# ffs97/deep-mixture-vae

Hardware: AMD Instinct MI355X
Metric: images/sec (train), MNIST K=10 z=64 batch=4096/GPU bf16 (higher is better)
Workload: dtype bf16; 1 GPU; configs[1]: DMVAE MLP 784-500-500-(2000|2000)-z64/K10-2000-500-500-784, one ELBO training step (gather+fwd+loss+bwd+Adam), synthetic rows resident in HBM; per_gpu_batch=4096, global_batch=4096, parallelism=dp1, rccl_ranks=0, multi_rank_rccl_verified_before_this_run=False, hip_graph=True, float_atomics=False, update=adam fused into the dW launch, mode=exact (expectation over q(c|x), priors.py:130-145)

## Files before the change

### deep-mixture-vae_amd/csrc/api.hip

```cpp
#include <stdarg.h>
#include <stdlib.h>
#include <string.h>

#include <map>
#include <mutex>
#include <string>
#include <vector>

#include "plan.h"
#include "gmm_fit.h"
#include "gmm_seed.h"
#include "eval_clusters.h"
#include "eval_loglik.h"
#include "tsne.h"
#include "cluster_metrics.h"
#include "mixture_density.h"
#include "knn.h"
#include "measure.h"

namespace dmvae {

static thread_local char g_err[512] = "";
void set_error(const char* fmt, ...) {
    va_list ap;
// ... 361 lines not shown
    if (me != hipSuccess) { set_error("dmvae_debug_conv_dw memset: %s", hipGetErrorString(me)); return (int)me; }
    return conv_layer_dw((hipStream_t)stream, dtype, rows, conv_p, conv_c, kdim, X, ldx, dY, ldy, N, n_valid, split, slab, dW, db);
}

static int debug_finalize_args(const dmvae_debug_finalize* f, const char* who, dmvae_finalize_args* out) {
    DMVAE_REQUIRE(f && f->rp && f->lp && f->state && f->nr >= 0 && f->nl >= 0 && f->nblk >= 0 && f->ncol >= 0 && (f->ncol == 0 || (f->part && f->gout)),
                  "%s: step_finalize arguments: null pointer or negative count", who);
    *out = step_finalize_args(f->rp, f->nr, f->lp, f->nl, f->inv_B, f->state, f->bump_adam, f->b1, f->b2, f->part, f->nblk, f->ncol, f->gout);
    return 0;
}
extern "C" int dmvae_debug_step_finalize(void* stream, const dmvae_debug_finalize* fin) {
    dmvae_finalize_args f;
    TRY(debug_finalize_args(fin, "dmvae_debug_step_finalize", &f));
    return step_finalize_launch((hipStream_t)stream, f.rp, f.nr, f.lp, f.nl, f.inv_B, f.st, f.bump_adam, f.b1, f.b2, f.part, f.nblk, f.ncol, f.gout);
}
extern "C" int dmvae_debug_gemm_dx_riders(void* stream, int M, int N, int K, const void* A, int64_t lda, const void* B, int64_t ldb, const dmvae_epilogue* epi,
                                          const dmvae_debug_finalize* fin, const dmvae_debug_gather* gat, int ngat, int gat_last) {
    DMVAE_REQUIRE(epi && (epi->kind == DMVAE_EPI_LATENT || epi->kind == DMVAE_EPI_RELU_MASK), "dmvae_debug_gemm_dx_riders: the LATENT or RELU_MASK epilogue");
    DMVAE_REQUIRE(fin || gat, "dmvae_debug_gemm_dx_riders: no riders (use dmvae_gemm)");
    DMVAE_REQUIRE(gat ? (ngat > 0 && ngat % 8 == 0) : ngat == 0, "dmvae_debug_gemm_dx_riders: ngat=%d: a positive multiple of 8 with a gather, 0 without", ngat);
    DMVAE_REQUIRE(!(fin && gat && gat->state), "dmvae_debug_gemm_dx_riders: step_finalize advances the batch cursor a gather addressed through the state reads: not in one launch");
    GemmArgs a;
    TRY(gemm_checked((hipStream_t)stream, DMVAE_BF16, DMVAE_GEMM_DX, M, N, K, A, lda, B, ldb, epi, 1, &a));
    GemmRiders r{};
    if (fin) {
        TRY(debug_finalize_args(fin, "dmvae_debug_gemm_dx_riders", &r.fin));
        r.nfin = (r.fin.nblocks + 7) & ~7;
    }
    if (gat) {
        DMVAE_REQUIRE(gat->data && gat->out_bf16 && gat->n_rows >= 0 && gat->dim > 0 && gat->B_pad > 0 && gat->n_valid >= 0 && gat->n_valid <= gat->B_pad &&
                      gat->ld % 4 == 0 && gat->ld >= gat->dim && (int64_t)gat->B_pad * (gat->ld / 4) < (int64_t(1) << 31) - int64_t(512) * 512 * 16,
                      "dmvae_debug_gemm_dx_riders: gather arguments (ld a multiple of 4, >= dim; n_valid <= B_pad; B_pad x ld within 32-bit quad indices)");
        r.gat = gather_args(DMVAE_BF16, gat->data, gat->n_rows, gat->dim, gat->perm, gat->first, gat->batch, gat->n_valid, gat->B_pad, gat->out_bf16, gat->ld,
                            nullptr, gat->ld, (int)gat->ld, gat->state);
        r.ngat = ngat;
        r.gat_last = gat_last ? 1 : 0;
    }
    DMVAE_REQUIRE(gemm_bf16_riders_room(a, false) >= r.nfin + r.ngat, "dmvae_debug_gemm_dx_riders: %d rider ids, the launch has room for %d (-1: not a small-tile launch)",
                  r.nfin + r.ngat, gemm_bf16_riders_room(a, false));
    DMVAE_REQUIRE(!fin || gemm_bf16_carries_finalize(a), "dmvae_debug_gemm_dx_riders: the two-wave 16-row tile cannot carry the step_finalize blocks");
    return gemm_bf16_dispatch((hipStream_t)stream, DMVAE_GEMM_DX, a, 1, &r);
}
extern "C" int dmvae_debug_gemm_grouped_fin(void* stream, const dmvae_gemm_problem* probs, int n, const dmvae_debug_finalize* fin) {
    DMVAE_REQUIRE(probs && n >= 1 && n <= DMVAE_MAX_GROUP, "dmvae_debug_gemm_grouped_fin: 1..%d problems", DMVAE_MAX_GROUP);
    dmvae_finalize_args f;
    TRY(debug_finalize_args(fin, "dmvae_debug_gemm_grouped_fin", &f));
    hipStream_t s = (hipStream_t)stream;
    std::vector<GemmArgs> q(n);
    for (int i = 0; i < n; ++i) {
        const dmvae_gemm_problem& pr = probs[i];
        TRY(gemm_checked(s, DMVAE_BF16, DMVAE_GEMM_DX, pr.M, pr.N, pr.K, pr.A, pr.lda, pr.B, pr.ldb, &pr.epi, 1, &q[i]));
    }
    return gemm_bf16_grouped(s, DMVAE_GEMM_DX, q.data(), n, &f);
}

extern "C" int dmvae_prof_enable(int on) {
    std::lock_guard<std::mutex> lk(g_prof_mu);
    g_prof_on = on != 0;
    return 0;
}
extern "C" int dmvae_prof_collect(dmvae_prof_row* rows, int max_rows) {
    std::lock_guard<std::mutex> lk(g_prof_mu);
    std::map<std::string, dmvae_prof_row> agg;
    std::vector<std::string> order;
    for (auto& r : g_prof) {
        (void)hipEventSynchronize(r.e1);
        float ms = 0.f;
        (void)hipEventElapsedTime(&ms, r.e0, r.e1);
        double kms = 0.0;
        bool kok = !r.k.empty();
        for (auto& pr : r.k) {
            float d = 0.f;
            if (hipEventSynchronize(pr.second) != hipSuccess || hipEventElapsedTime(&d, pr.first, pr.second) != hipSuccess || !(d > 0.f)) kok = false;
            kms += d;
            g_event_pool.push_back(pr.first);
            g_event_pool.push_back(pr.second);
        }
        (void)hipGetLastError();
        auto it = agg.find(r.name);
        if (it == agg.end()) {
            dmvae_prof_row row;
            memset(&row, 0, sizeof(row));
            snprintf(row.name, sizeof(row.name), "%s", r.name);
            it = agg.emplace(r.name, row).first;
            order.push_back(r.name);
        }
        it->second.launches += 1;
        it->second.total_ms += ms;
        it->second.kernel_ms += kok ? kms : 0.0;
        it->second.kernel_launches += kok ? (int64_t)r.k.size() : 0;
        it->second.flops += r.flops;
        it->second.bytes += r.bytes;
        g_event_pool.push_back(r.e0);
        g_event_pool.push_back(r.e1);
    }
    g_prof.clear();
    g_prof_cur = -1;
    int n = 0;
    for (auto& k : order) {
        if (n >= max_rows) break;
        rows[n++] = agg[k];
    }
    return n;
}

extern "C" int dmvae_debug_set_tile(int bm, int bn) {
// ... 20 lines not shown
```

### deep-mixture-vae_amd/csrc/gemm_bf16.hip

```cpp
#include <algorithm>
#include <cmath>
#include <functional>
#include <map>
#include <mutex>
#include <string>
#include <vector>

#include "gemm_tile.h"
#include "measure.h"

MEAS_TABLES_BF16

namespace dmvae {

template <int BM, int BN, int LAYOUT, int EPI, int NSTAGE, int NW, int BKT = BK, bool CONV = false, bool BONLY = false>
__device__ __forceinline__ void gemm_bf16_body(const GemmArgs& a, const int bid_raw, const int gstart, const int nwg, bf16_t* smem,
                                               const dmvae_adam_ctx* ac = nullptr, const int kslice = -1) {
    constexpr bool A_KC = (LAYOUT != DMVAE_GEMM_DW);
    constexpr bool B_KC = (LAYOUT == DMVAE_GEMM_DX);
    constexpr int A_ELEMS = BM * BKT, B_ELEMS = BN * BKT, STAGE = A_ELEMS + B_ELEMS;
    constexpr int WM = NW / 2;
    constexpr int TM = BM / (16 * WM), TN = BN / 32;
    static_assert(!BONLY || (LAYOUT == DMVAE_GEMM_DW && EPI == DMVAE_EPI_STORE_F32 && !CONV), "bias-only strips: dense DW / STORE_F32");
    constexpr int LOADS = ((BONLY ? 0 : BM) + BN) * BKT / (512 * NW);
// ... 185 lines not shown
    float lat[LAT_PRE ? NQ : 1][12];
    if constexpr (LAT_PRE) {
#pragma unroll
        for (int q = 0; q < NQ; ++q) {
            const int idx = q * (64 * NW) + tid;
            const int ml = idx / (BN / 4), c = idx % (BN / 4);
            loadf4(a.epi.aux0, (int64_t)(m0 + ml) * a.epi.ld0 + n0 + c * 4, lat[q]);
            loadf4(a.epi.aux1, (int64_t)(m0 + ml) * a.epi.ld1 + n0 + c * 4, lat[q] + 4);
            loadf4(a.epi.aux2, (int64_t)(m0 + ml) * a.epi.ld2 + n0 + c * 4, lat[q] + 8);
        }
    }
    constexpr bool HAS_BIAS = (EPI == DMVAE_EPI_BIAS_RELU || EPI == DMVAE_EPI_BIAS_F32 || EPI == DMVAE_EPI_BIAS_SIGMOID || EPI == DMVAE_EPI_BIAS_RECON);
    static_assert((64 * NW) % (BN / 4) == 0, "a thread keeps its column block across the epilogue's passes");
    float bq[4] = {0.f, 0.f, 0.f, 0.f};
    if constexpr (HAS_BIAS) loadf4(a.epi.bias, n0 + (tid % (BN / 4)) * 4, bq);
    uint2 gate[EPI == DMVAE_EPI_RELU_MASK ? NQ : 1];
    if constexpr (EPI == DMVAE_EPI_RELU_MASK) {
#pragma unroll
        for (int q = 0; q < NQ; ++q) {
            const int idx = q * (64 * NW) + tid;
            const int ml = idx / (BN / 4), c = idx % (BN / 4);
            if constexpr (MEAS_NO_MASK_READ) gate[q] = make_uint2(0x3f803f80u, 0x3f803f80u);
            else gate[q] = *reinterpret_cast<const uint2*>(reinterpret_cast<const bf16_t*>(a.epi.aux0) + (int64_t)(m0 + ml) * a.epi.ld0 + n0 + c * 4);
        }
    }
#pragma unroll
    for (int t = 0; t < NSTAGE; ++t)
        if (t < nk) issue(t, t);
    if (nk >= NSTAGE) wait_vmcnt<LOADS*(NSTAGE - 1)>();
    else wait_vmcnt<0>();
    __builtin_amdgcn_s_barrier();
    MEAS_ANAT(1);
    rd(0, 0, f0a, f0b);
    for (int kt = 0; kt < nk; kt += NSTAGE) {
#pragma unroll
        for (int s = 0; s < NSTAGE; ++s) {
            if (kt + s < nk) {
                rd(s, 1, f1a, f1b);
                mma(f0a, f0b);
                asm volatile("s_waitcnt lgkmcnt(0)" ::: "memory");
                if (kt + s + NSTAGE <= nk) wait_vmcnt<LOADS*(NSTAGE - 2)>();
                else wait_vmcnt<0>();
                __builtin_amdgcn_s_barrier();
                if constexpr (!MEAS_NO_KLOOP_LOADS) {
                    if (kt + s + NSTAGE < nk) issue(kt + s + NSTAGE, s);
                }
                if (kt + s + 1 < nk) rd((s + 1) % NSTAGE, 0, f0a, f0b);
                mma(f1a, f1b);
            }
        }
    }
    wait_vmcnt<0>();
    __builtin_amdgcn_s_barrier();
    MEAS_KLOOP_END();
    MEAS_ANAT(2);

    float loss = 0.f;
    const int li = lane & 15, g = lane >> 4;
    constexpr int CH = BN / 4, NT = 64 * NW;
    static_assert(BM * BN * 4 <= NSTAGE * STAGE * 2, "fp32 tile must fit in the ring");
    dmvae_epilogue epi_s = a.epi;
    if constexpr (EPI == DMVAE_EPI_STORE_F32 && (CONV || LAYOUT == DMVAE_GEMM_DW)) {
        const int ys = kslice >= 0 ? kslice : (int)blockIdx.y;
        epi_s.out = reinterpret_cast<float*>(epi_s.out) + (int64_t)ys * a.slab_stride;
        if (epi_s.out2) epi_s.out2 = reinterpret_cast<float*>(epi_s.out2) + (int64_t)ys * a.slab_stride2;
    }
    float* ct = reinterpret_cast<float*>(smem);
    if constexpr (MEAS_NO_EPILOGUE) {
#pragma unroll
        for (int i = 0; i < TM; ++i)
#pragma unroll
            for (int j = 0; j < TN; ++j) asm volatile("" ::"v"(acc[i][j]));
    } else if constexpr (!BONLY) {
#pragma unroll
    for (int i = 0; i < TM; ++i)
#pragma unroll
        for (int j = 0; j < TN; ++j) {
            const int ml = wm * (BM / WM) + i * 16 + li;
            const int c = (wn * (BN / 2) + j * 16) / 4 + g;
            *reinterpret_cast<f32x4*>(ct + ml * BN + ((c ^ (ml & 7)) << 2)) = acc[i][j];
        }
    __syncthreads();
    constexpr int KSPLIT_MAX_S = 8;
    constexpr bool KSLICE_OK = !CONV && LAYOUT != DMVAE_GEMM_DW && BM * BN <= 4096 && NW <= 4 && BM * BN * 4 + 16 <= NSTAGE * STAGE * 2 &&
                               (EPI == DMVAE_EPI_BIAS_RELU || EPI == DMVAE_EPI_RELU_MASK || EPI == DMVAE_EPI_BIAS_F32 || EPI == DMVAE_EPI_LATENT);
    if constexpr (KSLICE_OK) {
        if (a.tick != nullptr && gridDim.y > 1) {
            const int S = (int)gridDim.y, tile_lin = tm * tiles_n + tn;
            constexpr int Q = BM * BN;
            static_assert(KSPLIT_MAX_S == 8, "the combine issues eight loads per quad");
            f32x4* slab0 = reinterpret_cast<f32x4*>(a.ws) + (int64_t)tile_lin * S * (Q / 4);
            const f32x4* ct4 = reinterpret_cast<const f32x4*>(ct);
            for (int q = tid; q < Q / 4; q += 64 * NW) {
                const f32x4 v = ct4[q];
                f32x4* dst = slab0 + (int64_t)blockIdx.y * (Q / 4) + q;
                asm volatile("global_store_dwordx4 %0, %1, off sc1" ::"v"(dst), "v"(v) : "memory");
            }
            asm volatile("s_waitcnt vmcnt(0)" ::: "memory");
            __syncthreads();
            int* flag = reinterpret_cast<int*>(ct + BM * BN);
            if (tid == 0) *flag = __hip_atomic_fetch_add(a.tick + tile_lin, 1, __ATOMIC_RELAXED, __HIP_MEMORY_SCOPE_AGENT);
            __syncthreads();
            if (*flag != S - 1) return;
            for (int q = tid; q < Q / 4; q += 64 * NW) {
                const f32x4 *p0, *p1, *p2, *p3, *p4, *p5, *p6, *p7;
                auto at = [&](int sl) { return slab0 + (int64_t)(sl < S ? sl : S - 1) * (Q / 4) + q; };
// ... 131 lines not shown
    __shared__ __attribute__((aligned(16))) bf16_t smem[NSTAGE * (BM + BN) * BK];
    gemm_bf16_body<BM, BN, LAYOUT, EPI, NSTAGE, NW>(a, blockIdx.x, 0, gridDim.x, smem);
}

template <int BM, int BN, int EPI, int NSTAGE, int NW>
__global__ __launch_bounds__(64 * NW, NW / 2) void gemm_bf16_dx_riders_kernel(GemmArgs a, GemmRiders r) {
    __shared__ __attribute__((aligned(16))) bf16_t smem[NSTAGE * (BM + BN) * BK];
    const int lead = r.nfin + (r.gat_last ? 0 : r.ngat);
    if (blockIdx.y > 0 && ((int)blockIdx.x < lead || (r.gat_last && (int)blockIdx.x >= (int)gridDim.x - r.ngat))) return;
    if (r.gat_last && (int)blockIdx.x >= (int)gridDim.x - r.ngat) {
        if constexpr (MEAS_EMPTY_GATHER_RIDERS) return;
        gather_rows_block<bf16_t, 16>((int)blockIdx.x - ((int)gridDim.x - r.ngat), 64 * NW, r.gat);
        return;
    }
    if ((int)blockIdx.x < r.nfin) {
        if (NW > 4 && threadIdx.x >= 256) return;
        if ((int)blockIdx.x < r.fin.nblocks) step_finalize_block((int)blockIdx.x, r.fin, reinterpret_cast<float(*)[17]>(smem));
        return;
    }
    if ((int)blockIdx.x < lead) {
        if constexpr (MEAS_EMPTY_GATHER_RIDERS) return;
        gather_rows_block<bf16_t, 16>((int)blockIdx.x - r.nfin, 64 * NW, r.gat);
        return;
    }
    gemm_bf16_body<BM, BN, DMVAE_GEMM_DX, EPI, NSTAGE, NW>(a, (int)blockIdx.x - lead, lead, (int)gridDim.x - lead - (r.gat_last ? r.ngat : 0), smem);
}

template <int BM, int BN, int LAYOUT, int EPI, int NSTAGE, int NW>
__global__ __launch_bounds__(64 * NW, NW / 2) void gemm_bf16_conv_kernel(GemmArgs a) {
    __shared__ __attribute__((aligned(16))) bf16_t smem[NSTAGE * (BM + BN) * BK];
    if constexpr (LAYOUT == DMVAE_GEMM_DW) {
        if ((gridDim.y & 7) == 0) {
            const int L = (int)(blockIdx.y * gridDim.x + blockIdx.x), xcd = L & 7, j = L >> 3, T = (int)gridDim.x;
            gemm_bf16_body<BM, BN, LAYOUT, EPI, NSTAGE, NW, BK, true>(a, j % T, 0, -1, smem, nullptr, (j / T) * 8 + xcd);
            return;
        }
    }
    gemm_bf16_body<BM, BN, LAYOUT, EPI, NSTAGE, NW, BK, true>(a, blockIdx.x, 0, gridDim.x, smem);
}

void* gemm_bf16_anatomy() { return MEAS_SYMBOL(g_anat); }
void* gemm_bf16_stamps() { return MEAS_SYMBOL(g_stamps); }
struct GroupedArgs {
    int nprob;
    int kind[DMVAE_MAX_GROUP];
    int start[DMVAE_MAX_GROUP + 1];
    int cls_start[DMVAE_MAX_GROUP], cls_end[DMVAE_MAX_GROUP];
    int nsl[DMVAE_MAX_GROUP];
    GemmArgs p[DMVAE_MAX_GROUP];
    dmvae_adam_ctx adam;
    dmvae_finalize_args fin;
    int lead, lead_work;
    int xcut, xr0[8], xcnt[8];
};
template <int BM, int BN, int LAYOUT, int EPI, int NSTAGE, int NW = 4, bool SHORTK = false>
__global__ __launch_bounds__(64 * NW, NW == 8 ? 4 : 1) void gemm_bf16_grouped_kernel(GroupedArgs g) {
    __shared__ __attribute__((aligned(16))) bf16_t smem[SHORTK ? 2 * (64 + 64) * BK : 3 * (128 + 64) * BK];
    const dmvae_adam_ctx* ac = EPI == DMVAE_EPI_ADAM ? &g.adam : nullptr;
    if constexpr (EPI == DMVAE_EPI_ADAM) {
        if ((int)blockIdx.x < g.lead) {
            if ((int)blockIdx.x >= g.lead_work) return;
            const int64_t n4 = g.adam.seg_n >> 2;
            for (int64_t q = (int64_t)blockIdx.x * (64 * NW) + threadIdx.x; q < n4; q += (int64_t)g.lead_work * (64 * NW)) {
                const int64_t off = g.adam.seg_off + 4 * q;
                const float4 gq = *reinterpret_cast<const float4*>(g.adam.grad + off);
                const float gv[4] = {gq.x, gq.y, gq.z, gq.w};
                adam_quad(g.adam, off, gv);
            }
            return;
        }
    }
    int bx = (int)blockIdx.x;
    if constexpr (EPI == DMVAE_EPI_ADAM) bx -= g.lead;
    if constexpr (EPI == DMVAE_EPI_RELU_MASK) {
        if (bx < g.lead) {
            if (NW > 4 && threadIdx.x >= 256) return;
            if (bx < g.fin.nblocks) step_finalize_block(bx, g.fin, reinterpret_cast<float(*)[17]>(smem));
            return;
        }
        bx -= g.lead;
    }
    int i = 0, item;
    if (g.xcut) {
        const int x = bx & 7, j = bx >> 3;
        if (j >= g.xcnt[x]) return;
        item = g.xr0[x] + j;
    } else {
        while (i + 1 < g.nprob && bx >= g.start[i + 1]) ++i;
        item = g.cls_start[i] + xcd_run_index(bx, g.cls_start[i], g.cls_end[i]);
    }
    i = 0;
    while (i + 1 < g.nprob && item >= g.start[i + 1]) ++i;
    int bid = item - g.start[i];
    const int kind = g.kind[i];
    const int gs = 0, cnt = -1;
    int ksl = -1;
    if (g.nsl[i] > 1) {
        const int tiles_i = (g.start[i + 1] - g.start[i]) / g.nsl[i];
        ksl = bid / tiles_i;
        bid -= ksl * tiles_i;
    }
    MEAS_WG_BEGIN();
    if constexpr (SHORTK) {
        gemm_bf16_body<64, 64, LAYOUT, EPI, 2, NW>(g.p[i], bid, gs, cnt, smem, ac, ksl);
    } else {
        if (kind == 0) gemm_bf16_body<128, 128, LAYOUT, EPI, 2, NW>(g.p[i], bid, gs, cnt, smem, ac, ksl);
        else if (kind == 1) gemm_bf16_body<128, 64, LAYOUT, EPI, 3, NW>(g.p[i], bid, gs, cnt, smem, ac, ksl);
        else if (kind == 3) {
            if constexpr (LAYOUT == DMVAE_GEMM_DW && EPI == DMVAE_EPI_STORE_F32)
                gemm_bf16_body<64, 64, LAYOUT, EPI, 4, NW, BK, false, true>(g.p[i], bid, gs, cnt, smem, ac, ksl);
        }
// ... 26 lines not shown
        snprintf(nm[0], 64, "gemm_bf16_kernel<%d, %d, %d, %d, %d, %d>", BM, BN, LAYOUT, EPI, NSTAGE, NW);
        snprintf(nm[1], 64, "gemm_bf16_grouped_kernel<%d, %d, %d, %d, %d, %d>", BM, BN, LAYOUT, EPI, NSTAGE, NW);
        init = true;
    }
    return nm[grouped ? 1 : 0];
}
static double gemm_bytes(const GemmArgs& a, int layout = DMVAE_GEMM_FWD) {
    const int k = a.epi.kind;
    if (k == DMVAE_EPI_ADAM) return 2.0 * ((double)a.M * a.K + (double)a.K * a.N);
    const double osz = (k == DMVAE_EPI_STORE_F32 || k == DMVAE_EPI_ATOMIC_F32 || k == DMVAE_EPI_BIAS_F32 || k == DMVAE_EPI_BIAS_SIGMOID) ? 4.0 : 2.0;
    if (a.conv_c) {
        const double nv = a.epi.n_valid > 0 ? a.epi.n_valid : a.N;
        if (layout == DMVAE_GEMM_DW) return 2.0 * ((double)a.K * a.lda + (double)a.K * a.ldb) + 4.0 * a.M * nv;
        return 2.0 * ((double)a.M * a.lda + (double)a.K * a.N) + osz * a.M * nv;
    }
    return 2.0 * ((double)a.M * a.K + (double)a.K * a.N) + osz * a.M * a.N;
}

template <int BM, int BN, int LAYOUT, int EPI, int NSTAGE, int NW = 4>
static int launch(hipStream_t s, const GemmArgs& a, int split, const GemmRiders* riders = nullptr) {
    dim3 grid((a.M / BM) * (a.N / BN), split);
    if constexpr (LAYOUT == DMVAE_GEMM_DX && (EPI == DMVAE_EPI_LATENT || EPI == DMVAE_EPI_RELU_MASK)) {
        if (riders && (split == 1 || a.tick)) {
            GemmRiders r = *riders;
            double rbytes = 0.0;
            if (r.ngat) { r.gat.nblocks = r.ngat; rbytes = (double)r.gat.n_valid * r.gat.dim * (4 + 2); }
            ProfScope ps(s, kernel_name<BM, BN, LAYOUT, EPI, NSTAGE, NW>(false), 2.0 * a.M * a.N * (double)a.K, gemm_bytes(a) + rbytes);
            DMVAE_LAUNCH((gemm_bf16_dx_riders_kernel<BM, BN, EPI, NSTAGE, NW>), dim3(grid.x + r.nfin + r.ngat, split), dim3(64 * NW), 0, s, a, r);
            return check_launch("gemm_bf16 (dX + riders)");
        }
    }
    if (riders) { set_error("gemm_bf16: riders are carried by the dense DX launches with the LATENT or RELU_MASK epilogue only"); return DMVAE_EINVAL; }
    ProfScope ps(s, kernel_name<BM, BN, LAYOUT, EPI, NSTAGE, NW>(false), 2.0 * a.M * a.N * (double)a.K, gemm_bytes(a));
    DMVAE_LAUNCH((gemm_bf16_kernel<BM, BN, LAYOUT, EPI, NSTAGE, NW>), grid, dim3(64 * NW), 0, s, a);
    return check_launch("gemm_bf16");
}

template <int BM, int BN, int LAYOUT, int EPI, int NSTAGE, int NW = 4>
static int launch_conv(hipStream_t s, const GemmArgs& a, int split) {
    dim3 grid((a.M / BM) * (a.N / BN), split);
    static const std::string nm = [] {
        char b[64];
        snprintf(b, sizeof(b), "gemm_bf16_conv_kernel<%d, %d, %d, %d, %d, %d>", BM, BN, LAYOUT, EPI, NSTAGE, NW);
        return std::string(b);
    }();
    const double P = a.conv_p, inner = (P - 2.0) * (P - 2.0) / (P * P), nv = a.epi.n_valid > 0 ? a.epi.n_valid : a.N;
    const double fl = 2.0 * (LAYOUT == DMVAE_GEMM_DW ? (double)a.K : (double)a.M) * inner * 9.0 * a.conv_c * nv;
    ProfScope ps(s, nm.c_str(), fl, gemm_bytes(a, LAYOUT));
    DMVAE_LAUNCH((gemm_bf16_conv_kernel<BM, BN, LAYOUT, EPI, NSTAGE, NW>), grid, dim3(64 * NW), 0, s, a);
    return check_launch("gemm_bf16_conv");
}

template <int LAYOUT, int EPI>
static int grouped_launch(hipStream_t s, const GemmArgs* probs, int nprob, const dmvae_adam_ctx* ctx = nullptr, const dmvae_finalize_args* fin = nullptr) {
    auto best_kind = [](const GemmArgs& p) { return p.bias_only ? 3 : (p.M % 128 == 0 && p.N % 128 == 0) ? 0 : (p.M % 128 == 0 ? 1 : 2); };
    auto nslices = [](const GemmArgs& p) { return (p.k_split > 0 && p.k_split < p.K) ? p.K / p.k_split : 1; };
    auto tiles = [&](const GemmArgs& p, int kind) {
        if (kind == 3) return (p.N / 64) * nslices(p);
        return (p.M / (kind == 2 ? 64 : 128)) * (p.N / (kind == 0 ? 128 : 64)) * nslices(p);
    };
    auto wg_bytes = [&](const GemmArgs& p, int kind) {
        if (kind == 3) return 2.0 * 64 * (double)(p.K / nslices(p));
        return 2.0 * ((kind == 2 ? 64 : 128) + (kind == 0 ? 128 : 64)) * (double)(p.K / nslices(p));
    };
    int kinds[DMVAE_MAX_GROUP];
    bool shortk = g_shortk && LAYOUT != DMVAE_GEMM_DW && EPI != DMVAE_EPI_ADAM;
    for (int i = 0; i < nprob; ++i) shortk = shortk && probs[i].K <= 128;
    for (int i = 0; i < nprob; ++i) kinds[i] = (g_grouped_mixed && !shortk) ? best_kind(probs[i]) : 2;
    if (g_grouped_mixed == 1 && !shortk) {
        static std::mutex mu;
        static std::map<std::vector<int>, std::vector<int>> memo;
        std::vector<int> key;
        for (int i = 0; i < nprob; ++i) { key.push_back(probs[i].M); key.push_back(probs[i].N); key.push_back(probs[i].K); key.push_back(nslices(probs[i]) * 2 + (probs[i].bias_only ? 1 : 0)); }
        std::lock_guard<std::mutex> lk(mu);
        auto it = memo.find(key);
        if (it == memo.end()) {
            std::vector<int> cur(kinds, kinds + nprob), best = cur;
            double best_max = 1e300, best_sum = 1e300;
            std::vector<double> s;
            for (;;) {
                s.clear();
                double sum = 0.0;
                for (int i = 0; i < nprob; ++i) {
                    const int t = tiles(probs[i], cur[i]);
                    s.insert(s.end(), (size_t)t, wg_bytes(probs[i], cur[i]));
                    sum += t * wg_bytes(probs[i], cur[i]);
                }
                std::sort(s.begin(), s.end(), std::greater<double>());
                double load[256] = {0.0}, mx = 0.0;
                for (size_t j = 0; j < s.size(); ++j) load[j & 255] += s[j];
                for (double l : load) mx = std::max(mx, l);
                if (mx < best_max * 0.99 || (mx < best_max * 1.01 && sum < best_sum)) { best_max = std::min(mx, best_max); best_sum = sum; best = cur; }
                int i = 0;
                while (i < nprob && (cur[i] == 2 || kinds[i] == 3)) { cur[i] = kinds[i]; ++i; }
                if (i == nprob) break;
                ++cur[i];
            }
            it = memo.emplace(key, best).first;
        }
        for (int i = 0; i < nprob; ++i) kinds[i] = it->second[i];
    }
    int order[DMVAE_MAX_GROUP];
    for (int i = 0; i < nprob; ++i) order[i] = i;
    std::stable_sort(order, order + nprob, [&](int x, int y) { return wg_bytes(probs[x], kinds[x]) > wg_bytes(probs[y], kinds[y]); });
    GroupedArgs g;
    g.nprob = nprob;
    int total = 0, n = 0;
    double flops = 0.0, bytes = 0.0;
    for (int o = 0; o < nprob; ++o) {
        const int i = order[o], kind = kinds[i];
        g.start[n] = total;
        g.kind[n] = kind;
        g.nsl[n] = nslices(probs[i]);
        g.p[n] = probs[i];
        g.p[n].group_m = gemm_auto_group_m(probs[i].M / (kind >= 2 ? 64 : 128), probs[i].N / (kind == 0 ? 128 : 64),
                                      kind >= 2 ? 64 : 128, kind == 0 ? 128 : 64);
        total += tiles(probs[i], kind);
        flops += 2.0 * probs[i].M * probs[i].N * (double)probs[i].K;
        bytes += gemm_bytes(probs[i]);
        ++n;
    }
    for (int i = nprob; i < DMVAE_MAX_GROUP; ++i) { g.kind[i] = 2; g.nsl[i] = 1; }
    for (int i = nprob; i <= DMVAE_MAX_GROUP; ++i) g.start[i] = total;
    for (int i = 0; i < DMVAE_MAX_GROUP; ++i) { g.cls_start[i] = g.start[std::min(i, nprob)]; g.cls_end[i] = g.start[std::min(i + 1, nprob)]; }
    if (g_grouped_cls)
        for (int lo = 0; lo < nprob;) {
            int hi = lo + 1;
            while (hi < nprob && g.kind[hi] == g.kind[lo] && 2 * std::min(g.p[hi].K / g.nsl[hi], g.p[lo].K / g.nsl[lo]) > std::max(g.p[hi].K / g.nsl[hi], g.p[lo].K / g.nsl[lo])) ++hi;
            const double run = std::max(1.0, (g.start[hi] - g.start[lo]) / 8.0);
            for (int i = lo; i < hi; ++i) {
                g.cls_start[i] = g.start[lo];
                g.cls_end[i] = g.start[hi];
                const int kind = g.kind[i], bm = kind >= 2 ? 64 : 128, bn = kind == 0 ? 128 : 64;
                const int t = (g.start[i + 1] - g.start[i]) / g.nsl[i];
                g.p[i].group_m = gemm_auto_group_m(g.p[i].M / bm, g.p[i].N / bn, bm, bn, std::min<double>(t, run));
            }
            lo = hi;
        }
    g.xcut = 0;
    int grid_items = total;
    if (LAYOUT == DMVAE_GEMM_DW && g_grouped_xcut && total >= 64) {
        double tot_b = 0.0;
        std::vector<double> cost((size_t)total);
        for (int i = 0; i < nprob; ++i)
            for (int j = g.start[i]; j < g.start[i + 1]; ++j) { cost[j] = wg_bytes(g.p[i], g.kind[i]); tot_b += cost[j]; }
        int cuts[9] = {0};
        double acc = 0.0;
        int x = 1;
        for (int j = 0; j < total && x < 8; ++j) {
            acc += cost[j];
            while (x < 8 && acc >= tot_b * x / 8.0 - 1e-6) cuts[x++] = j + 1;
        }
        while (x < 8) cuts[x++] = total;
        cuts[8] = total;
        int mx = 0;
        for (int k = 0; k < 8; ++k) { g.xr0[k] = cuts[k]; g.xcnt[k] = cuts[k + 1] - cuts[k]; mx = std::max(mx, g.xcnt[k]); }
        g.xcut = 1;
        grid_items = 8 * mx;
        for (int i = 0; i < nprob; ++i) {
            int share = 1;
            for (int k = 0; k < 8; ++k) share = std::max(share, std::min(cuts[k + 1], g.start[i + 1]) - std::max(cuts[k], g.start[i]));
            const int kind = g.kind[i], bm = kind >= 2 ? 64 : 128, bn = kind == 0 ? 128 : 64;
            const int t = (g.start[i + 1] - g.start[i]) / g.nsl[i];
            g.p[i].group_m = gemm_auto_group_m(g.p[i].M / bm, g.p[i].N / bn, bm, bn, std::min<double>(t, share));
        }
    }
    int extra = 0;
    g.fin = dmvae_finalize_args{};
    g.lead = 0; g.lead_work = 0;
    if (fin && EPI == DMVAE_EPI_RELU_MASK) { g.fin = *fin; g.lead = (fin->nblocks + 7) & ~7; extra = g.lead; }
    g.adam = dmvae_adam_ctx{};
    if (ctx) {
        g.adam = *ctx;
        double elems = (double)ctx->seg_n;
        for (int i = 0; i < nprob; ++i) elems += (double)probs[i].M * probs[i].N + (probs[i].epi.out2 ? probs[i].N : 0);
        bytes += elems * (24.0 + (ctx->param_bf16 ? 2.0 : 0.0) + (ctx->store_grad ? 4.0 : 0.0)) + 4.0 * ctx->seg_n;
        if (ctx->seg_n > 0) { g.lead_work = (int)std::min<int64_t>(4, (ctx->seg_n / 4 + 255) / 256); g.lead = 8; extra = g.lead; }
    }
    static const std::string pname = [] {
        char b[64];
        snprintf(b, sizeof(b), "gemm_bf16_grouped_mixed_tiles<L%d, E%d>", LAYOUT, EPI);
        return std::string(b);
    }();
    ProfScope ps(s, pname.c_str(), flops, bytes);
    if constexpr (LAYOUT != DMVAE_GEMM_DW) {
        if (shortk) {
            DMVAE_LAUNCH((gemm_bf16_grouped_kernel<64, 64, LAYOUT, EPI, 2, 4, true>), dim3(total + extra), dim3(256), 0, s, g);
            return check_launch("gemm_bf16_grouped");
        }
    }
    if constexpr (LAYOUT == DMVAE_GEMM_DX && EPI == DMVAE_EPI_RELU_MASK) {
        if (g_dx_group_nw == 8) {
            DMVAE_LAUNCH((gemm_bf16_grouped_kernel<64, 64, LAYOUT, EPI, 4, 8>), dim3(total + extra), dim3(512), 0, s, g);
            return check_launch("gemm_bf16_grouped");
        }
    }
    DMVAE_LAUNCH((gemm_bf16_grouped_kernel<64, 64, LAYOUT, EPI, 4, 4>), dim3(grid_items + extra), dim3(256), 0, s, g);
    return check_launch("gemm_bf16_grouped");
}

int gemm_bf16_grouped(hipStream_t s, int layout, const GemmArgs* probs, int nprob, const dmvae_finalize_args* fin) {
    if (nprob < 1 || nprob > DMVAE_MAX_GROUP) { set_error("dmvae_gemm_grouped: 1..%d problems", DMVAE_MAX_GROUP); return DMVAE_EINVAL; }
    const int epi = probs[0].epi.kind;
    for (int i = 1; i < nprob; ++i)
        if (probs[i].epi.kind != epi) { set_error("dmvae_gemm_grouped: all problems must share the epilogue kind"); return DMVAE_EINVAL; }
    if (layout == DMVAE_GEMM_DW && epi == DMVAE_EPI_STORE_F32) return grouped_launch<DMVAE_GEMM_DW, DMVAE_EPI_STORE_F32>(s, probs, nprob);
    if (layout == DMVAE_GEMM_FWD && epi == DMVAE_EPI_BIAS_F32) return grouped_launch<DMVAE_GEMM_FWD, DMVAE_EPI_BIAS_F32>(s, probs, nprob);
    if (fin && !(layout == DMVAE_GEMM_DX && epi == DMVAE_EPI_RELU_MASK)) { set_error("dmvae_gemm_grouped: step_finalize rides on DX / RELU_MASK groups only"); return DMVAE_EINVAL; }
    if (layout == DMVAE_GEMM_DX && epi == DMVAE_EPI_RELU_MASK) {
        bool taken[DMVAE_MAX_GROUP];
        const int rc = heads_dx_stream_launch(s, probs, nprob, fin, taken);
        if (rc) return rc;
        GemmArgs rest[DMVAE_MAX_GROUP];
        int nrest = 0, ntaken = 0;
        for (int i = 0; i < nprob; ++i) {
            if (taken[i]) ++ntaken;
            else rest[nrest++] = probs[i];
        }
        if (nrest == 0) return 0;
        return grouped_launch<DMVAE_GEMM_DX, DMVAE_EPI_RELU_MASK>(s, rest, nrest, nullptr, ntaken ? nullptr : fin);
    }
    set_error("dmvae_gemm_grouped: layout %d with epilogue %d is not instantiated", layout, epi);
    return DMVAE_EUNSUPPORTED;
}
static int peel_large_dw(hipStream_t s, const GemmArgs* probs, int nprob, const dmvae_adam_ctx* ctx, std::vector<GemmArgs>& rest) {
    std::vector<GemmArgs> large;
    bool any = false;
    for (int i = 0; i < nprob; ++i)
        any = any || (probs[i].k_split == probs[i].K && gemm_bf16_256_ok(DMVAE_GEMM_DW, probs[i].epi.kind, probs[i].M, probs[i].N, probs[i].K, probs[i].conv_c != 0));
    for (int i = 0; i < nprob; ++i) {
        const GemmArgs& p = probs[i];
        if (p.k_split != p.K && !p.bias_only && !p.epi.out2 && p.slab_stride && gemm_bf16_256_slice_ok(p.M, p.N, p.k_split)) { large.push_back(p); continue; }
        const bool own = p.k_split == p.K && gemm_bf16_256_ok(DMVAE_GEMM_DW, p.epi.kind, p.M, p.N, p.K, p.conv_c != 0);
        const bool rides = any && gemm_bf16_256_rides() && p.k_split == p.K && !p.conv_c && p.M % 256 == 0 && p.N % 256 == 0 && p.K >= 1024 &&
                           (p.epi.kind == DMVAE_EPI_STORE_F32 || p.epi.kind == DMVAE_EPI_ADAM);
        if (own || rides) large.push_back(p);
        else rest.push_back(p);
    }
    return large.empty() ? 0 : gemm_bf16_256_dw_all(s, large.data(), (int)large.size(), ctx);
}
int gemm_bf16_grouped_dw(hipStream_t s, const GemmArgs* probs, int nprob) {
    if (nprob < 1 || nprob > DMVAE_MAX_GROUP) { set_error("dmvae_gemm_grouped_dw: 1..%d problems", DMVAE_MAX_GROUP); return DMVAE_EINVAL; }
    std::vector<GemmArgs> rest;
    for (int i = 0; i < nprob; ++i)
        if (probs[i].epi.kind != DMVAE_EPI_STORE_F32) return gemm_bf16_grouped(s, DMVAE_GEMM_DW, probs, nprob, nullptr);
    const int rc = peel_large_dw(s, probs, nprob, nullptr, rest);
    if (rc) return rc;
    return rest.empty() ? 0 : gemm_bf16_grouped(s, DMVAE_GEMM_DW, rest.data(), (int)rest.size(), nullptr);
}
int gemm_bf16_grouped_dw_adam(hipStream_t s, const GemmArgs* probs, int nprob, const dmvae_adam_ctx& ctx) {
    if (nprob < 1 || nprob > DMVAE_MAX_GROUP) { set_error("dmvae_gemm_grouped_dw_adam: 1..%d problems", DMVAE_MAX_GROUP); return DMVAE_EINVAL; }
    for (int i = 0; i < nprob; ++i)
        if (probs[i].epi.kind != DMVAE_EPI_ADAM || !probs[i].epi.out) { set_error("dmvae_gemm_grouped_dw_adam: every problem needs epilogue kind ADAM and out = its gradient address"); return DMVAE_EINVAL; }
    if (!ctx.param || !ctx.grad || !ctx.m || !ctx.v || !ctx.state || (ctx.seg_off & 3) || (ctx.seg_n & 3) || ctx.seg_n < 0) {
        set_error("dmvae_gemm_grouped_dw_adam: null arena / state, or a segment that is not a multiple of 4 elements");
        return DMVAE_EINVAL;
    }
    for (int i = 0; i < nprob; ++i) {
        const int64_t end = (reinterpret_cast<const float*>(probs[i].epi.out) - ctx.grad) + (int64_t)probs[i].M * probs[i].epi.ldo;
        if (end < 0 || end > ADAM_QUADS_MAX_ELEMS) { set_error("dmvae_gemm_grouped_dw_adam: gradient %d ends %lld elements into the arena (limit 2^30)", i, (long long)end); return DMVAE_EUNSUPPORTED; }
    }
    std::vector<GemmArgs> rest;
    dmvae_adam_ctx c1 = ctx;
    c1.seg_n = 0;
    const int rc = peel_large_dw(s, probs, nprob, &c1, rest);
    if (rc) return rc;
    if (!rest.empty()) return grouped_launch<DMVAE_GEMM_DW, DMVAE_EPI_ADAM>(s, rest.data(), (int)rest.size(), &ctx);
    if (ctx.seg_n > 0) {
        AdamArgs a;
        a.n = ctx.seg_n; a.p = ctx.param + ctx.seg_off; a.g = ctx.grad + ctx.seg_off; a.m = ctx.m + ctx.seg_off; a.v = ctx.v + ctx.seg_off;
        a.pb = ctx.param_bf16 ? reinterpret_cast<bf16_t*>(ctx.param_bf16) + ctx.seg_off : nullptr;
        a.lr = 0.f; a.b1 = ctx.beta1; a.b2 = ctx.beta2; a.eps = ctx.epsilon; a.gscale = ctx.grad_scale; a.zero_grad = 0; a.ieee = ctx.ieee;
        a.t_host = ~0ull; a.st = reinterpret_cast<const dmvae_state*>(ctx.state);
        return adam_launch(s, a);
    }
    return 0;
}

static int g_force_tile = 0;
void gemm_bf16_force_tile(int t) { g_force_tile = t; }
static int g_nw8 = 1;
void gemm_bf16_set_knob(int which, int v) {
    if (which == 0) g_group_m = v < 0 ? 0 : v;
    if (which == 1) g_nw8 = v;
    if (which == 2) g_grouped_mixed = v;
    if (which == 4) g_grouped_cls = v;
    if (which == 5) g_conv_short = v;
    if (which == 6) gemm_bf16_256_set_policy(v);
    if (which == 7) g_shortk = v;
    if (which == 8) gemm_bf16_256_set_stagger(v);
    if (which == 9) g_dx_group_nw = v;
    if (which == 18) g_thin = v;
    if (which == 20) g_grouped_xcut = v;
}

static int gemm_bf16_thin_rows(const GemmArgs& a) {
    if (!g_thin || a.conv_c || a.N != 64 || a.K < 1024 || (a.k_split != a.K && !a.tick)) return 0;
    if (g_thin >= 2 && a.M % 16 == 0 && a.M / 16 <= 256) return 16;
    if (a.M % 32 == 0 && a.M / 32 <= 256) return 32;
    return 0;
}

int gemm_bf16_tile_m(int M, int N, int split) {
    if (g_force_tile) {
        const int bm = g_force_tile / 1000, bn = g_force_tile % 1000;
        if (M % bm == 0 && N % bn == 0) return g_force_tile;
    }
    static const int cand[4][2] = {{128, 128}, {128, 64}, {64, 128}, {64, 64}};
    double best = -1.0;
    int pick = 64 * 1000 + 64;
    for (auto& c : cand) {
        if (M % c[0] || N % c[1]) continue;
        const double wgs = (double)(M / c[0]) * (N / c[1]) * split;
        const double score = (double)c[0] * c[1] / (c[0] + c[1]) * (wgs >= 256.0 ? 1.0 : wgs / 256.0);
        if (score > best * 1.0001) { best = score; pick = c[0] * 1000 + c[1]; }
    }
    if (pick == 128128 && (double)(M / 128) * (N / 128) * split <= 256.0 && (double)(M / 128) * (N / 64) * split >= 384.0) pick = 128064;
    return pick;
}

// ... 91 lines not shown
```

### deep-mixture-vae_amd/csrc/gemm_epilogue.h

```cpp
#pragma once
#include "common.h"

namespace dmvae {

struct GemmArgs {
    const void* A; int64_t lda;
    const void* B; int64_t ldb;
    int M, N, K, k_split;
    int group_m;
    int conv_p, conv_c;
    dmvae_epilogue epi;
    float* ws = nullptr; int64_t ws_elems = 0;
    int64_t slab_stride = 0;
    int64_t slab_stride2 = 0;
    float* csum_out = nullptr; int64_t csum_ld = 0;
    const float* csum_in = nullptr; int csum_rows = 0;
    int bias_only = 0;
    int* tick = nullptr;
};

__host__ __device__ __forceinline__ int64_t conv_tap_offset(int tap, int c0, int P, int64_t lda) {
    return (int64_t)((tap / 3 - 1) * P + (tap % 3 - 1)) * lda + c0;
}

template <typename T> struct ActIO;
template <> struct ActIO<bf16_t> {
    static __device__ __forceinline__ void store4(void* base, int64_t off, const float v[4]) {
        uint2 p;
        p.x = pack2bf(v[0], v[1]);
        p.y = pack2bf(v[2], v[3]);
        *reinterpret_cast<uint2*>(reinterpret_cast<bf16_t*>(base) + off) = p;
    }
    static __device__ __forceinline__ void load4(const void* base, int64_t off, float v[4]) {
        const uint2 p = *reinterpret_cast<const uint2*>(reinterpret_cast<const bf16_t*>(base) + off);
        v[0] = __uint_as_float(p.x << 16);
        v[1] = __uint_as_float(p.x & 0xffff0000u);
        v[2] = __uint_as_float(p.y << 16);
        v[3] = __uint_as_float(p.y & 0xffff0000u);
    }
};
template <> struct ActIO<float> {
    static __device__ __forceinline__ void store4(void* base, int64_t off, const float v[4]) {
        *reinterpret_cast<float4*>(reinterpret_cast<float*>(base) + off) = make_float4(v[0], v[1], v[2], v[3]);
    }
    static __device__ __forceinline__ void load4(const void* base, int64_t off, float v[4]) {
        const float4 p = *reinterpret_cast<const float4*>(reinterpret_cast<const float*>(base) + off);
        v[0] = p.x; v[1] = p.y; v[2] = p.z; v[3] = p.w;
    }
};

__device__ __forceinline__ void loadf4(const void* base, int64_t off, float v[4]) {
    ActIO<float>::load4(base, off, v);
}

__device__ __forceinline__ float xent_logits(float l, float x) {
    return fmaxf(l, 0.f) - l * x + log1pf(__expf(-fabsf(l)));
}
__device__ __forceinline__ float sigmoidf_(float l) { return 1.0f / (1.0f + __expf(-l)); }
struct dmvae_gather_args {
    const float* data; int64_t n_rows; int dim; const int32_t* perm;
    int64_t first; int batch, n_valid, B_pad;
    void* out_act; int64_t ld_act; float* out_f32; int64_t ld_f32; int cols_pad;
    const dmvae_state* st;
    int nblocks;
};
template <typename ACT, int U, bool PERM>
__device__ __forceinline__ void gather_rows_pass(const int base, const int nthreads, const int total, const int quads, const int64_t first, const dmvae_gather_args& g) {
    int r[U], c[U];
    int64_t idx[U];
    bool inb[U];
#pragma unroll
// ... 8 lines not shown
    if constexpr (PERM) {
#pragma unroll
        for (int u = 0; u < U; ++u) idx[u] = (int64_t)g.perm[idx[u]];
    }
    float4 q[U];
#pragma unroll
    for (int u = 0; u < U; ++u) {
        inb[u] = inb[u] && idx[u] >= 0 && idx[u] < g.n_rows && c[u] < g.dim;
        q[u] = *reinterpret_cast<const float4*>(g.data + (inb[u] ? idx[u] * g.dim + c[u] : 0));
    }
#pragma unroll
    for (int u = 0; u < U; ++u) {
        if (r[u] < 0) continue;
        const float v[4] = {inb[u] ? q[u].x : 0.f, inb[u] ? q[u].y : 0.f, inb[u] ? q[u].z : 0.f, inb[u] ? q[u].w : 0.f};
        if (g.out_act) ActIO<ACT>::store4(g.out_act, (int64_t)r[u] * g.ld_act + c[u], v);
        if (g.out_f32) ActIO<float>::store4(g.out_f32, (int64_t)r[u] * g.ld_f32 + c[u], v);
    }
}
template <typename ACT, int U = 8>
__device__ __forceinline__ void gather_rows_block(const int bx, const int nthreads, const dmvae_gather_args& g) {
    int64_t first = g.first;
    if (g.st) first = (int64_t)g.st->batch_cursor * g.batch;
    const int quads = g.cols_pad >> 2;
    const int total = g.B_pad * quads;
    if (g.dim % 4 == 0 && (reinterpret_cast<uintptr_t>(g.data) & 15) == 0 && g.n_rows > 0) {
        for (int base = bx * nthreads * U + (int)threadIdx.x; base < total; base += g.nblocks * nthreads * U) {
            if (g.perm) gather_rows_pass<ACT, U, true>(base, nthreads, total, quads, first, g);
            else gather_rows_pass<ACT, U, false>(base, nthreads, total, quads, first, g);
        }
        return;
    }
    for (int i = bx * nthreads + (int)threadIdx.x; i < total; i += g.nblocks * nthreads) {
        const int r = i / quads, c = (i - r * quads) * 4;
        float v[4] = {0.f, 0.f, 0.f, 0.f};
        if (r < g.n_valid) {
            int64_t src = first + r;
            if (g.perm) src = (src >= 0 && src < g.n_rows) ? (int64_t)g.perm[src] : -1;
            if (src >= 0 && src < g.n_rows) {
                const float* p = g.data + src * g.dim + c;
#pragma unroll
                for (int j = 0; j < 4; ++j) v[j] = (c + j < g.dim) ? p[j] : 0.f;
            }
        }
        if (g.out_act) ActIO<ACT>::store4(g.out_act, (int64_t)r * g.ld_act + c, v);
        if (g.out_f32) ActIO<float>::store4(g.out_f32, (int64_t)r * g.ld_f32 + c, v);
    }
}

struct GemmRiders {
    dmvae_finalize_args fin; int nfin = 0;
    dmvae_gather_args gat; int ngat = 0;
    int gat_last = 0;
};

__device__ __forceinline__ void xent_sigmoid(float l, float x, float& xent, float& sig) {
    const float e = __expf(-fabsf(l));
    const float inv = __frcp_rn(1.0f + e);
    xent = fmaxf(l, 0.f) - l * x + __logf(1.0f + e);
    sig = l >= 0.f ? inv : e * inv;
}

template <int EPI, typename ACT>
__device__ __forceinline__ void epilogue_quad(const dmvae_epilogue& e, int m, int n, float v[4], float& loss, const float* xpre = nullptr, float* stored = nullptr,
                                              const float* bpre = nullptr, const float* ypre = nullptr) {
    if constexpr (EPI == DMVAE_EPI_BIAS_RELU) {
        float b[4];
        if (bpre) { b[0] = bpre[0]; b[1] = bpre[1]; b[2] = bpre[2]; b[3] = bpre[3]; }
        else loadf4(e.bias, n, b);
#pragma unroll
        for (int j = 0; j < 4; ++j) v[j] = fmaxf(v[j] + b[j], 0.f);
        ActIO<ACT>::store4(e.out, (int64_t)m * e.ldo + n, v);
    } else if constexpr (EPI == DMVAE_EPI_BIAS_F32) {
        float b[4];
        if (bpre) { b[0] = bpre[0]; b[1] = bpre[1]; b[2] = bpre[2]; b[3] = bpre[3]; }
        else loadf4(e.bias, n, b);
#pragma unroll
        for (int j = 0; j < 4; ++j) v[j] += b[j];
        ActIO<float>::store4(e.out, (int64_t)m * e.ldo + n, v);
    } else if constexpr (EPI == DMVAE_EPI_BIAS_SIGMOID) {
        float b[4];
        if (bpre) { b[0] = bpre[0]; b[1] = bpre[1]; b[2] = bpre[2]; b[3] = bpre[3]; }
        else loadf4(e.bias, n, b);
#pragma unroll
        for (int j = 0; j < 4; ++j) v[j] = sigmoidf_(v[j] + b[j]);
        ActIO<float>::store4(e.out, (int64_t)m * e.ldo + n, v);
    } else if constexpr (EPI == DMVAE_EPI_BIAS_RECON) {
        float b[4], x[4], d[4];
        if (bpre) { b[0] = bpre[0]; b[1] = bpre[1]; b[2] = bpre[2]; b[3] = bpre[3]; }
        else loadf4(e.bias, n, b);
        if (xpre) { x[0] = xpre[0]; x[1] = xpre[1]; x[2] = xpre[2]; x[3] = xpre[3]; }
        else loadf4(e.aux0, (int64_t)m * e.ld0 + n, x);
        const bool rowok = m < e.m_valid;
#pragma unroll
        for (int j = 0; j < 4; ++j) {
            const float l = v[j] + b[j];
            v[j] = l;
            const bool ok = rowok && (n + j) < e.n_valid;
            if ((e.recon_kind & 0xff) == 0) {
                float xe, sg;
                xent_sigmoid(l, x[j], xe, sg);
                loss += ok ? xe : 0.f;
                d[j] = ok ? (sg - x[j]) * e.scale : 0.f;
            } else {
                const float r = l - x[j];
                loss += ok ? 0.5f * r * r : 0.f;
                d[j] = ok ? r * e.scale : 0.f;
// ... 41 lines not shown
```

### deep-mixture-vae_amd/csrc/kernels.h

```cpp
#pragma once
#include "gemm_epilogue.h"

namespace dmvae {

struct AdamArgs {
    int64_t n;
    float* p; float* g; float* m; float* v; bf16_t* pb;
    float lr, b1, b2, eps, gscale;
    int zero_grad;
    int ieee;
    uint64_t t_host;
    const dmvae_state* st;
};

#define DMVAE_MAX_GROUP 16
int gemm_bf16_dispatch(hipStream_t s, int layout, const GemmArgs& a, int split, const GemmRiders* riders = nullptr);
int gemm_bf16_riders_room(const GemmArgs& a, bool own_cu);
bool gemm_bf16_carries_finalize(const GemmArgs& a);
int gemm_bf16_grouped_dw(hipStream_t s, const GemmArgs* probs, int nprob);
int gemm_bf16_grouped(hipStream_t s, int layout, const GemmArgs* probs, int nprob, const dmvae_finalize_args* fin = nullptr);
dmvae_finalize_args step_finalize_args(const float* rp, int nr, const float* lp, int nl, float inv_B, void* st, int bump_adam,
                                       float b1, float b2, const float* part, int nblk, int ncol, float* gout);
int gemm_bf16_tile_m(int M, int N, int split);
int gemm_auto_group_m(int tiles_m, int tiles_n, int bm, int bn, double run = 0.0);
bool gemm_bf16_256_ok(int layout, int epi, int M, int N, int K, bool conv);
int gemm_bf16_256_launch(hipStream_t s, int layout, const GemmArgs& a, const dmvae_adam_ctx* ctx = nullptr);
void gemm_bf16_256_set_policy(int v);
void gemm_bf16_256_set_stagger(int v);
bool gemm_bf16_256_slice_ok(int M, int N, int k_split);
bool gemm_bf16_256_rides();
int gemm_bf16_256_dw_all(hipStream_t s, const GemmArgs* probs, int n, const dmvae_adam_ctx* ctx);
void* heads_dx_phase_table();
int heads_dx_stream_launch(hipStream_t s, const GemmArgs* probs, int nprob, const dmvae_finalize_args* fin, bool* taken);
void heads_dx_stream_set(int v);
void gemm_bf16_force_tile(int t);
void gemm_bf16_set_knob(int which, int v);
int gemm_f32_dispatch(hipStream_t s, int layout, const GemmArgs& a, int split);
int gemm_f32_trio(hipStream_t s, const GemmArgs& g1, int split1, const GemmArgs& g2, int split2, const GemmArgs& g3, int split3);
int latent_nblocks(int B_pad, int D, int K);
int latent_launch(hipStream_t s, const dmvae_latent_args* a);
void latent_set_blocks_target(int v);
int latent_vade_nblocks(int B_pad);
int latent_vade_launch(hipStream_t s, const dmvae_latent_args* a);
size_t latent_vade_lds_bytes(int D, int K);
bool latent_vade_mfma_needed(int D, int K);
bool latent_vade_mfma_forced();
void latent_vade_force_mfma(int v);
int64_t latent_vade_mfma_ws_bytes(int B_pad, int D, int K, int* n_slabs);
int latent_vade_mfma_launch(hipStream_t s, const dmvae_latent_args* a, float* ws, int64_t ws_bytes);
bool heads_latent_ok(int B_pad, int D, int K, int Dp, int Kp, int Hp, int mode, int rows_per_latent_block);
int heads_latent_launch(hipStream_t s, const dmvae_latent_args* a, const dmvae_heads_args* h);
void heads_latent_set(int v);
int64_t heads_latent_kslice_floats(int B_pad, int Dp, int slices);
int strip_fwd2_launch(hipStream_t s, int B_pad, int K0, const void* X, int64_t ldx, const void* W0, int64_t ld0, const float* b0,
                      const void* W1, int64_t ld1, const float* b1, void* Y1, int64_t ldy1, void* Y2, int64_t ldy2);
bool latent_mfma_applies(int D, int K, int mode);
int64_t latent_mfma_ws_bytes(int B_pad, int D, int K);
int latent_mfma_launch(hipStream_t s, const dmvae_latent_args* a, float* ws, int64_t ws_bytes);
int adam_launch(hipStream_t s, const AdamArgs& a);
int adam_shadow_launch(hipStream_t s, const AdamArgs& a, int blocks);
int adam_finish_launch(hipStream_t s, void* st);
int adam_slabs_launch(hipStream_t s, const AdamArgs& a, const float* slabs, int nslab, int64_t stride, int64_t seg_lo, int64_t seg_hi);
int slab_reduce_launch(hipStream_t s, const float* slabs, int64_t n, int nslab, int64_t stride, float* out);
int colsum_prepare(int64_t max_n);
float* colsum_global_scratch(int64_t* elems);
int colsum_launch(hipStream_t s, int in_dtype, const void* in, int64_t ld, int M, int N, float* out, float* ws, int64_t ws_elems);
int recon_nblocks(int B_pad, int I_pad);
int recon_launch(hipStream_t s, int act_dtype, int recon_kind, int B, int B_pad, int I, int I_pad, const float* logits, int64_t ldl,
                 const float* x, int64_t ldx, float inv_B, void* dl, int64_t ldd, float* partials);
int loss_finalize_launch(hipStream_t s, const float* rp, int nr, const float* lp, int nl, float inv_B, void* st, int bump_adam);
int step_finalize_launch(hipStream_t s, const float* rp, int nr, const float* lp, int nl, float inv_B, void* st, int bump_adam,
                         float b1, float b2, const float* part, int nblk, int ncol, float* gout);
int gemm_bf16_grouped_dw_adam(hipStream_t s, const GemmArgs* probs, int nprob, const dmvae_adam_ctx& ctx);
dmvae_gather_args gather_args(int act_dtype, const float* data, int64_t n_rows, int dim, const int32_t* perm, int64_t first, int batch, int n_valid,
                              int B_pad, void* out_act, int64_t ld_act, float* out_f32, int64_t ld_f32, int cols_pad, const void* st);
int gather_launch(hipStream_t s, int act_dtype, const float* data, int64_t n_rows, int dim, const int32_t* perm, int64_t first, int batch,
                  int n_valid, int B_pad, void* out_act, int64_t ld_act, float* out_f32, int64_t ld_f32, int cols_pad, const void* st);
int philox_launch(hipStream_t s, float* out, int64_t n, uint64_t seed, uint64_t step, uint32_t sid, int gumbel);
int cast_launch(hipStream_t s, const void* in, void* out, int64_t n, int to_bf16);
int spin_launch(hipStream_t s, int us);
void* gemm_bf16_stamps();
void* gemm_bf16_anatomy();
void* gemm_bf16_256_anatomy();
int conv_first_fwd_launch(hipStream_t s, int dtype, const void* x, int64_t bstride, int H, int64_t n_img, const void* W, int ldw,
                          const float* bias, int cout, void* out, int ld);
int conv_first_dw_blocks(int H, int64_t n_img);
int conv_first_dw_launch(hipStream_t s, int dtype, const void* x, int64_t bstride, int H, int64_t n_img, const void* dY, int ld, int cout,
                         float* dW, int ldw, float* db, float* part);
int zero_border_launch(hipStream_t s, int dtype, void* a, int P, int ld, int64_t n_img);
int maxpool2_fwd_launch(hipStream_t s, int dtype, const void* in, int H, int ld, int64_t n_img, void* out, int out_border);
int maxpool2_bwd_relu_launch(hipStream_t s, int dtype, const void* in, const void* dout, int H, int ld, int64_t n_img, void* din, int dout_border);
int conv_wflip_launch(hipStream_t s, int dtype, const void* W, int cin, int cin_ld, int cout, int ldw, void* Wt, int Kt);

}
```

### deep-mixture-vae_amd/csrc/measure.h

```cpp
#pragma once

#ifndef DMVAE_ABLATE
#define DMVAE_ABLATE 0
#endif

namespace dmvae {
constexpr bool MEAS_NO_MFMA = DMVAE_ABLATE == 1 || DMVAE_ABLATE == 4;
constexpr bool MEAS_NO_LDS_READ = DMVAE_ABLATE == 2 || DMVAE_ABLATE == 4;
constexpr bool MEAS_NO_KLOOP_LOADS = DMVAE_ABLATE == 3;
constexpr bool MEAS_NO_EPILOGUE = DMVAE_ABLATE == 5;
constexpr bool MEAS_NO_MASK_READ = DMVAE_ABLATE == 8;
constexpr bool MEAS_NO_BIAS_MFMA = DMVAE_ABLATE == 9;
constexpr bool MEAS_STAMPS = DMVAE_ABLATE == 6;
constexpr bool MEAS_NO_STEP_GATHER = DMVAE_ABLATE == 11;
constexpr bool MEAS_EMPTY_GATHER_RIDERS = DMVAE_ABLATE == 12;
}

#if DMVAE_ABLATE == 6
#define MEAS_TABLES_BF16                                  \
    __device__ unsigned long long g_mid[2048];            \
    __device__ unsigned long long g_anat[2048 * 8];       \
    __device__ unsigned long long g_stamps[2048 * 4];
#define MEAS_HWID() (((unsigned long long)__builtin_amdgcn_s_getreg((31 << 11) | 4) << 32) | (unsigned)__builtin_amdgcn_s_getreg((3 << 11) | 20))
#define MEAS_ANAT(i) do { if (threadIdx.x == 0 && blockIdx.x < 2048) g_anat[blockIdx.x * 8 + (i)] = __builtin_amdgcn_s_memrealtime(); } while (0)
#define MEAS_KLOOP_END() do { if (threadIdx.x == 0 && blockIdx.x < 2048) g_mid[blockIdx.x] = __builtin_amdgcn_s_memrealtime(); } while (0)
#define MEAS_ANAT_DRAIN()                                                                             \
    do {                                                                                              \
        MEAS_ANAT(3);                                                                                 \
        asm volatile("s_waitcnt vmcnt(0)" ::: "memory");                                              \
        MEAS_ANAT(4);                                                                                 \
        if (threadIdx.x == 0 && blockIdx.x < 2048) g_anat[blockIdx.x * 8 + 5] = MEAS_HWID();          \
    } while (0)
#define MEAS_WG_BEGIN() const unsigned long long meas_t0_ = __builtin_amdgcn_s_memrealtime()
#define MEAS_WG_END(layout, kind)                                                                                          \
    do {                                                                                                                   \
        if (threadIdx.x == 0 && blockIdx.x < 2048) {                                                                       \
            unsigned long long* st_ = g_stamps + 4 * blockIdx.x;                                                           \
            st_[0] = meas_t0_;                                                                                             \
            st_[1] = __builtin_amdgcn_s_memrealtime();                                                                     \
            st_[2] = MEAS_HWID();                                                                                          \
            st_[3] = ((g_mid[blockIdx.x] - meas_t0_) << 16) | ((unsigned long long)(layout) << 8) | (unsigned)(kind);       \
        }                                                                                                                  \
    } while (0)
#define MEAS_TABLES_256 __device__ unsigned long long g_anat256[4096 * 8];
#define MEAS_ANAT256(i)                                                                                  \
    do {                                                                                                 \
        if (threadIdx.x == 0 && blockIdx.x < 4096) {                                                     \
            g_anat256[blockIdx.x * 8 + (i)] = __builtin_amdgcn_s_memrealtime();                          \
            if ((i) < 2) g_anat256[blockIdx.x * 8 + 4 + (i)] = __builtin_amdgcn_s_memtime();             \
        }                                                                                                \
    } while (0)
#define MEAS_ANAT256_DRAIN()                                                                             \
    do {                                                                                                 \
        asm volatile("s_waitcnt vmcnt(0)" ::: "memory");                                                 \
        __syncthreads();                                                                                 \
        MEAS_ANAT256(2);                                                                                 \
        if (threadIdx.x == 0 && blockIdx.x < 4096) g_anat256[blockIdx.x * 8 + 3] = MEAS_HWID();          \
    } while (0)
#define MEAS_SYMBOL(sym) ([] { void* p_ = nullptr; return hipGetSymbolAddress(&p_, HIP_SYMBOL(sym)) == hipSuccess ? p_ : nullptr; }())
#else
#define MEAS_TABLES_BF16
#define MEAS_TABLES_256
#define MEAS_ANAT(i) do { } while (0)
#define MEAS_KLOOP_END() do { } while (0)
#define MEAS_ANAT_DRAIN() do { } while (0)
#define MEAS_WG_BEGIN() do { } while (0)
#define MEAS_WG_END(layout, kind) do { } while (0)
#define MEAS_ANAT256(i) do { } while (0)
#define MEAS_ANAT256_DRAIN() do { } while (0)
#define MEAS_SYMBOL(sym) (static_cast<void*>(nullptr))
#endif

#if DMVAE_ABLATE == 10
#define MEAS_TABLES_HDX __device__ unsigned long long g_hdx[1024 * 16];
#define MEAS_HDX_BEGIN() unsigned long long hx_[12] = {}; unsigned long long hx_last_; hx_[0] = __builtin_amdgcn_s_memtime(); hx_[10] = __builtin_amdgcn_s_memrealtime()
#define MEAS_HDX_MARK(i) do { hx_last_ = __builtin_amdgcn_s_memtime(); hx_[i] = hx_last_; } while (0)
#define MEAS_HDX_ACC(i) do { const unsigned long long t_ = __builtin_amdgcn_s_memtime(); hx_[i] += t_ - hx_last_; hx_last_ = t_; } while (0)
#define MEAS_HDX_END(steps)                                                                                                        \
    do {                                                                                                                           \
        MEAS_HDX_MARK(3);                                                                                                          \
        asm volatile("s_waitcnt vmcnt(0)" ::: "memory");                                                                           \
        MEAS_HDX_MARK(4);                                                                                                          \
        hx_[11] = __builtin_amdgcn_s_memrealtime();                                                                                \
        if (threadIdx.x == 0 && blockIdx.x < 1024) {                                                                               \
            for (int i_ = 0; i_ < 12; ++i_) g_hdx[blockIdx.x * 16 + i_] = hx_[i_];                                                 \
            g_hdx[blockIdx.x * 16 + 13] = (unsigned long long)(steps);                                                             \
            g_hdx[blockIdx.x * 16 + 12] = (((unsigned long long)__builtin_amdgcn_s_getreg((31 << 11) | 4) << 32) | (unsigned)__builtin_amdgcn_s_getreg((3 << 11) | 20)); \
        }                                                                                                                          \
    } while (0)
#define MEAS_SYMBOL_HDX(sym) ([] { void* p_ = nullptr; return hipGetSymbolAddress(&p_, HIP_SYMBOL(sym)) == hipSuccess ? p_ : nullptr; }())
#else
#define MEAS_TABLES_HDX
#define MEAS_HDX_BEGIN() do { } while (0)
#define MEAS_HDX_MARK(i) do { } while (0)
#define MEAS_HDX_ACC(i) do { } while (0)
#define MEAS_HDX_END(steps) do { } while (0)
#define MEAS_SYMBOL_HDX(sym) (static_cast<void*>(nullptr))
#endif

#if DMVAE_ABLATE == 7
#define MEAS_LAT_STAMP(i) do { if (blockIdx.x == 0 && threadIdx.x == 0) reinterpret_cast<unsigned long long*>(L.a.loss_partials + 2 * gridDim.x)[i] = __builtin_amdgcn_s_memrealtime(); } while (0)
#else
#define MEAS_LAT_STAMP(i) do { } while (0)
#endif
```

### deep-mixture-vae_amd/csrc/plan.h

```cpp
#pragma once
#include <string.h>

#include <string>
#include <vector>

#include "kernels.h"

#define TRY(x) do { int rc_ = (x); if (rc_) return rc_; } while (0)

struct PLayer {
    std::string name;
    int in, out, in_pad, out_pad;
    int64_t w_off, b_off, ldw;
};

struct PConv {
    std::string name;
    int cin, cout, hw, pool;
    int cin_ld, cout_ld;
    int cin_np, cout_np;
    int P;
    int kdim, ktdim;
    int64_t w_off, b_off;
    int64_t o_act, o_dact;
// ... 10 lines not shown
    const PAct* whole = nullptr;

    PAct sub(int c0, int n) const {
        PAct v = *this;
        v.off += (int64_t)c0 * es; v.cols = n; v.cs_live = false; v.whole = whole ? whole : this;
        if (cs >= 0) v.cs += (int64_t)c0 * 4;
        return v;
    }
    void mark_cs_live() const { (whole ? whole : this)->cs_live = true; }
};

struct dmvae_plan {
    dmvae_config cfg;
    std::vector<PConv> conv;
    int flat = 0;
    int64_t o_wt = 0, o_c0part = 0, o_cslab = 0;
    int64_t conv_param_end = 0;
    int Bp, Ip, Dp, Kp, Hp, Tp;
    int es;
    std::vector<PLayer> enc, dec;
    PLayer zc, mv, lg, out;
    int64_t prior_off;
    int64_t tail_off = 0;
    int64_t param_elems;
    std::vector<dmvae_tensor_info> tensors;
    struct {
        PAct x, xf, x2, cflat, dflat, hzc, mv, lg, Z, Zf, gmu, glv, clv, w, dlg, recon, dl, dmv, dhzc;
        std::vector<PAct> enc, dec, denc, ddec;
    } a;
    int64_t o_rpart, o_lpart, o_dprior, o_cs, o_lws = 0;
    int64_t lws_bytes = 0;
    int64_t o_ksws = -1, ksws_elems = 0, o_ktick = -1;
    int n_rpart, n_lblk, n_pblk;
    int n_lblk_cap = 0;
    int64_t cs_elems;
    int64_t work_bytes;
    dmvae_buffers buf;
    bool bound;
    std::vector<dmvae::GemmArgs> dw_queue;
    int dw_slices_max = 1;
    int64_t o_dwslab = 0;
    int dw_slices_now = 1;
    bool dw_macro_now = false;
    int dw_macro_tiles = 0;
    bool fused_update = false;
    bool staged = false;
    int stage_groups = 3;
    struct { const float* data; int64_t n_rows; const int32_t* perm; int64_t first; int n_valid; const void* st; } tsrc{};
    bool tsrc_valid = false;
    bool tsrc_used = false;
    bool tgt_gather = false;
    int xsel = 0;
    struct { const float* data; int64_t n_rows; const int32_t* perm; int64_t first; int n_valid; const void* st; bool armed, done; dmvae::dmvae_gather_args gat; } pf{};
    bool vade = false;
    struct {
        bool on = false;
        dmvae_moe_config cfg{};
        int EO = 0, EOp = 0;
        PLayer L;
        PAct P, dP, inp, dq, pred, acc;
        int64_t o_part = 0;
        int nblk = 0;
        const int32_t* perm = nullptr; int64_t first = 0; const void* st = nullptr;
    } moe;
};

static inline int pad64(int x) { return (x + 63) / 64 * 64; }
static inline char* WS(const dmvae_plan* p, int64_t off) { return reinterpret_cast<char*>(p->buf.work) + off; }
static inline char* WS(const dmvae_plan* p, const PAct& a) { return WS(p, a.off); }
template <class X> static inline float* WSf(const dmvae_plan* p, const X& x) { return reinterpret_cast<float*>(WS(p, x)); }
static inline const void* Wp(const dmvae_plan* p, int64_t off) {
    return p->cfg.dtype == DMVAE_BF16 ? (const void*)(reinterpret_cast<const bf16_t*>(p->buf.param_bf16) + off)
                                      : (const void*)(p->buf.param + off);
}
static inline const PAct& XB(const dmvae_plan* p, int other = 0) { return ((p->xsel ^ other) && p->a.x2.off >= 0) ? p->a.x2 : p->a.x; }
static inline char* rows0(const dmvae_plan* p, int64_t off, int P, int ld) { return WS(p, off) + (int64_t)(P + 1) * ld * p->es; }

template <class A> static inline void latent_inputs(const dmvae_plan* p, A& a, const float* eps, int64_t ld_eps) {
    a.B_pad = p->Bp; a.D = p->cfg.latent_dim; a.K = p->cfg.n_classes;
    a.mean = WSf(p, p->a.mv); a.ld_mean = p->a.mv.ld;
    a.log_var = WSf(p, p->a.mv.sub(p->Dp, p->Dp)); a.ld_log_var = p->a.mv.ld;
    a.prior_means = p->buf.param + p->prior_off;
    a.prior_log_vars = a.prior_means + (int64_t)p->cfg.n_classes * p->cfg.latent_dim;
    a.eps = eps; a.ld_eps = ld_eps; a.seed = p->cfg.seed;
}
template <class A> static inline void latent_sample(const dmvae_plan* p, A& a) {
    a.Z_act = WS(p, p->a.Z); a.ld_Z = p->a.Z.ld;
    a.Z_f32 = p->cfg.dtype == DMVAE_BF16 ? WSf(p, p->a.Zf) : nullptr; a.ld_Zf = p->a.Zf.ld;
}

namespace dmvae {
int gemm_checked(hipStream_t s, int dtype, int layout, int M, int N, int K, const void* A, int64_t lda, const void* B, int64_t ldb,
                 const dmvae_epilogue* epi, int split, GemmArgs* deferred = nullptr, int conv_p = 0, int conv_c = 0);
int gemm_partials(int dtype, int M, int N);
constexpr int KSPLIT_MAX_ROWS = 256, KSPLIT_MAX_SLICES = 8;
bool step_set_knob(int which, int value);
int fwd_dense(dmvae_plan* p, hipStream_t s, const PAct& in, const PLayer& L, int kind, const PAct& out, GemmArgs* deferred = nullptr);
int encode_impl(dmvae_plan* p, hipStream_t s, bool heads = true);
int decode_hidden(dmvae_plan* p, hipStream_t s);
int moe_stage(dmvae_plan* p, hipStream_t s, int n_valid, float inv_B, bool backward);
int conv_dw_split(int64_t K, int tiles);
int conv_layer_dw(hipStream_t s, int dt, int M, int P, int cin, int kdim, const void* in, int64_t cin_ld, const void* dact, int64_t cout_ld,
                  int cout_np, int cout, int sp, float* slab, float* dW, float* db);
}
```

### deep-mixture-vae_amd/csrc/plan.hip

```cpp
#include <stdlib.h>

#include <algorithm>

#include "plan.h"
#include "moe_head.h"

using namespace dmvae;

static inline int64_t align_up(int64_t x, int64_t a) { return (x + a - 1) / a * a; }
static int64_t take(int64_t& w, int64_t bytes) { int64_t o = w; w += align_up(bytes, 256); return o; }
static PAct take_act(int64_t& w, int64_t rows, int cols, int es) {
    PAct a;
    a.off = take(w, rows * cols * es); a.cols = cols; a.ld = cols; a.es = es;
    return a;
}

static void add_tensor(dmvae_plan* p, const std::string& name, int64_t off, int rows, int cols, int64_t ld) {
    dmvae_tensor_info t;
    memset(&t, 0, sizeof(t));
    snprintf(t.name, sizeof(t.name), "%s", name.c_str());
    t.offset = off; t.rows = rows; t.cols = cols; t.ld = ld;
    p->tensors.push_back(t);
}

// ... 153 lines not shown
    }
    p->n_rpart = gemm_partials(c->dtype, p->Bp, p->Ip);
    p->o_rpart = take(w, (int64_t)p->n_rpart * 4);
    p->n_lblk = p->vade ? latent_vade_nblocks(p->Bp) : latent_nblocks(p->Bp, c->latent_dim, c->n_classes);
    p->n_lblk_cap = std::max(p->n_lblk, (p->Bp + 15) / 16);
    p->o_lpart = take(w, (int64_t)p->n_lblk_cap * 2 * 4);
    p->lws_bytes = p->vade ? (latent_vade_mfma_needed(c->latent_dim, c->n_classes) ? latent_vade_mfma_ws_bytes(p->Bp, c->latent_dim, c->n_classes, nullptr) : 0)
                 : latent_mfma_applies(c->latent_dim, c->n_classes, c->mode) ? latent_mfma_ws_bytes(p->Bp, c->latent_dim, c->n_classes) : 0;
    p->n_pblk = p->lws_bytes ? 1 : p->n_lblk;
    p->o_dprior = take(w, (int64_t)(p->lws_bytes ? 1 : p->n_lblk_cap) * 2 * KD * 4);
    if (p->lws_bytes) p->o_lws = take(w, p->lws_bytes);
    if (c->dtype == DMVAE_BF16 && p->Bp <= 2048) {
        int64_t need = p->Bp <= KSPLIT_MAX_ROWS ? (int64_t)(p->Bp / 64) * 8 * KSPLIT_MAX_SLICES * 4096 : 0;
        if (p->Dp == 64 || p->Dp == 128)
            for (int S = 2; S <= KSPLIT_MAX_SLICES; S *= 2)
                if ((p->Bp / 16) * S <= 256) need = std::max(need, heads_latent_kslice_floats(p->Bp, p->Dp, S));
        if (need > 0) {
            p->ksws_elems = need;
            p->o_ksws = take(w, p->ksws_elems * 4);
            p->o_ktick = take(w, 256 * 4);
        }
    }
    int maxN = std::max(std::max(2 * p->Hp, p->Ip), p->flat);
    for (auto& L : p->enc) maxN = std::max(maxN, L.out_pad);
    for (auto& L : p->dec) maxN = std::max(maxN, L.out_pad);
    maxN = std::max(maxN, 2 * KD);
    p->cs_elems = (int64_t)64 * maxN;
    p->o_cs = take(w, p->cs_elems * 4);
    {
        bool macro = false;
        int n_dw = 0, n_elig = 0, tiles = 0;
        auto cnt = [&](const PLayer& L) {
            macro = macro || gemm_bf16_256_ok(DMVAE_GEMM_DW, DMVAE_EPI_ADAM, L.in_pad, L.out_pad, (int)Bp, false);
            ++n_dw;
            if (L.in_pad % 256 == 0 && L.out_pad % 256 == 0) { ++n_elig; tiles += (L.in_pad / 256) * (L.out_pad / 256); }
        };
        for (auto& L : p->enc) cnt(L);
        for (auto& L : p->dec) cnt(L);
        if (!p->vade) { cnt(p->zc); cnt(p->lg); }
        cnt(p->mv); cnt(p->out);
        if (c->dtype == DMVAE_BF16 && p->conv.empty() && Bp >= 8192 && Bp % (4 * 64) == 0 && !macro && n_dw + n_elig < DMVAE_MAX_GROUP) {
            p->dw_slices_max = 4;
            p->o_dwslab = take(w, (int64_t)p->dw_slices_max * p->param_elems * 4);
            p->dw_macro_tiles = tiles;
        }
    }
    p->tgt_gather = c->dtype == DMVAE_BF16 && c->input_dim % 4 == 0 &&
                    !gemm_bf16_256_ok(DMVAE_GEMM_FWD, DMVAE_EPI_BIAS_RECON, p->Bp, p->Ip, p->dec.back().out_pad, false);
    p->work_bytes = w;
    *out = p;
    return 0;
}

extern "C" void dmvae_plan_destroy(dmvae_plan* p) { delete p; }

extern "C" int dmvae_plan_sizes(const dmvae_plan* p, dmvae_sizes* o) {
    DMVAE_REQUIRE(p && o, "dmvae_plan_sizes: null argument");
    o->param_elems = p->param_elems;
    o->work_bytes = p->work_bytes;
    o->batch_pad = p->Bp;
    o->input_pad = p->Ip;
    o->n_tensors = (int)p->tensors.size();
    o->reserved = 0;
    return 0;
}
extern "C" int dmvae_plan_tensor(const dmvae_plan* p, int i, dmvae_tensor_info* o) {
    DMVAE_REQUIRE(p && o && i >= 0 && i < (int)p->tensors.size(), "dmvae_plan_tensor: bad index %d", i);
    *o = p->tensors[i];
    return 0;
}
extern "C" int dmvae_plan_bind(dmvae_plan* p, const dmvae_buffers* b) {
    DMVAE_REQUIRE(p && b && b->param && b->grad && b->m && b->v && b->work && b->state, "dmvae_plan_bind: null buffer");
    DMVAE_REQUIRE(p->cfg.dtype == DMVAE_F32 || b->param_bf16, "dmvae_plan_bind: bf16 plan needs the bf16 parameter shadow");
    DMVAE_REQUIRE((uintptr_t)b->work % 256 == 0 && (uintptr_t)b->param % 256 == 0 && (uintptr_t)b->grad % 256 == 0, "dmvae_plan_bind: buffers must be 256-byte aligned");
    p->buf = *b;
    if (p->buf.arena_elems == 0) p->buf.arena_elems = p->param_elems;
    DMVAE_REQUIRE(p->buf.arena_elems >= p->param_elems && p->buf.arena_elems % 4 == 0, "dmvae_plan_bind: arena_elems %lld < the plan's %lld parameters (or not a multiple of 4)",
                  (long long)p->buf.arena_elems, (long long)p->param_elems);
    p->bound = true;
    return 0;
}

extern "C" int dmvae_plan_attach_moe(dmvae_plan* p, const dmvae_moe_config* m) {
    DMVAE_REQUIRE(p && m, "dmvae_plan_attach_moe: null argument");
    DMVAE_REQUIRE(!p->bound && !p->moe.on, "dmvae_plan_attach_moe: attach once, before dmvae_plan_bind");
    if (p->vade || !p->conv.empty() || p->dw_slices_max > 1) {
        set_error("dmvae_plan_attach_moe: the MoE head runs on DMVAE plans with the MLP trunk and fewer than 8192 rows (VaDE: its gate p(c|z) "
                  "sends gradients through Z; conv trunk: the flat input is not resident; larger batches: dW K-slices)");
        return DMVAE_EUNSUPPORTED;
    }
    const int E = m->n_experts, O = m->output_dim;
    DMVAE_REQUIRE(E == p->cfg.n_classes, "dmvae_plan_attach_moe: n_experts %d must equal the gate's n_classes %d", E, p->cfg.n_classes);
    DMVAE_REQUIRE(E >= 1 && E <= 256 && O >= 1 && O <= 64 && E * O <= 1024, "dmvae_plan_attach_moe: E=%d, O=%d (E <= 256, O <= 64, E*O <= 1024)", E, O);
    DMVAE_REQUIRE(m->labels && m->label_rows > 0, "dmvae_plan_attach_moe: null labels");
    auto& M = p->moe;
    M.cfg = *m;
    M.EO = E * O; M.EOp = pad64(M.EO);
    const bool fl = m->featLearn != 0;
    PLayer& L = M.L;
    L.name = "moe"; L.in = fl ? p->cfg.latent_dim : p->cfg.input_dim; L.in_pad = fl ? p->Dp : p->Ip; L.out = M.EO; L.out_pad = M.EOp; L.ldw = M.EOp;
    L.w_off = p->out.w_off + (int64_t)p->out.in_pad * p->out.out_pad;
    const int64_t tail = align_up(L.w_off + (int64_t)L.in_pad * L.ldw, 4096);
    const int64_t dt = tail - p->tail_off;
    for (auto& c : p->conv) c.b_off += dt;
    for (auto& l : p->enc) l.b_off += dt;
    for (auto& l : p->dec) l.b_off += dt;
    p->zc.b_off += dt; p->mv.b_off += dt; p->lg.b_off += dt; p->out.b_off += dt;
// ... 81 lines not shown
```

### deep-mixture-vae_amd/csrc/step.hip

```cpp
#include <algorithm>

#include "plan.h"
#include "moe_head.h"
#include "measure.h"

using namespace dmvae;

static int g_dw_slices = 0;
static int g_dw_macro = 1;
static int g_pf_rides = 1;
static int g_fin_rides = 1;
static int g_heads_dx_form = 0;
static int g_ksplit = 1;
bool dmvae::step_set_knob(int which, int value) {
    int* const k = which == 10 ? &g_dw_slices : which == 11 ? &g_dw_macro : which == 12 ? &g_heads_dx_form : which == 16 ? &g_fin_rides :
                   which == 17 ? &g_pf_rides : which == 21 ? &g_ksplit : nullptr;
    if (k) *k = value;
    return k != nullptr;
}

static void batch_rows(dmvae_plan* p, const int32_t* perm, int64_t first, const void* st) {
    p->pf.armed = p->pf.done = false;
    p->moe.perm = perm; p->moe.first = first; p->moe.st = st;
}
extern "C" int dmvae_plan_load_batch(dmvae_plan* p, void* stream, const float* data, int64_t n_rows, const int32_t* perm,
                                     int64_t first, int n_valid, int use_state_cursor) {
    DMVAE_REQUIRE(p && p->bound && data, "dmvae_plan_load_batch: plan not bound / null data");
    DMVAE_REQUIRE(n_valid >= 0 && n_valid <= p->cfg.max_batch, "dmvae_plan_load_batch: n_valid=%d exceeds max_batch=%d", n_valid, p->cfg.max_batch);
    void* xa = p->cfg.dtype == DMVAE_BF16 ? (void*)WS(p, XB(p)) : nullptr;
    p->tsrc_valid = false;
    batch_rows(p, perm, first, use_state_cursor ? p->buf.state : nullptr);
    return gather_launch((hipStream_t)stream, p->cfg.dtype, data, n_rows, p->cfg.input_dim, perm, first, p->cfg.max_batch, n_valid, p->Bp, xa, p->Ip,
                         WSf(p, p->a.xf), p->Ip, p->Ip, use_state_cursor ? p->buf.state : nullptr);
}

extern "C" int dmvae_plan_load_batch_step(dmvae_plan* p, void* stream, const float* data, int64_t n_rows, const int32_t* perm,
                                          int64_t first, int n_valid, int use_state_cursor) {
    DMVAE_REQUIRE(p && p->bound && data, "dmvae_plan_load_batch_step: plan not bound / null data");
    DMVAE_REQUIRE(n_valid >= 0 && n_valid <= p->cfg.max_batch, "dmvae_plan_load_batch_step: n_valid=%d exceeds max_batch=%d", n_valid, p->cfg.max_batch);
    if (!p->tgt_gather) return dmvae_plan_load_batch(p, stream, data, n_rows, perm, first, n_valid, use_state_cursor);
    p->tsrc.data = data; p->tsrc.n_rows = n_rows; p->tsrc.perm = perm; p->tsrc.first = first; p->tsrc.n_valid = n_valid;
    p->tsrc.st = use_state_cursor ? p->buf.state : nullptr;
    p->tsrc_valid = true;
    p->tsrc_used = false;
    batch_rows(p, perm, first, p->tsrc.st);
    if constexpr (MEAS_NO_STEP_GATHER) {
        static int calls = 0;
        if (++calls > 2) return 0;
    }
    return gather_launch((hipStream_t)stream, DMVAE_BF16, data, n_rows, p->cfg.input_dim, perm, first, p->cfg.max_batch, n_valid, p->Bp,
                         WS(p, XB(p)), p->Ip, nullptr, p->Ip, p->Ip, use_state_cursor ? p->buf.state : nullptr);
}

extern "C" int dmvae_plan_prefetch_batch(dmvae_plan* p, const float* data, int64_t n_rows, const int32_t* perm, int64_t first, int n_valid,
                                         int use_state_cursor) {
    DMVAE_REQUIRE(p && p->bound && data, "dmvae_plan_prefetch_batch: plan not bound / null data");
    DMVAE_REQUIRE(n_valid >= 0 && n_valid <= p->cfg.max_batch, "dmvae_plan_prefetch_batch: n_valid=%d exceeds max_batch=%d", n_valid, p->cfg.max_batch);
    if (p->moe.on) { set_error("dmvae_plan_prefetch_batch: not with a MoE attachment (its labels follow the current batch)"); return DMVAE_EUNSUPPORTED; }
    if (!p->tgt_gather || p->a.x2.off < 0) { set_error("dmvae_plan_prefetch_batch: this plan assembles its batches with dmvae_plan_load_batch (f32, conv trunk, or an output layer on the macro tile)"); return DMVAE_EUNSUPPORTED; }
    DMVAE_REQUIRE(p->tsrc_valid && !p->tsrc_used, "dmvae_plan_prefetch_batch: no current batch (dmvae_plan_load_batch_step or dmvae_plan_swap_batch first)");
    p->pf.data = data; p->pf.n_rows = n_rows; p->pf.perm = perm; p->pf.first = first; p->pf.n_valid = n_valid;
    p->pf.st = use_state_cursor ? p->buf.state : nullptr;
    p->pf.armed = true; p->pf.done = false;
    return 0;
}
extern "C" int dmvae_plan_swap_batch(dmvae_plan* p) {
    DMVAE_REQUIRE(p && p->bound, "dmvae_plan_swap_batch: plan not bound");
    DMVAE_REQUIRE(p->pf.done, "dmvae_plan_swap_batch: no pass has run since dmvae_plan_prefetch_batch");
    p->xsel ^= 1;
    p->tsrc.data = p->pf.data; p->tsrc.n_rows = p->pf.n_rows; p->tsrc.perm = p->pf.perm; p->tsrc.first = p->pf.first; p->tsrc.n_valid = p->pf.n_valid;
    p->tsrc.st = p->pf.st;
    p->tsrc_valid = true; p->tsrc_used = false;
    p->pf.armed = p->pf.done = false;
    return 0;
}
// ... 64 lines not shown
    if (p->dw_queue.empty()) return 0;
    if (!p->staged && group != 2) return 0;
    if (p->staged && p->stage_groups == 2 && group == 0) return 0;
    return launch_dw_queue(p, s, group == 2);
}

static int launch_dw_slabs(dmvae_plan* p, hipStream_t target, bool with_prior) {
    const float* slab = WSf(p, p->o_dwslab);
    int64_t wlo = p->param_elems, whi = 0, blo = p->param_elems, bhi = 0;
    for (auto& a : p->dw_queue) {
        const int64_t w0 = reinterpret_cast<const float*>(a.epi.out) - slab;
        wlo = std::min(wlo, w0);
        whi = std::max(whi, w0 + (int64_t)a.M * a.epi.ldo);
        if (a.epi.out2) {
            const int64_t b0 = reinterpret_cast<const float*>(a.epi.out2) - slab;
            blo = std::min(blo, b0);
            bhi = std::max(bhi, b0 + (int64_t)a.N);
        }
    }
    const int64_t lo = std::min(wlo, blo), hi = std::max(whi, bhi);
    const int rc = gemm_bf16_grouped_dw(target, p->dw_queue.data(), (int)p->dw_queue.size());
    p->dw_queue.clear();
    if (rc) return rc;
    if (p->fused_update) {
        DMVAE_REQUIRE(with_prior && lo == 0, "dW slabs: the fused step flushes ONE group holding every layer");
        AdamArgs a;
        a.n = p->param_elems; a.p = p->buf.param; a.g = p->buf.grad; a.m = p->buf.m; a.v = p->buf.v;
        a.pb = reinterpret_cast<bf16_t*>(p->buf.param_bf16);
        a.lr = 0.f; a.b1 = p->cfg.beta1; a.b2 = p->cfg.beta2; a.eps = p->cfg.adam_eps; a.gscale = 1.f;
        a.zero_grad = 0; a.ieee = p->cfg.adam_ieee;
        a.t_host = ~0ull;
        a.st = reinterpret_cast<const dmvae_state*>(p->buf.state);
        return adam_slabs_launch(target, a, slab, p->dw_slices_now, p->param_elems, hi, p->param_elems);
    }
    if (!p->staged || bhi <= blo || blo <= whi)
        return slab_reduce_launch(target, slab + lo, hi - lo, p->dw_slices_now, p->param_elems, p->buf.grad + lo);
    TRY(slab_reduce_launch(target, slab + wlo, whi - wlo, p->dw_slices_now, p->param_elems, p->buf.grad + wlo));
    return slab_reduce_launch(target, slab + blo, bhi - blo, p->dw_slices_now, p->param_elems, p->buf.grad + blo);
}

static int launch_dw_queue(dmvae_plan* p, hipStream_t target, bool with_prior) {
    if (p->dw_queue.empty()) return 0;
    if (p->dw_slices_now > 1) return launch_dw_slabs(p, target, with_prior);
    int rc;
    if (p->fused_update) {
        dmvae_adam_ctx c;
        memset(&c, 0, sizeof(c));
        c.param = p->buf.param; c.grad = p->buf.grad; c.m = p->buf.m; c.v = p->buf.v; c.param_bf16 = p->buf.param_bf16;
        c.state = p->buf.state; c.beta1 = p->cfg.beta1; c.beta2 = p->cfg.beta2; c.epsilon = p->cfg.adam_eps; c.grad_scale = 1.f;
        c.store_grad = 0;
        c.ieee = p->cfg.adam_ieee;
        c.seg_off = p->prior_off;
        c.seg_n = with_prior ? ((2 * (int64_t)p->cfg.n_classes * p->cfg.latent_dim + 3) & ~(int64_t)3) : 0;
        rc = gemm_bf16_grouped_dw_adam(target, p->dw_queue.data(), (int)p->dw_queue.size(), c);
    } else {
        rc = gemm_bf16_grouped_dw(target, p->dw_queue.data(), (int)p->dw_queue.size());
    }
    p->dw_queue.clear();
    return rc;
}

static int dx_dense(dmvae_plan* p, hipStream_t s, const PAct& dy, const PLayer& L, const PAct& y_fwd, const PAct& dx, GemmArgs* deferred = nullptr,
                    const GemmRiders* riders = nullptr) {
    DMVAE_REQUIRE(dy.cols == L.out_pad && y_fwd.cols == L.in_pad && dx.cols == L.in_pad, "dx_dense %s: views of %d -> %d / %d columns on a %d -> %d layer",
                  L.name.c_str(), dy.cols, y_fwd.cols, dx.cols, L.in_pad, L.out_pad);
    dmvae_epilogue e;
    memset(&e, 0, sizeof(e));
    e.kind = DMVAE_EPI_RELU_MASK; e.out = WS(p, dx); e.ldo = dx.ld; e.aux0 = WS(p, y_fwd); e.ld0 = y_fwd.ld;
    const int N = L.in_pad, K = L.out_pad, dt = p->cfg.dtype;
    const bool macro = !deferred && dx.cs >= 0 && dt == DMVAE_BF16 && gemm_bf16_256_ok(DMVAE_GEMM_DX, DMVAE_EPI_RELU_MASK, p->Bp, N, K, false);
    if (!riders && !macro) return gemm_plan(p, s, DMVAE_GEMM_DX, N, K, WS(p, dy), dy.ld, Wp(p, L.w_off), L.ldw, &e, deferred);
    GemmArgs a;
    TRY(gemm_checked(s, dt, DMVAE_GEMM_DX, p->Bp, N, K, WS(p, dy), dy.ld, Wp(p, L.w_off), L.ldw, &e, 1, &a));
    if (riders) return gemm_bf16_dispatch(s, DMVAE_GEMM_DX, a, 1, riders);
    a.csum_out = WSf(p, dx.cs); a.csum_ld = dx.ld;
    dx.mark_cs_live();
    return gemm_bf16_dispatch(s, DMVAE_GEMM_DX, a, 1);
}

static int conv_trunk_forward(dmvae_plan* p, hipStream_t s) {
    const int dt = p->cfg.dtype;
    const void* in = nullptr;
    for (size_t i = 0; i < p->conv.size(); ++i) {
        const PConv& L = p->conv[i];
        const int M = p->Bp * L.P * L.P;
        dmvae_epilogue e;
        memset(&e, 0, sizeof(e));
        e.kind = DMVAE_EPI_BIAS_RELU; e.out = rows0(p, L.o_act, L.P, L.cout_ld); e.ldo = L.cout_ld; e.bias = p->buf.param + L.b_off;
        e.n_valid = L.cout;
        if (i == 0) {
            TRY(conv_first_fwd_launch(s, dt, WS(p, p->a.x), p->Ip, L.hw, p->Bp, Wp(p, L.w_off), L.cout_np, p->buf.param + L.b_off, L.cout,
                                      rows0(p, L.o_act, L.P, L.cout_ld), L.cout_ld));
        } else {
            TRY(gemm_checked(s, dt, DMVAE_GEMM_FWD, M, L.cout_np, L.kdim, in, L.cin_ld, Wp(p, L.w_off), L.cout_np, &e, 1, nullptr, L.P, L.cin));
            TRY(zero_border_launch(s, dt, rows0(p, L.o_act, L.P, L.cout_ld), L.P, L.cout_ld, p->Bp));
        }
        in = rows0(p, L.o_act, L.P, L.cout_ld);
        if (L.pool) {
            const bool last = i + 1 == p->conv.size();
            const int Po = (L.hw + 1) / 2 + 2;
            void* out = last ? (void*)WS(p, L.o_pool) : (void*)rows0(p, L.o_pool, Po, L.cout_ld);
            TRY(maxpool2_fwd_launch(s, dt, in, L.hw, L.cout_ld, p->Bp, out, last ? 0 : 1));
            in = out;
        }
    }
    return 0;
// ... 99 lines not shown
    }
    return 0;
}

int dmvae::moe_stage(dmvae_plan* p, hipStream_t s, int n_valid, float inv_B, bool backward) {
    auto& M = p->moe;
    const dmvae_config& c = p->cfg;
    const bool fl = M.cfg.featLearn != 0;
    if (!fl) TRY(fwd_dense(p, s, XB(p), M.L, DMVAE_EPI_BIAS_F32, M.P));
    MoeHeadArgs a;
    memset(&a, 0, sizeof(a));
    a.B = n_valid; a.B_pad = p->Bp; a.E = M.cfg.n_experts; a.O = M.cfg.output_dim;
    a.featLearn = fl; a.classification = M.cfg.classification != 0; a.backward = backward; a.act_dtype = c.dtype;
    a.inv_B = inv_B;
    a.P = WSf(p, M.P); a.ldP = M.P.ld;
    a.logits = WSf(p, p->a.lg); a.ld_lg = p->a.lg.ld;
    a.Y = M.cfg.labels; a.n_rows = M.cfg.label_rows;
    a.perm = M.perm; a.first = M.first; a.batch = c.max_batch; a.st = reinterpret_cast<const dmvae_state*>(M.st);
    a.mean = WSf(p, p->a.mv); a.ld_mean = p->a.mv.ld; a.D = c.latent_dim; a.Dp = p->Dp;
    a.W = p->buf.param + M.L.w_off; a.ldW = M.L.ldw; a.bias = p->buf.param + M.L.b_off;
    a.inp_act = WS(p, M.inp); a.ld_inp = M.inp.ld;
    a.gmu = WSf(p, p->a.gmu); a.ld_g = p->a.gmu.ld;
    a.dP_act = WS(p, M.dP); a.ld_dP = M.dP.ld;
    a.dlogits_act = WS(p, p->a.dlg); a.ld_dl = p->a.dlg.ld;
    a.dq_ws = WSf(p, M.dq); a.ld_dq = M.dq.ld;
    a.pred = WSf(p, M.pred); a.ld_pred = M.pred.ld;
    a.partials = WSf(p, M.o_part);
    a.acc = WSf(p, M.acc);
    TRY(moe_head_launch(s, a));
    if (!backward) return 0;
    return grad_dense(p, s, fl ? M.inp : XB(p), M.dP, M.L);
}

struct Pass {
    hipStream_t s;
    int n_valid, stage;
    bool all;
    float inv_B, vae_inv_B;
    bool hl_fused;
    bool heads_big;
    dmvae_finalize_args fin;
    bool fin_rides, fin_in_dz, fin_in_out;
    GemmRiders rid_dz, rid_out;
    dmvae_latent_args la;
};

static void pick_dw_slices(dmvae_plan* p) {
    const bool macro = g_dw_macro && p->dw_slices_max >= 4 && 4 * p->dw_macro_tiles >= 160 && p->Bp >= 16384 && gemm_bf16_256_slice_ok(256, 256, p->Bp / 4);
    const int want = g_dw_slices > 0 ? g_dw_slices : macro ? 4 : (p->Bp >= 16384 ? 2 : 1);
    p->dw_slices_now = (p->dw_slices_max > 1 && want > 1 && p->Bp % (want * 64) == 0) ? std::min(want, p->dw_slices_max) : 1;
    p->dw_macro_now = g_dw_macro && p->dw_slices_now > 1;
}

static int pick_forms(dmvae_plan* p, Pass& ps) {
    const dmvae_config& c = p->cfg;
    const int dt = c.dtype;
    ps.vae_inv_B = (p->moe.on && !p->moe.cfg.lossVAE) ? 0.f : ps.inv_B;
    ps.hl_fused = dt == DMVAE_BF16 && !p->vade && heads_latent_ok(p->Bp, c.latent_dim, c.n_classes, p->Dp, p->Kp, p->Hp, c.mode, 16) && p->mv.ldw >= 2 * p->Dp && p->lg.ldw >= p->Kp;
    const int n_lblk = p->vade ? p->n_lblk : ps.hl_fused ? p->Bp / 16 : latent_nblocks(p->Bp, c.latent_dim, c.n_classes);
    const int n_pblk = p->lws_bytes ? 1 : n_lblk;
    DMVAE_REQUIRE(n_lblk <= p->n_lblk_cap, "dmvae_plan_forward_backward: the latent kernel would run %d blocks, the plan's partial-sum buffers hold %d", n_lblk, p->n_lblk_cap);
    ps.fin = step_finalize_args(WSf(p, p->o_rpart), p->n_rpart, WSf(p, p->o_lpart), n_lblk, ps.inv_B, p->buf.state, 1, c.beta1, c.beta2,
                                WSf(p, p->o_dprior), n_pblk, 2 * c.n_classes * c.latent_dim, p->buf.grad + p->prior_off);
    ps.heads_big = dt == DMVAE_BF16 && gemm_bf16_256_ok(DMVAE_GEMM_DX, DMVAE_EPI_RELU_MASK, p->Bp, p->Hp, 2 * p->Dp, false) &&
                   gemm_bf16_256_ok(DMVAE_GEMM_DX, DMVAE_EPI_RELU_MASK, p->Bp, p->Hp, p->Kp, false);
    return 0;
}

static void place_riders(dmvae_plan* p, Pass& ps) {
    const dmvae_config& c = p->cfg;
    const int dt = c.dtype;
    ps.fin_rides = ps.all && dt == DMVAE_BF16 && !ps.heads_big && !p->vade && g_fin_rides;
    ps.fin_in_dz = ps.fin_in_out = false;
    const int fin_lead = (ps.fin.nblocks + 7) & ~7;
    GemmArgs dz_shape{}, out_shape{};
    dz_shape.M = p->Bp; dz_shape.N = p->Dp; dz_shape.K = p->dec.empty() ? 64 : p->dec[0].out_pad; dz_shape.epi.kind = DMVAE_EPI_LATENT; dz_shape.k_split = dz_shape.K;
    out_shape.M = p->Bp; out_shape.N = p->dec.empty() ? 64 : p->dec.back().out_pad; out_shape.K = p->Ip; out_shape.epi.kind = DMVAE_EPI_RELU_MASK;
    const int dz_room = (dt == DMVAE_BF16 && !p->dec.empty()) ? gemm_bf16_riders_room(dz_shape, true) : -1;
    const int out_room = (dt == DMVAE_BF16 && !p->dec.empty()) ? gemm_bf16_riders_room(out_shape, false) : -1;
    if (ps.fin_rides && g_fin_rides == 3 && out_room >= fin_lead) ps.fin_in_out = true;
    if (ps.fin_rides && g_fin_rides == 1) ps.fin_in_dz = dz_room >= fin_lead && gemm_bf16_carries_finalize(dz_shape);
    if (ps.fin_rides && g_fin_rides == 1 && !ps.fin_in_dz && out_room >= fin_lead) ps.fin_in_out = true;
    if (p->pf.armed && (ps.all || ps.stage == 0)) {
        p->pf.gat = gather_args(DMVAE_BF16, p->pf.data, p->pf.n_rows, c.input_dim, p->pf.perm, p->pf.first, c.max_batch, p->pf.n_valid, p->Bp, WS(p, XB(p, 1)), p->Ip,
                                nullptr, p->Ip, p->Ip, p->pf.st);
        if (ps.fin_rides && g_fin_rides == 1 && g_pf_rides && dz_room >= 64 && out_room >= fin_lead) {
            ps.fin_in_dz = false; ps.fin_in_out = true;
            ps.rid_dz.gat = p->pf.gat;
            ps.rid_dz.gat_last = g_pf_rides != 2;
            ps.rid_dz.ngat = (g_pf_rides == 3 ? std::min(2 * dz_room, 512) : std::min(dz_room, 256)) & ~7;
        }
    }
    if (ps.fin_in_dz) { ps.rid_dz.fin = ps.fin; ps.rid_dz.nfin = fin_lead; }
    if (ps.fin_in_out) { ps.rid_out.fin = ps.fin; ps.rid_out.nfin = fin_lead; }
}

static void latent_args_of(const dmvae_plan* p, Pass& ps, const float* eps, int64_t ld_eps, const float* gumbel, int64_t ld_gumbel) {
    const dmvae_config& c = p->cfg;
    const auto& a = p->a;
    dmvae_latent_args& la = ps.la;
    memset(&la, 0, sizeof(la));
    latent_inputs(p, la, eps, ld_eps);
    latent_sample(p, la);
    la.B = ps.n_valid; la.mode = p->vade ? 2 : c.mode; la.act_dtype = c.dtype;
    la.kl_ratio = 1.f; la.temperature = c.temperature; la.inv_B = ps.vae_inv_B; la.noise_step = 0;
    la.logits = WSf(p, a.lg); la.ld_logits = a.lg.ld;
// ... 107 lines not shown
    const auto& a = p->a;
    const int ne = (int)p->enc.size();
    if (p->vade) {
        TRY(grad_dense(p, ps.s, a.enc[ne - 1], a.dmv, p->mv));
        TRY(dx_dense(p, ps.s, a.dmv, p->mv, a.enc[ne - 1], a.denc[ne - 1]));
        return flush_dw(p, ps.s, 1);
    }
    const PAct hz = a.hzc.sub(0, p->Hp), hc = a.hzc.sub(p->Hp, p->Hp);
    TRY(grad_dense(p, ps.s, hz, a.dmv, p->mv));
    TRY(grad_dense(p, ps.s, hc, a.dlg, p->lg));
    {
        GemmArgs q[2];
        const bool grp = p->cfg.dtype == DMVAE_BF16 && !ps.heads_big;
        const dmvae_finalize_args* fin = (ps.fin_rides && !ps.fin_in_dz && !ps.fin_in_out) ? &ps.fin : nullptr;
        TRY(dx_dense(p, ps.s, a.dmv, p->mv, hz, a.dhzc.sub(0, p->Hp), grp ? &q[0] : nullptr));
        TRY(dx_dense(p, ps.s, a.dlg, p->lg, hc, a.dhzc.sub(p->Hp, p->Hp), grp ? &q[1] : nullptr));
        if (grp && g_heads_dx_form == 2) {
            TRY(gemm_bf16_dispatch(ps.s, DMVAE_GEMM_DX, q[0], 1));
            TRY(gemm_bf16_grouped(ps.s, DMVAE_GEMM_DX, q + 1, 1, fin));
        } else if (grp) TRY(gemm_bf16_grouped(ps.s, DMVAE_GEMM_DX, q, 2, fin));
    }
    TRY(grad_dense(p, ps.s, a.enc[ne - 1], a.dhzc, p->zc));
    return flush_dw(p, ps.s, 1);
}

static int backward_trunk(dmvae_plan* p, Pass& ps) {
    const auto& a = p->a;
    const int ne = (int)p->enc.size();
    if (p->pf.armed) {
        const dmvae_gather_args& g = p->pf.gat;
        TRY(gather_launch(ps.s, DMVAE_BF16, g.data, g.n_rows, g.dim, g.perm, g.first, g.batch, g.n_valid, g.B_pad, g.out_act, g.ld_act, nullptr, g.ld_f32, g.cols_pad, g.st));
        p->pf.armed = false; p->pf.done = true;
    }
    if (!p->vade) TRY(dx_dense(p, ps.s, a.dhzc, p->zc, a.enc[ne - 1], a.denc[ne - 1]));
    for (int i = ne - 1; i >= 0; --i) {
        TRY(grad_dense(p, ps.s, i > 0 ? a.enc[i - 1] : trunk_input(p), a.denc[i], p->enc[i]));
        if (i > 0) TRY(dx_dense(p, ps.s, a.denc[i], p->enc[i], a.enc[i - 1], a.denc[i - 1]));
        else if (!p->conv.empty()) TRY(dx_dense(p, ps.s, a.denc[0], p->enc[0], a.cflat, a.dflat));
    }
    TRY(flush_dw(p, ps.s, 2));
    return p->conv.empty() ? 0 : conv_trunk_backward(p, ps.s);
}

static int forward_backward_impl(dmvae_plan* p, void* stream, int n_valid, const float* eps, int64_t ld_eps,
                                 const float* gumbel, int64_t ld_gumbel, float inv_B, int stage) {
    DMVAE_REQUIRE(p && p->bound, "dmvae_plan_forward_backward: plan not bound");
    DMVAE_REQUIRE(n_valid > 0 && n_valid <= p->cfg.max_batch, "dmvae_plan_forward_backward: n_valid=%d out of range", n_valid);
    DMVAE_REQUIRE(stage >= -1 && stage <= 2, "dmvae_plan_forward_backward_stage: stage %d (0, 1, 2)", stage);
    if (p->moe.on && stage >= 0) { set_error("dmvae_plan_forward_backward_stage: not with a MoE attachment (one rank)"); return DMVAE_EUNSUPPORTED; }
    Pass ps;
    ps.s = (hipStream_t)stream; ps.n_valid = n_valid; ps.stage = stage; ps.all = stage < 0; ps.inv_B = inv_B;
    p->staged = !ps.all;
    if (ps.all || stage == 0) pick_dw_slices(p);
    TRY(pick_forms(p, ps));
    place_riders(p, ps);
    latent_args_of(p, ps, eps, ld_eps, gumbel, ld_gumbel);
    if (ps.all || stage == 0) {
        TRY(forward_and_loss(p, ps));
        TRY(backward_decoder(p, ps));
    }
    if (ps.all || stage == 1) TRY(backward_heads(p, ps));
    if (ps.all || stage == 2) TRY(backward_trunk(p, ps));
    return 0;
}

extern "C" int dmvae_plan_forward_backward(dmvae_plan* p, void* stream, int n_valid, const float* eps, int64_t ld_eps,
                                           const float* gumbel, int64_t ld_gumbel, float inv_B) {
    return forward_backward_impl(p, stream, n_valid, eps, ld_eps, gumbel, ld_gumbel, inv_B, -1);
}
extern "C" int dmvae_plan_forward_backward_stage(dmvae_plan* p, void* stream, int stage, int n_valid, const float* eps, int64_t ld_eps,
                                                 const float* gumbel, int64_t ld_gumbel, float inv_B) {
    DMVAE_REQUIRE(stage >= 0 && stage <= 2, "dmvae_plan_forward_backward_stage: stage %d (0, 1, 2)", stage);
    return forward_backward_impl(p, stream, n_valid, eps, ld_eps, gumbel, ld_gumbel, inv_B, stage);
}

extern "C" int dmvae_plan_train_step(dmvae_plan* p, void* stream, int n_valid, const float* eps, int64_t ld_eps,
                                     const float* gumbel, int64_t ld_gumbel, float inv_B) {
    DMVAE_REQUIRE(p && p->bound, "dmvae_plan_train_step: plan not bound");
    if (p->cfg.dtype != DMVAE_BF16 || !p->conv.empty()) {
        TRY(dmvae_plan_forward_backward(p, stream, n_valid, eps, ld_eps, gumbel, ld_gumbel, inv_B));
        return dmvae_plan_update(p, stream, 1.f);
    }
    p->fused_update = true;
    const int rc = dmvae_plan_forward_backward(p, stream, n_valid, eps, ld_eps, gumbel, ld_gumbel, inv_B);
    p->fused_update = false;
    return rc;
}

extern "C" int dmvae_plan_update(dmvae_plan* p, void* stream, float grad_scale) {
    DMVAE_REQUIRE(p && p->bound, "dmvae_plan_update: plan not bound");
    return dmvae_plan_update_range(p, stream, grad_scale, 0, p->param_elems);
}
extern "C" int dmvae_plan_update_range(dmvae_plan* p, void* stream, float grad_scale, int64_t lo, int64_t hi) {
    DMVAE_REQUIRE(p && p->bound, "dmvae_plan_update_range: plan not bound");
    DMVAE_REQUIRE(lo >= 0 && hi > lo && hi <= p->buf.arena_elems && lo % 4 == 0 && hi % 4 == 0,
                  "dmvae_plan_update_range: [%lld, %lld) must be a 4-aligned range of the %lld-element arena", (long long)lo, (long long)hi, (long long)p->buf.arena_elems);
    AdamArgs a;
    a.n = hi - lo; a.p = p->buf.param + lo; a.g = p->buf.grad + lo; a.m = p->buf.m + lo; a.v = p->buf.v + lo;
    a.pb = p->cfg.dtype == DMVAE_BF16 ? reinterpret_cast<bf16_t*>(p->buf.param_bf16) + lo : nullptr;
    a.lr = 0.f; a.b1 = p->cfg.beta1; a.b2 = p->cfg.beta2; a.eps = p->cfg.adam_eps; a.gscale = grad_scale;
    a.zero_grad = 0;
    a.ieee = p->cfg.adam_ieee;
    a.t_host = ~0ull;
    a.st = reinterpret_cast<const dmvae_state*>(p->buf.state);
    return adam_launch((hipStream_t)stream, a);
}
// ... 1 lines not shown
```

### deep-mixture-vae_amd/dmvae_hip/_lib.py

```python
import ctypes as C
import os

import torch

_HERE = os.path.dirname(os.path.abspath(__file__))
LIB_PATH = os.environ.get("DMVAE_HIP_LIB") or os.path.join(_HERE, "libdmvae_hip.so")

ABI_VERSION = 5
F32, BF16 = 0, 1
EUNSUPPORTED = -2
ADAM_ZERO_GRAD, ADAM_IEEE, ADAM_SHADOW = 1, 2, 4
GEMM_FWD, GEMM_DX, GEMM_DW = 0, 1, 2
(EPI_BIAS_RELU, EPI_BIAS_F32, EPI_BIAS_RECON, EPI_RELU_MASK, EPI_LATENT,
 EPI_STORE_F32, EPI_ATOMIC_F32, EPI_BIAS_SIGMOID, EPI_ADAM) = range(9)
MAX_LAYERS = 8
TRUNK_MLP, TRUNK_CNN = 0, 1
MODEL_DMVAE, MODEL_VADE = 0, 1

EXPORTS = [
    "dmvae_gemm", "dmvae_gemm_partials", "dmvae_gemm_grouped_dw", "dmvae_gemm_grouped", "dmvae_gemm_grouped_dw_adam", "dmvae_plan_train_step", "dmvae_latent_ws_bytes", "dmvae_latent_nblocks_vade", "dmvae_latent_vade_ws_bytes",
    "dmvae_plan_forward_backward_stage", "dmvae_plan_grad_buckets", "dmvae_plan_set_stage_groups", "dmvae_plan_update_range",
"dmvae_latent_nblocks", "dmvae_latent_fwd", "dmvae_heads_latent_fwd", "dmvae_heads_latent_ok", "dmvae_heads_latent_kslice_floats",
    "dmvae_recon_fwd_bwd", "dmvae_recon_nblocks", "dmvae_colsum", "dmvae_loss_finalize",
    "dmvae_adam_tf", "dmvae_adam_finish", "dmvae_gather_rows", "dmvae_philox_normal",
    "dmvae_philox_gumbel", "dmvae_cast_f32_to_bf16", "dmvae_cast_bf16_to_f32",
    "dmvae_plan_create", "dmvae_plan_destroy", "dmvae_plan_sizes", "dmvae_plan_tensor",
    "dmvae_plan_bind", "dmvae_plan_load_batch", "dmvae_plan_load_batch_step", "dmvae_plan_prefetch_batch", "dmvae_plan_swap_batch", "dmvae_plan_forward_backward",
    "dmvae_plan_update", "dmvae_plan_encode", "dmvae_plan_decode", "dmvae_plan_view",
    "dmvae_plan_attach_moe", "dmvae_plan_moe_set_labels", "dmvae_plan_moe_predict",
    "dmvae_gmm_ws_bytes", "dmvae_gmm_fit", "dmvae_gmm_kmeans",
    "dmvae_gmm_seed_ws_bytes", "dmvae_gmm_seed", "dmvae_philox_uniform",
    "dmvae_confusion_add", "dmvae_plan_eval_clusters",
    "dmvae_plan_eval_loglik_ws_bytes", "dmvae_plan_eval_loglik",
    "dmvae_tsne_ws_bytes", "dmvae_tsne_joint_p", "dmvae_tsne_gradient", "dmvae_tsne_step", "dmvae_tsne_fit", "dmvae_tsne_p",
    "dmvae_argmax_labels", "dmvae_silhouette_ws_bytes", "dmvae_silhouette",
    "dmvae_mixture_logpdf_ws_bytes", "dmvae_mixture_logpdf_split", "dmvae_mixture_logpdf", "dmvae_posterior_sample", "dmvae_column_stats_ws_bytes",
    "dmvae_column_stats", "dmvae_sum_f64",
    "dmvae_knn_ws_bytes", "dmvae_knn", "dmvae_knn_vote", "dmvae_knn_ranks",
    "dmvae_prof_enable", "dmvae_prof_collect", "dmvae_debug_spin", "dmvae_debug_strip_fwd2", "dmvae_debug_stamps", "dmvae_debug_anatomy", "dmvae_debug_anatomy256", "dmvae_debug_set_tile", "dmvae_debug_set_knob", "dmvae_abi_version", "dmvae_last_error",
    "dmvae_debug_conv_first_fwd", "dmvae_debug_conv_first_dw", "dmvae_debug_zero_border", "dmvae_debug_maxpool2_fwd", "dmvae_debug_maxpool2_bwd_relu",
    "dmvae_debug_conv_wflip", "dmvae_debug_conv_gemm", "dmvae_debug_conv_dw",
    "dmvae_debug_step_finalize", "dmvae_debug_gemm_dx_riders", "dmvae_debug_gemm_grouped_fin",
]


class MoeConfig(C.Structure):
    _fields_ = [("n_experts", C.c_int32), ("output_dim", C.c_int32), ("featLearn", C.c_int32), ("classification", C.c_int32),
                ("lossVAE", C.c_int32), ("reserved", C.c_int32), ("labels", C.c_void_p), ("label_rows", C.c_int64)]


class GmmConfig(C.Structure):
    _fields_ = [("N", C.c_int32), ("D", C.c_int32), ("K", C.c_int32), ("n_init", C.c_int32), ("max_iter", C.c_int32),
                ("kmeans_iter", C.c_int32), ("tol", C.c_float), ("reg_covar", C.c_float), ("flags", C.c_int32)]


class GmmResult(C.Structure):
    _fields_ = [(n, C.c_void_p) for n in (
        "weights", "means", "covariances", "lower_bound", "n_iter", "converged", "best_restart", "lower_bounds", "n_iters",
        "convergeds", "all_weights", "all_means", "all_covariances", "centers", "labels", "kmeans_iters")]


class TsneConfig(C.Structure):
    _fields_ = [("N", C.c_int32), ("D", C.c_int32), ("perplexity", C.c_float), ("early_exaggeration", C.c_float), ("learning_rate", C.c_float),
                ("n_iter", C.c_int32), ("exaggeration_iters", C.c_int32), ("seed", C.c_uint64), ("flags", C.c_int32)]


class GmmSeedConfig(C.Structure):
    _fields_ = [("N", C.c_int32), ("D", C.c_int32), ("K", C.c_int32), ("n_init", C.c_int32), ("local_trials", C.c_int32),
                ("seed", C.c_uint64), ("flags", C.c_int32)]


class Epilogue(C.Structure):
    _fields_ = [
        ("kind", C.c_int32), ("m_valid", C.c_int32), ("n_valid", C.c_int32), ("d_off", C.c_int32),
        ("recon_kind", C.c_int32), ("scale", C.c_float),
        ("out", C.c_void_p), ("ldo", C.c_int64),
        ("out2", C.c_void_p), ("ldo2", C.c_int64),
        ("bias", C.c_void_p),
        ("aux0", C.c_void_p), ("ld0", C.c_int64),
        ("aux1", C.c_void_p), ("ld1", C.c_int64),
        ("aux2", C.c_void_p), ("ld2", C.c_int64),
        ("partials", C.c_void_p),
    ]


class GemmProblem(C.Structure):
    _fields_ = [("M", C.c_int32), ("N", C.c_int32), ("K", C.c_int32), ("reserved", C.c_int32),
                ("A", C.c_void_p), ("lda", C.c_int64), ("B", C.c_void_p), ("ldb", C.c_int64),
                ("epi", Epilogue)]


class AdamCtx(C.Structure):
    _fields_ = [("param", C.c_void_p), ("grad", C.c_void_p), ("m", C.c_void_p), ("v", C.c_void_p),
                ("param_bf16", C.c_void_p), ("state", C.c_void_p),
                ("beta1", C.c_float), ("beta2", C.c_float), ("epsilon", C.c_float), ("grad_scale", C.c_float),
# ... 82 lines not shown

class ProfRow(C.Structure):
    _fields_ = [("name", C.c_char * 48), ("launches", C.c_int64), ("total_ms", C.c_double),
                ("flops", C.c_double), ("bytes", C.c_double), ("kernel_ms", C.c_double), ("kernel_launches", C.c_int64)]


def _load():
    if not os.path.exists(LIB_PATH):
        raise ImportError(
            "libdmvae_hip.so not found at %s: build it with `python deep-mixture-vae_amd/build.py` "
            "(hipcc --offload-arch=gfx950).  There is no CPU fallback." % LIB_PATH)
    lib = C.CDLL(LIB_PATH)
    vp, i32, i64, u32, u64, f32 = C.c_void_p, C.c_int, C.c_int64, C.c_uint32, C.c_uint64, C.c_float
    P = C.POINTER
    sig = {
        "dmvae_gemm": [vp, i32, i32, i32, i32, i32, vp, i64, vp, i64, P(Epilogue), i32],
        "dmvae_gemm_partials": [i32, i32, i32],
        "dmvae_gemm_grouped_dw": [vp, i32, P(GemmProblem), i32],
        "dmvae_gemm_grouped": [vp, i32, i32, P(GemmProblem), i32],
        "dmvae_gemm_grouped_dw_adam": [vp, P(GemmProblem), i32, P(AdamCtx)],
        "dmvae_plan_train_step": [vp, vp, i32, vp, i64, vp, i64, f32],
        "dmvae_plan_forward_backward_stage": [vp, vp, i32, i32, vp, i64, vp, i64, f32],
        "dmvae_plan_grad_buckets": [vp, P(i64)],
        "dmvae_plan_set_stage_groups": [vp, i32],
        "dmvae_plan_update_range": [vp, vp, f32, i64, i64],
        "dmvae_latent_nblocks": [i32, i32, i32],
        "dmvae_latent_nblocks_vade": [i32],
        "dmvae_latent_ws_bytes": [i32, i32, i32, i32],
        "dmvae_latent_vade_ws_bytes": [i32, i32, i32, i32, P(C.c_int)],
        "dmvae_latent_fwd": [vp, P(LatentArgs)],
        "dmvae_heads_latent_fwd": [vp, P(HeadsArgs), P(LatentArgs)],
        "dmvae_heads_latent_ok": [i32, i32, i32, i32, i32, i32, i32],
        "dmvae_heads_latent_kslice_floats": [i32, i32, i32],
        "dmvae_recon_fwd_bwd": [vp, i32, i32, i32, i32, i32, i32, vp, i64, vp, i64, f32, vp, i64, vp],
        "dmvae_recon_nblocks": [i32, i32],
        "dmvae_colsum": [vp, i32, vp, i64, i32, i32, vp],
        "dmvae_loss_finalize": [vp, vp, i32, vp, i32, f32, vp],
        "dmvae_adam_tf": [vp, i64, vp, vp, vp, vp, vp, f32, f32, f32, f32, f32, i32, u64, vp],
        "dmvae_adam_finish": [vp, vp],
        "dmvae_gather_rows": [vp, i32, vp, i64, i32, vp, i64, i32, i32, i32, vp, i64, vp, i64, vp],
        "dmvae_philox_normal": [vp, vp, i64, u64, u64, u32],
        "dmvae_philox_gumbel": [vp, vp, i64, u64, u64, u32],
        "dmvae_cast_f32_to_bf16": [vp, vp, vp, i64],
        "dmvae_cast_bf16_to_f32": [vp, vp, vp, i64],
        "dmvae_plan_create": [P(Config), P(vp)],
        "dmvae_plan_destroy": [vp],
        "dmvae_plan_sizes": [vp, P(Sizes)],
        "dmvae_plan_tensor": [vp, i32, P(TensorInfo)],
        "dmvae_plan_bind": [vp, P(Buffers)],
        "dmvae_plan_load_batch": [vp, vp, vp, i64, vp, i64, i32, i32],
        "dmvae_plan_load_batch_step": [vp, vp, vp, i64, vp, i64, i32, i32],
        "dmvae_plan_prefetch_batch": [vp, vp, i64, vp, i64, i32, i32],
        "dmvae_plan_swap_batch": [vp],
        "dmvae_plan_forward_backward": [vp, vp, i32, vp, i64, vp, i64, f32],
        "dmvae_plan_update": [vp, vp, f32],
        "dmvae_plan_encode": [vp, vp, i32],
        "dmvae_plan_decode": [vp, vp, vp, i64, i32],
        "dmvae_plan_view": [vp, C.c_char_p, P(vp), P(i64), P(C.c_int32)],
        "dmvae_plan_attach_moe": [vp, P(MoeConfig)],
        "dmvae_plan_moe_set_labels": [vp, vp, i64],
        "dmvae_plan_moe_predict": [vp, vp, i32],
        "dmvae_gmm_ws_bytes": [P(GmmConfig)],
        "dmvae_gmm_fit": [vp, P(GmmConfig), vp, i64, vp, vp, vp, vp, i64, P(GmmResult)],
        "dmvae_gmm_kmeans": [vp, P(GmmConfig), vp, i64, vp, vp, i64, P(GmmResult)],
        "dmvae_gmm_seed_ws_bytes": [P(GmmSeedConfig)],
        "dmvae_gmm_seed": [vp, P(GmmSeedConfig), vp, i64, vp, vp, i64, vp, vp],
        "dmvae_philox_uniform": [vp, vp, i64, u64, u64, u32],
        "dmvae_confusion_add": [vp, vp, i64, i32, i32, vp, i64, vp, i64, vp, i32, vp],
        "dmvae_plan_eval_clusters": [vp, vp, i32, vp, i64, vp, i64, i32, vp, i64, u64, vp, i32, vp],
        "dmvae_plan_eval_loglik_ws_bytes": [vp],
        "dmvae_plan_eval_loglik": [vp, vp, i32, i64, i64, i32, vp, i64, u64, vp, i64, vp, vp],
        "dmvae_tsne_ws_bytes": [P(TsneConfig)],
        "dmvae_tsne_joint_p": [vp, P(TsneConfig), vp, i64, vp, i64, vp],
        "dmvae_tsne_gradient": [vp, P(TsneConfig), vp, i64, vp, f32, vp],
        "dmvae_tsne_step": [vp, P(TsneConfig), vp, i64, vp, vp, vp, f32, f32],
        "dmvae_tsne_fit": [vp, P(TsneConfig), vp, i64, vp, vp, i64, vp, vp],
        "dmvae_tsne_p": [vp],
        "dmvae_argmax_labels": [vp, vp, i64, i32, i32, vp],
        "dmvae_silhouette_ws_bytes": [i64, i32],
        "dmvae_silhouette": [vp, vp, i64, i32, i32, vp, i32, vp, i64, vp, vp, vp],
        "dmvae_mixture_logpdf_ws_bytes": [i64, i64, i64],
        "dmvae_mixture_logpdf_split": [i32, i32, i32],
        "dmvae_mixture_logpdf": [vp, vp, i64, i32, i32, vp, i64, vp, i64, i32, vp, vp, i64, vp],
        "dmvae_posterior_sample": [vp, vp, i64, vp, i64, i32, i32, vp, i64, u64, u64, i64, vp, i64, vp],
        "dmvae_column_stats_ws_bytes": [i64, i64],
        "dmvae_column_stats": [vp, vp, i64, vp, i64, i32, i32, vp, i64, vp],
        "dmvae_sum_f64": [vp, vp, i64, vp],
        "dmvae_knn_ws_bytes": [i64, i64, i32, i32],
        "dmvae_knn": [vp, vp, i64, i32, vp, i64, i32, i32, i32, i64, vp, i64, vp, vp, i64],
        "dmvae_knn_vote": [vp, vp, i64, i32, i32, vp, i32, i32, vp, i64, vp],
        "dmvae_knn_ranks": [vp, vp, i64, i32, i32, vp, i64, i32, vp, i64, vp],
        "dmvae_prof_enable": [i32],
        "dmvae_debug_spin": [vp, i32],
        "dmvae_debug_strip_fwd2": [vp, i32, i32, vp, i64, vp, i64, vp, vp, i64, vp, vp, i64, vp, i64],
        "dmvae_debug_stamps": [P(vp)],
        "dmvae_debug_anatomy": [P(vp)],
        "dmvae_debug_anatomy256": [P(vp)],
        "dmvae_prof_collect": [P(ProfRow), i32],
        "dmvae_debug_set_tile": [i32, i32],
        "dmvae_debug_set_knob": [i32, i32],
        "dmvae_debug_conv_first_fwd": [vp, i32, vp, i64, i32, i64, vp, i32, vp, vp, i32],
        "dmvae_debug_conv_first_dw": [vp, i32, vp, i64, i32, i64, vp, i32, vp, i32, vp, vp, i64, P(C.c_int)],
        "dmvae_debug_zero_border": [vp, i32, vp, i32, i32, i64],
        "dmvae_debug_maxpool2_fwd": [vp, i32, vp, i32, i32, i64, vp, i32],
        "dmvae_debug_maxpool2_bwd_relu": [vp, i32, vp, vp, i32, i32, i64, vp, i32],
        "dmvae_debug_conv_wflip": [vp, i32, vp, i32, i32, i32, i32, vp, i32],
        "dmvae_debug_conv_gemm": [vp, i32, i32, i32, i32, i32, vp, i64, vp, i64, P(Epilogue), i32, i32, i32],
        "dmvae_debug_conv_dw": [vp, i32, i32, i32, i32, vp, i64, vp, i64, i32, i32, i32, vp, vp, vp],
        "dmvae_debug_step_finalize": [vp, P(DebugFinalize)],
        "dmvae_debug_gemm_dx_riders": [vp, i32, i32, i32, vp, i64, vp, i64, P(Epilogue), P(DebugFinalize), P(DebugGather), i32, i32],
        "dmvae_debug_gemm_grouped_fin": [vp, P(GemmProblem), i32, P(DebugFinalize)],
        "dmvae_abi_version": [],
        "dmvae_last_error": [],
    }
    for name, args in sig.items():
        fn = getattr(lib, name)
        fn.argtypes = args
        fn.restype = C.c_int
    lib.dmvae_last_error.restype = C.c_char_p
    lib.dmvae_latent_ws_bytes.restype = C.c_int64
    lib.dmvae_latent_vade_ws_bytes.restype = C.c_int64
    lib.dmvae_heads_latent_kslice_floats.restype = C.c_int64
    lib.dmvae_gmm_ws_bytes.restype = C.c_int64
    lib.dmvae_gmm_seed_ws_bytes.restype = C.c_int64
    lib.dmvae_plan_eval_loglik_ws_bytes.restype = C.c_int64
    lib.dmvae_tsne_ws_bytes.restype = C.c_int64
    lib.dmvae_tsne_p.restype = C.c_void_p
    lib.dmvae_silhouette_ws_bytes.restype = C.c_int64
    lib.dmvae_mixture_logpdf_ws_bytes.restype = C.c_int64
    lib.dmvae_column_stats_ws_bytes.restype = C.c_int64
    lib.dmvae_knn_ws_bytes.restype = C.c_int64
    lib.dmvae_plan_destroy.restype = None
    got = lib.dmvae_abi_version()
    if got != ABI_VERSION:
        raise ImportError("%s reports ABI version %d, this binding is written against %d (include/dmvae_hip.h): rebuild it with "
                          "`python deep-mixture-vae_amd/build.py`" % (LIB_PATH, got, ABI_VERSION))
    return lib


lib = _load()


class DmvaeError(RuntimeError):
    pass


def check(rc, what=""):
    if rc != 0:
        msg = lib.dmvae_last_error().decode("utf-8", "replace")
        raise DmvaeError("%s failed (code %d): %s" % (what or "dmvae call", rc, msg))


def ptr(t):
    return None if t is None else C.c_void_p(t.data_ptr())
```

### deep-mixture-vae_amd/dmvae_hip/runtime.py

```python
import ctypes as C
import math
import os

import numpy as np
import torch

from . import _lib
from ._lib import lib, check, ptr


def _require_gpu():
    if not torch.cuda.is_available():
        raise RuntimeError(
            "dmvae_hip needs an AMD GPU (gfx950): torch.cuda.is_available() is False. "
            "There is no CPU execution path in this package.")


class Session:

    def __init__(self, device=None):
        _require_gpu()
        self.rank = int(os.environ.get("RANK", "0"))
        self.world_size = int(os.environ.get("WORLD_SIZE", "1"))
        self.local_rank = int(os.environ.get("LOCAL_RANK", "0"))
# ... 93 lines not shown
        cfg.n_dec = len(self.dec_layers)
        for i, v in enumerate(self.dec_layers):
            cfg.dec[i] = int(v)
        cfg.input_type = {"binary": 0, "real": 1}[input_type]
        cfg.dtype = self.dtype
        cfg.max_batch = self.max_batch
        cfg.mode = self.mode
        cfg.temperature = float(temperature)
        cfg.beta1, cfg.beta2, cfg.adam_eps = float(beta1), float(beta2), float(adam_eps)
        cfg.seed = int(seed) & 0xFFFFFFFFFFFFFFFF
        cfg.deterministic = 1 if deterministic else 0
        cfg.trunk = _lib.TRUNK_CNN if self.cnn else _lib.TRUNK_MLP
        cfg.model = _lib.MODEL_VADE if model == "vade" else _lib.MODEL_DMVAE
        self.adam_ieee = bool(adam_ieee)
        cfg.adam_ieee = 1 if adam_ieee else 0
        self._cfg = cfg
        h = C.c_void_p()
        check(lib.dmvae_plan_create(C.byref(cfg), C.byref(h)), "dmvae_plan_create")
        self._plan = h
        self.moe = None
        if moe is not None:
            labels = moe["labels"]
            assert labels.dtype == torch.float32 and labels.is_contiguous() and labels.dim() == 2 and labels.shape[1] == int(moe["output_dim"])
            mc = _lib.MoeConfig()
            mc.n_experts, mc.output_dim = int(moe["n_experts"]), int(moe["output_dim"])
            mc.featLearn, mc.classification, mc.lossVAE = int(bool(moe["featLearn"])), int(bool(moe["classification"])), int(bool(moe["lossVAE"]))
            mc.labels, mc.label_rows = labels.data_ptr(), labels.shape[0]
            check(lib.dmvae_plan_attach_moe(self._plan, C.byref(mc)), "dmvae_plan_attach_moe")
            self.moe = dict(moe)
            self._moe_labels = labels
        sz = _lib.Sizes()
        check(lib.dmvae_plan_sizes(self._plan, C.byref(sz)), "dmvae_plan_sizes")
        self.sizes = sz
        self.batch_pad, self.input_pad = sz.batch_pad, sz.input_pad
        gran = 64 * max(1, self.session.world_size)
        n = (sz.param_elems + gran - 1) // gran * gran
        self.param = torch.zeros(n, dtype=torch.float32, device=dev)
        self.grad = torch.zeros(n, dtype=torch.float32, device=dev)
        self.m = torch.zeros(n, dtype=torch.float32, device=dev)
        self.v = torch.zeros(n, dtype=torch.float32, device=dev)
        self.param_bf16 = torch.zeros(n, dtype=torch.bfloat16, device=dev) if self.dtype == _lib.BF16 else None
        self.work = torch.zeros(sz.work_bytes, dtype=torch.uint8, device=dev)
        self.state_t = torch.zeros(C.sizeof(_lib.State), dtype=torch.uint8, device=dev)
        b = _lib.Buffers(ptr(self.param), ptr(self.grad), ptr(self.m), ptr(self.v),
                         ptr(self.param_bf16), ptr(self.work), ptr(self.state_t), n)
        check(lib.dmvae_plan_bind(self._plan, C.byref(b)), "dmvae_plan_bind")
        self.tensors = {}
        for i in range(sz.n_tensors):
            ti = _lib.TensorInfo()
            check(lib.dmvae_plan_tensor(self._plan, i, C.byref(ti)), "dmvae_plan_tensor")
            self.tensors[ti.name.decode()] = (ti.offset, ti.rows, ti.cols, ti.ld)
        self.write_state(kl_ratio=1.0, lr=0.002, epoch_weight=1.0, batches_per_epoch=0)
        self._graph = None
        self._pf_primed = False
        self._xsel = 0

    def __del__(self):
        try:
            if getattr(self, "_plan", None):
                lib.dmvae_plan_destroy(self._plan)
                self._plan = None
        except Exception:
            pass

    def _strided(self, arena, name):
        off, rows, cols, ld = self.tensors[name]
        if name.startswith("b_"):
            return torch.as_strided(arena, (cols,), (1,), off)
        return torch.as_strided(arena, (rows, cols), (ld, 1), off)

    def param_view(self, name):
        return self._strided(self.param, name)

    def grad_view(self, name):
        return self._strided(self.grad, name)

    def parameter_names(self):
        return list(self.tensors.keys())

    def _to_host(self, view, name):
        return view.detach().cpu().numpy().copy()

    def _require_current_master(self, what):
        if getattr(self, "_master_stale", False):
            raise RuntimeError("%s: the fp32 master weights are stale outside this rank's slice after sharded data-parallel steps; "
                               "call StepEngine.sync_master(exchange) on EVERY rank first (it is a collective)" % what)

    def get_parameters(self):
        self._require_current_master("get_parameters")
        return {k: self._to_host(self.param_view(k), k) for k in self.tensors}

    def get_gradients(self):
        return {k: self._to_host(self.grad_view(k), k) for k in self.tensors}

    def set_parameters(self, params):
        if set(self.tensors) <= set(params):
            self._master_stale = False
        self._require_current_master("set_parameters (it re-derives the whole bf16 shadow from the fp32 arena)")
        for k, v in params.items():
            dst = self.param_view(k)
            dst.copy_(torch.as_tensor(np.asarray(v, dtype=np.float32)).to(self.device).reshape(dst.shape))
        self.refresh_shadow()

    def init_parameters(self, seed=0):
        rng = np.random.RandomState(seed)
        p = {}
# ... 12 lines not shown
                p["b_" + name] = np.zeros((fo,))
            else:
                lb = math.sqrt(6.0 / (1 + fo))
                p["b_" + name] = rng.uniform(-lb, lb, size=(fo,))
        p["prior_means"] = rng.randn(self.n_classes, self.latent_dim)
        p["prior_log_vars"] = np.zeros((self.n_classes, self.latent_dim))
        if self.moe is not None:
            E, O = int(self.moe["n_experts"]), int(self.moe["output_dim"])
            w = rng.randn(E, O, self.latent_dim if self.moe["featLearn"] else self.input_dim)
            p["W_moe"] = w.transpose(2, 0, 1).reshape(w.shape[2], E * O)
            p["b_moe"] = np.zeros((E * O,))
        self.param.zero_()
        self.m.zero_()
        self.v.zero_()
        self._moments_sharded = False
        self.grad.zero_()
        self.set_parameters(p)
        st = self.read_state()
        self.write_state(adam_t=0, noise_step=0, kl_ratio=st.kl_ratio, lr=st.lr)

    def moe_acc(self):
        return self._moe_acc_view().cpu().numpy().astype(np.float64)

    def _moe_acc_view(self):
        p, ld, dt = C.c_void_p(), C.c_int64(), C.c_int32()
        check(lib.dmvae_plan_view(self._plan, b"moe_acc", C.byref(p), C.byref(ld), C.byref(dt)), "dmvae_plan_view")
        off = p.value - self.work.data_ptr()
        return self.work[off: off + 16].view(torch.float32)

    def moe_zero_acc(self):
        self._moe_acc_view().zero_()

    def moe_set_labels(self, labels):
        assert labels.dtype == torch.float32 and labels.is_contiguous() and labels.shape[1] == int(self.moe["output_dim"])
        self._moe_labels = labels
        check(lib.dmvae_plan_moe_set_labels(self._plan, ptr(labels), labels.shape[0]), "dmvae_plan_moe_set_labels")

    def moe_predict(self, n_valid=None):
        n_valid = self.max_batch if n_valid is None else int(n_valid)
        check(lib.dmvae_plan_moe_predict(self._plan, self._stream(), n_valid), "dmvae_plan_moe_predict")

    def moe_reference_parameters(self):
        E, O = int(self.moe["n_experts"]), int(self.moe["output_dim"])
        w = self._to_host(self.param_view("W_moe"), "W_moe")
        b = self._to_host(self.param_view("b_moe"), "b_moe")
        return w.reshape(w.shape[0], E, O).transpose(1, 2, 0).copy(), b.reshape(E, O).T.copy()

    def refresh_shadow(self):
        self._require_current_master("refresh_shadow")
        if self.param_bf16 is not None:
            check(lib.dmvae_cast_f32_to_bf16(self._stream(), ptr(self.param), ptr(self.param_bf16),
                                             self.param.numel()), "dmvae_cast_f32_to_bf16")

    def read_state(self):
        raw = self.state_t.cpu().numpy().tobytes()
        return _lib.State.from_buffer_copy(raw)

    def write_state(self, **kw):
        st = self.read_state() if kw.pop("_merge", True) else _lib.State()
        for k, v in kw.items():
            setattr(st, k, v)
        host = torch.frombuffer(bytearray(bytes(st)), dtype=torch.uint8)
        self.state_t.copy_(host)
        self._pf_primed = False

    def reset_optimizer(self, lr=None):
        self.m.zero_()
        self.v.zero_()
        self._moments_sharded = False
        kw = dict(adam_t=0, lr_t=0.0)
        if lr is not None:
            kw["lr"] = float(lr)
        self.write_state(**kw)

    def reset_epoch(self, batches_per_epoch, kl_ratio=None, epoch_weight=None):
        kw = dict(batch_cursor=0, batches_per_epoch=int(batches_per_epoch), epoch_loss=0.0, epoch_recon=0.0,
                  epoch_klz=0.0, epoch_klc=0.0,
                  epoch_weight=float(epoch_weight if epoch_weight is not None else 1.0 / max(1, batches_per_epoch)))
        if kl_ratio is not None:
            kw["kl_ratio"] = float(kl_ratio)
        self.write_state(**kw)

    def _stream(self):
        return C.c_void_p(torch.cuda.current_stream(self.device).cuda_stream)

    def load_batch(self, data, perm=None, first=0, n_valid=None, use_state_cursor=False):
        assert data.dtype == torch.float32 and data.is_contiguous() and data.shape[1] == self.input_dim
        assert perm is None or (perm.dtype == torch.int32 and perm.is_contiguous())
        n_valid = self.max_batch if n_valid is None else int(n_valid)
        self._pf_primed = False
        if self.moe is not None:
            self._batch_src = (data, perm)
        check(lib.dmvae_plan_load_batch(self._plan, self._stream(), ptr(data), data.shape[0], ptr(perm),
                                        int(first), n_valid, 1 if use_state_cursor else 0), "dmvae_plan_load_batch")

    def _load_batch_for_step(self, data, perm=None, first=0, n_valid=None, use_state_cursor=False):
        assert data.dtype == torch.float32 and data.is_contiguous() and data.shape[1] == self.input_dim
        assert perm is None or (perm.dtype == torch.int32 and perm.is_contiguous())
        n_valid = self.max_batch if n_valid is None else int(n_valid)
        self._step_src = (data, perm)
        self._pf_primed = False
        check(lib.dmvae_plan_load_batch_step(self._plan, self._stream(), ptr(data), data.shape[0], ptr(perm),
                                             int(first), n_valid, 1 if use_state_cursor else 0), "dmvae_plan_load_batch_step")

    def forward_backward(self, n_valid=None, eps=None, gumbel=None, inv_B=None):
        n_valid = self.max_batch if n_valid is None else int(n_valid)
        if eps is not None:
            assert eps.dtype == torch.float32 and eps.is_contiguous() and eps.shape == (n_valid, self.latent_dim)
        if gumbel is not None:
# ... 240 lines not shown
                     "weights": self.n_classes, "eval_w": self.n_classes, "recon": self.input_dim, "x": self.input_dim,
                     "moe_pred": self.moe["output_dim"] if self.moe else 0,
                     "moe_P": self.moe["n_experts"] * self.moe["output_dim"] if self.moe else 0,
                     "moe_dP": self.moe["n_experts"] * self.moe["output_dim"] if self.moe else 0,
                     "dlogits": self.n_classes, "gmu": self.latent_dim,
                     "Z": self.latent_dim, "dxlogits": self.input_dim}.get(name, ld.value)
        return t[: (self.max_batch if rows is None else rows), : (full_cols if cols is None else cols)]

    def hidden_activations(self, rows=None):
        out = {}
        if self.model == "vade":
            if self.cnn:
                for name, _, _, _, _ in CONV_STACK:
                    out[name] = self.view(name, rows)
            for i, w in enumerate(self.enc_layers):
                out["enc%d" % i] = self.view("enc%d" % i, rows, w)
            for i, w in enumerate(self.dec_layers):
                out["dec%d" % i] = self.view("dec%d" % i, rows, w)
            return out
        hp = self.view("hzc", rows).shape[1] // 2
        if self.cnn:
            for i, (name, _, co, hw, _) in enumerate(CONV_STACK):
                out[name] = self.view(name, rows)
        for i, w in enumerate(self.enc_layers):
            out["enc%d" % i] = self.view("enc%d" % i, rows, w)
        hzc = self.view("hzc", rows)
        out["zh"] = hzc[:, : self.head_dim]
        out["ch"] = hzc[:, hp: hp + self.head_dim]
        for i, w in enumerate(self.dec_layers):
            out["dec%d" % i] = self.view("dec%d" % i, rows, w)
        return out

    def train_step(self, data, perm, n_valid=None, eps=None, gumbel=None, first=0, use_state_cursor=False,
                   grad_sync=None, grad_scale=1.0, inv_B=None, fused=None):
        self._load_batch_for_step(data, perm, first, n_valid, use_state_cursor)
        if fused is None:
            fused = grad_sync is None and float(grad_scale) == 1.0
        if fused:
            assert grad_sync is None and float(grad_scale) == 1.0
            self.forward_backward_update(n_valid, eps, gumbel, inv_B)
            return
        if grad_sync is not None:
            self._step_with_exchange(grad_sync, grad_scale, n_valid, eps, gumbel, inv_B)
            return
        self.forward_backward(n_valid, eps, gumbel, inv_B)
        self.update(grad_scale)

    def _prefetch_batch(self, data, perm, first=0, n_valid=None, use_state_cursor=True):
        n_valid = self.max_batch if n_valid is None else int(n_valid)
        self._step_src = (data, perm)
        check(lib.dmvae_plan_prefetch_batch(self._plan, ptr(data), data.shape[0], ptr(perm), int(first), n_valid, 1 if use_state_cursor else 0),
              "dmvae_plan_prefetch_batch")

    def _prefetch_ok(self, data, perm, side):
        if self.dtype != _lib.BF16:
            return False
        with torch.cuda.stream(side):
            self._load_batch_for_step(data, perm, 0, None, True)
        side.synchronize()
        rc = lib.dmvae_plan_prefetch_batch(self._plan, ptr(data), data.shape[0], ptr(perm), 0, self.max_batch, 1)
        if rc == _lib.EUNSUPPORTED:
            return False
        check(rc, "dmvae_plan_prefetch_batch")
        return True

    def capture_step(self, data, perm, grad_sync=None, grad_scale=1.0, inv_B=None, pipelined=None):
        side = torch.cuda.Stream(device=self.device)
        side.wait_stream(torch.cuda.current_stream(self.device))
        saved = (self.param.clone(), self.m.clone(), self.v.clone(), self.state_t.clone(), getattr(self, "_moments_sharded", False))
        with torch.cuda.stream(side):
            for _ in range(2):
                self.train_step(data, perm, None, None, None, 0, True, grad_sync, grad_scale, inv_B)
        torch.cuda.current_stream(self.device).wait_stream(side)
        torch.cuda.synchronize(self.device)
        self.param.copy_(saved[0]); self.m.copy_(saved[1]); self.v.copy_(saved[2]); self.state_t.copy_(saved[3])
        self.grad.zero_()
        self._master_stale = False
        self._moments_sharded = saved[4]
        self.refresh_shadow()
        torch.cuda.synchronize(self.device)
        if pipelined is None:
            env = os.environ.get("DMVAE_PREFETCH", "")
            pipelined = env == "1" if env in ("0", "1") else self.max_batch <= PIPELINE_MAX_BATCH
        if grad_sync is None and pipelined and float(grad_scale) == 1.0 and self._prefetch_ok(data, perm, side):
            graphs = []
            for _ in range(2):
                g = torch.cuda.CUDAGraph()
                with torch.cuda.graph(g, stream=side):
                    self._prefetch_batch(data, perm)
                    self.forward_backward_update(None, None, None, inv_B)
                check(lib.dmvae_plan_swap_batch(self._plan), "dmvae_plan_swap_batch")
                graphs.append(g)
            self._graph = tuple(graphs)
            self._pf_primed, self._xsel = True, 0

            def replay_pipelined():
                if not self._pf_primed:
                    self._load_batch_for_step(data, perm, 0, None, True)
                    self._pf_primed, self._xsel = True, 0
                graphs[self._xsel].replay()
                self._xsel ^= 1
            return replay_pipelined
        if grad_sync is None:
            g = torch.cuda.CUDAGraph()
            with torch.cuda.graph(g, stream=side):
                self.train_step(data, perm, None, None, None, 0, True, None, grad_scale, inv_B)
            self._graph = (g,)

            def replay():
                self._pf_primed = False
                g.replay()
            return replay
        def eager_step():
            self.train_step(data, perm, None, None, None, 0, True, grad_sync, grad_scale, inv_B)
        self._graph = None
        return eager_step


def latent_eval(mean, log_var, logits, prior_means, prior_log_vars, eps=None, gumbel=None, mode="exact",
                temperature=1.0, kl_ratio=1.0, session=None):
    sess = session or default_session()
    dev = sess.device
    f = lambda a: torch.as_tensor(np.ascontiguousarray(np.asarray(a, dtype=np.float32))).to(dev)
    mean = np.asarray(mean, dtype=np.float32)
    logits = np.asarray(logits, dtype=np.float32)
    B, D = mean.shape
    K = logits.shape[1]
    Bp = (B + 63) // 64 * 64
    ldD, ldK = (D + 63) // 64 * 64, (K + 63) // 64 * 64

    def padded(a, ld):
        t = torch.zeros((Bp, ld), dtype=torch.float32, device=dev)
        a = f(a)
        t[: a.shape[0], : a.shape[1]] = a
        return t
    md, lvd, lgd = padded(mean, ldD), padded(log_var, ldD), padded(logits, ldK)
    epsd = f(eps) if eps is not None else torch.zeros((B, D), dtype=torch.float32, device=dev)
    gd = f(np.asarray(gumbel).reshape(B, K)) if gumbel is not None else torch.zeros((B, K), dtype=torch.float32, device=dev)
    pmd, plvd = f(prior_means), f(prior_log_vars)
    Z = torch.zeros((Bp, ldD), dtype=torch.float32, device=dev)
    w = torch.zeros((Bp, K), dtype=torch.float32, device=dev)
    gmu, glv, clv = (torch.zeros((Bp, ldD), dtype=torch.float32, device=dev) for _ in range(3))
    dlg = torch.zeros((Bp, ldK), dtype=torch.float32, device=dev)
    nblk = lib.dmvae_latent_nblocks_vade(Bp) if mode == "vade" else lib.dmvae_latent_nblocks(Bp, D, K)
    dpri = torch.zeros((nblk, 2 * K * D), dtype=torch.float32, device=dev)
    lp = torch.zeros((nblk, 2), dtype=torch.float32, device=dev)
    a = _lib.LatentArgs()
    a.B, a.B_pad, a.D, a.K = B, Bp, D, K
    a.mode, a.act_dtype = {"exact": 0, "relaxed": 1, "vade": 2}[mode], _lib.F32
    a.kl_ratio, a.temperature, a.inv_B = float(kl_ratio), float(temperature), 1.0 / B
    a.mean, a.ld_mean = md.data_ptr(), ldD
    a.log_var, a.ld_log_var = lvd.data_ptr(), ldD
    a.logits, a.ld_logits = lgd.data_ptr(), ldK
    a.eps, a.ld_eps = epsd.data_ptr(), D
    a.gumbel, a.ld_gumbel = gd.data_ptr(), K
# ... 32 lines not shown
```

### include/dmvae_hip.h

```cpp
#ifndef DMVAE_HIP_H
#define DMVAE_HIP_H

#include <stddef.h>
#include <stdint.h>

#ifdef __cplusplus
extern "C" {
#endif

#define DMVAE_ABI_VERSION 5

enum { DMVAE_F32 = 0, DMVAE_BF16 = 1 };

enum {
    DMVAE_EINVAL = -1,
    DMVAE_EUNSUPPORTED = -2,
    DMVAE_ESTATE = -3
};

enum { DMVAE_GEMM_FWD = 0, DMVAE_GEMM_DX = 1, DMVAE_GEMM_DW = 2 };

enum {
    DMVAE_EPI_BIAS_RELU = 0,
    DMVAE_EPI_BIAS_F32 = 1,
// ... 157 lines not shown
    int32_t n_dec; int32_t dec[DMVAE_MAX_LAYERS];
    int32_t input_type;
    int32_t dtype;
    int32_t max_batch;
    int32_t mode;
    float temperature;
    float beta1, beta2, adam_eps;
    uint64_t seed;
    int32_t deterministic;
    int32_t trunk;
    int32_t model;
    int32_t adam_ieee;
} dmvae_config;

typedef struct dmvae_tensor_info {
    char name[32];
    int64_t offset;
    int32_t rows, cols;
    int64_t ld;
} dmvae_tensor_info;

typedef struct dmvae_sizes {
    int64_t param_elems;
    int64_t work_bytes;
    int32_t batch_pad;
    int32_t input_pad;
    int32_t n_tensors;
    int32_t reserved;
} dmvae_sizes;

typedef struct dmvae_buffers {
    float* param; float* grad; float* m; float* v;
    void* param_bf16;
    void* work;
    void* state;
    int64_t arena_elems;
} dmvae_buffers;

typedef struct dmvae_plan dmvae_plan;

int dmvae_plan_create(const dmvae_config* cfg, dmvae_plan** out);
void dmvae_plan_destroy(dmvae_plan* p);
int dmvae_plan_sizes(const dmvae_plan* p, dmvae_sizes* out);
int dmvae_plan_tensor(const dmvae_plan* p, int index, dmvae_tensor_info* out);
int dmvae_plan_bind(dmvae_plan* p, const dmvae_buffers* b);

int dmvae_plan_load_batch(dmvae_plan* p, void* stream, const float* data, int64_t n_rows,
                          const int32_t* perm, int64_t first, int n_valid, int use_state_cursor);
int dmvae_plan_load_batch_step(dmvae_plan* plan, void* stream, const float* data, int64_t n_rows, const int32_t* perm,
                               int64_t first, int n_valid, int use_state_cursor);
int dmvae_plan_prefetch_batch(dmvae_plan* plan, const float* data, int64_t n_rows, const int32_t* perm, int64_t first, int n_valid,
                              int use_state_cursor);
int dmvae_plan_swap_batch(dmvae_plan* plan);
int dmvae_plan_forward_backward(dmvae_plan* p, void* stream, int n_valid,
                                const float* eps, int64_t ld_eps, const float* gumbel, int64_t ld_gumbel,
                                float inv_B);
int dmvae_plan_forward_backward_stage(dmvae_plan* p, void* stream, int stage, int n_valid,
                                      const float* eps, int64_t ld_eps, const float* gumbel, int64_t ld_gumbel,
                                      float inv_B);
int dmvae_plan_grad_buckets(const dmvae_plan* p, int64_t bounds[5]);
int dmvae_plan_set_stage_groups(dmvae_plan* p, int n_groups);
int dmvae_plan_update(dmvae_plan* p, void* stream, float grad_scale);
int dmvae_plan_update_range(dmvae_plan* p, void* stream, float grad_scale, int64_t lo, int64_t hi);
int dmvae_plan_train_step(dmvae_plan* p, void* stream, int n_valid,
                          const float* eps, int64_t ld_eps, const float* gumbel, int64_t ld_gumbel,
                          float inv_B);
int dmvae_plan_encode(dmvae_plan* p, void* stream, int n_valid);
int dmvae_plan_decode(dmvae_plan* p, void* stream, const float* Z, int64_t ldz, int n_valid);
int dmvae_plan_view(const dmvae_plan* p, const char* name, void** ptr, int64_t* ld, int32_t* dtype);

typedef struct dmvae_moe_config {
    int32_t n_experts;
    int32_t output_dim;
    int32_t featLearn;
    int32_t classification;
    int32_t lossVAE;
    int32_t reserved;
    const float* labels;
    int64_t label_rows;
} dmvae_moe_config;
int dmvae_plan_attach_moe(dmvae_plan* p, const dmvae_moe_config* cfg);
int dmvae_plan_moe_set_labels(dmvae_plan* p, const float* labels, int64_t label_rows);
int dmvae_plan_moe_predict(dmvae_plan* p, void* stream, int n_valid);

typedef struct dmvae_gmm_config {
    int32_t N, D, K;
    int32_t n_init;
    int32_t max_iter;
    int32_t kmeans_iter;
    float tol;
    float reg_covar;
    int32_t flags;
} dmvae_gmm_config;
typedef struct dmvae_gmm_result {
    float* weights;
    float* means;
    float* covariances;
    double* lower_bound;
    int32_t* n_iter;
    int32_t* converged;
    int32_t* best_restart;
    double* lower_bounds;
    int32_t* n_iters;
    int32_t* convergeds;
    float* all_weights;
    float* all_means;
// ... 83 lines not shown
```

### include/dmvae_hip_debug.h

```cpp
#ifndef DMVAE_HIP_DEBUG_H
#define DMVAE_HIP_DEBUG_H

#include "dmvae_hip.h"

#ifdef __cplusplus
extern "C" {
#endif

typedef struct dmvae_prof_row {
    char name[48];
    int64_t launches;
    double total_ms;
    double flops;
    double bytes;
    double kernel_ms;
    int64_t kernel_launches;
} dmvae_prof_row;
int dmvae_prof_enable(int on);
int dmvae_debug_spin(void* stream, int microseconds);
int dmvae_prof_collect(dmvae_prof_row* rows, int max_rows);
int dmvae_debug_strip_fwd2(void* stream, int B_pad, int K0, const void* X, int64_t ldx, const void* W0, int64_t ld0, const float* b0,
                           const void* W1, int64_t ld1, const float* b1, void* Y1, int64_t ldy1, void* Y2, int64_t ldy2);
int dmvae_debug_stamps(void** device_ptr);
int dmvae_debug_anatomy(void** device_ptr);
int dmvae_debug_anatomy256(void** device_ptr);
int dmvae_debug_set_tile(int bm, int bn);
int dmvae_debug_set_knob(int which, int value);

int dmvae_debug_conv_first_fwd(void* stream, int dtype, const void* x, int64_t bstride, int H, int64_t n_img, const void* W, int ldw,
                               const float* bias, void* out, int ld);
int dmvae_debug_conv_first_dw(void* stream, int dtype, const void* x, int64_t bstride, int H, int64_t n_img, const void* dY, int ld,
                              float* dW, int ldw, float* db, float* part, int64_t part_floats, int* n_blocks);
int dmvae_debug_zero_border(void* stream, int dtype, void* a, int P, int ld, int64_t n_img);
int dmvae_debug_maxpool2_fwd(void* stream, int dtype, const void* in, int H, int ld, int64_t n_img, void* out, int out_border);
int dmvae_debug_maxpool2_bwd_relu(void* stream, int dtype, const void* in, const void* dout, int H, int ld, int64_t n_img, void* din, int dout_border);
int dmvae_debug_conv_wflip(void* stream, int dtype, const void* W, int cin, int cin_ld, int cout, int ldw, void* Wt, int Kt);
int dmvae_debug_conv_gemm(void* stream, int dtype, int layout, int M, int N, int K, const void* A, int64_t lda,
                          const void* B, int64_t ldb, const dmvae_epilogue* epi, int split_k, int conv_p, int conv_c);
int dmvae_debug_conv_dw(void* stream, int dtype, int rows, int conv_p, int conv_c, const void* X, int64_t ldx, const void* dY, int64_t ldy,
                        int N, int n_valid, int split, float* slab, float* dW, float* db);

typedef struct dmvae_debug_finalize {
    const float* rp; int nr;
    const float* lp; int nl;
    float inv_B; void* state; int bump_adam;
    float b1, b2;
    const float* part; int nblk, ncol;
    float* gout;
} dmvae_debug_finalize;
typedef struct dmvae_debug_gather {
    const float* data; int64_t n_rows; int dim;
    const int32_t* perm; int64_t first;
    int batch, n_valid, B_pad;
    void* out_bf16; int64_t ld;
    const void* state;
} dmvae_debug_gather;
int dmvae_debug_step_finalize(void* stream, const dmvae_debug_finalize* fin);
int dmvae_debug_gemm_dx_riders(void* stream, int M, int N, int K, const void* A, int64_t lda, const void* B, int64_t ldb, const dmvae_epilogue* epi,
                               const dmvae_debug_finalize* fin, const dmvae_debug_gather* gat, int ngat, int gat_last);
int dmvae_debug_gemm_grouped_fin(void* stream, const dmvae_gemm_problem* probs, int n, const dmvae_debug_finalize* fin);

#ifdef __cplusplus
}
#endif
#endif
```

Before: 14.52 million images/sec.

## Gather next batch in tail rider blocks of the dW+Adam grouped launch

Adds rider workgroups at the end of the grouped weight-gradient+Adam launch. They wait on an atomic arrival counter until every tile reading the batch buffer has finished its K-loop, then gather the next batch's rows into that buffer, which removes the separate gather launch and overlaps it with the dW epilogues. Tiles that read the batch are sorted earlier, and a bounded poll sets a sticky error word if the wait times out. The cost is spin-waiting blocks occupying CUs, plus a risk of a race or timeout if the readers are not all resident.

```diff
diff --git a/deep-mixture-vae_amd/csrc/api.hip b/deep-mixture-vae_amd/csrc/api.hip
--- a/deep-mixture-vae_amd/csrc/api.hip
+++ b/deep-mixture-vae_amd/csrc/api.hip
@@ -437,6 +437,25 @@
         TRY(gemm_checked(s, DMVAE_BF16, DMVAE_GEMM_DX, pr.M, pr.N, pr.K, pr.A, pr.lda, pr.B, pr.ldb, &pr.epi, 1, &q[i]));
     }
     return gemm_bf16_grouped(s, DMVAE_GEMM_DX, q.data(), n, &f);
+}
+
+extern "C" int dmvae_debug_gemm_grouped_dw_adam_gather(void* stream, const dmvae_gemm_problem* probs, int n, const dmvae_adam_ctx* ctx,
+                                                       const dmvae_debug_gather* gat, int ngat, int32_t* sync) {
+    DMVAE_REQUIRE(probs && ctx && gat && sync && n >= 1 && n <= DMVAE_MAX_GROUP, "dmvae_debug_gemm_grouped_dw_adam_gather: 1..%d problems, a context, a gather and its sync words", DMVAE_MAX_GROUP);
+    DMVAE_REQUIRE(gat->data && gat->out_bf16 && gat->n_rows >= 0 && gat->dim > 0 && gat->ld % 4 == 0 && gat->ld >= gat->dim,
+                  "dmvae_debug_gemm_grouped_dw_adam_gather: gather arguments (ld a multiple of 4, >= dim)");
+    hipStream_t s = (hipStream_t)stream;
+    std::vector<GemmArgs> q(n);
+    for (int i = 0; i < n; ++i) {
+        const dmvae_gemm_problem& pr = probs[i];
+        TRY(gemm_checked(s, DMVAE_BF16, DMVAE_GEMM_DW, pr.M, pr.N, pr.K, pr.A, pr.lda, pr.B, pr.ldb, &pr.epi, 1, &q[i]));
+    }
+    GatherTail t;
+    t.gat = gather_args(DMVAE_BF16, gat->data, gat->n_rows, gat->dim, gat->perm, gat->first, gat->batch, gat->n_valid, gat->B_pad, gat->out_bf16, gat->ld,
+                        nullptr, gat->ld, (int)gat->ld, gat->state);
+    t.ngat = ngat;
+    t.sync = sync;
+    return gemm_bf16_grouped_dw_adam(s, q.data(), n, *ctx, &t);
 }
 
 extern "C" int dmvae_prof_enable(int on) {
diff --git a/deep-mixture-vae_amd/csrc/gemm_bf16.hip b/deep-mixture-vae_amd/csrc/gemm_bf16.hip
--- a/deep-mixture-vae_amd/csrc/gemm_bf16.hip
+++ b/deep-mixture-vae_amd/csrc/gemm_bf16.hip
@@ -261,6 +261,9 @@
     }
     wait_vmcnt<0>();
     __builtin_amdgcn_s_barrier();
+    if constexpr (DW && EPI == DMVAE_EPI_ADAM && !CONV) {
+        if (a.arrive != nullptr && tid == 0) __hip_atomic_fetch_add(a.arrive, 1, __ATOMIC_RELAXED, __HIP_MEMORY_SCOPE_AGENT);
+    }
     MEAS_KLOOP_END();
     MEAS_ANAT(2);
 
@@ -498,11 +501,43 @@
     dmvae_finalize_args fin;
     int lead, lead_work;
     int xcut, xr0[8], xcnt[8];
+    GatherTail tail;
+    int tail_need;
 };
+__device__ __forceinline__ void gather_tail_rider(const GatherTail& t, const int need, const int rid, const int nthreads, int* flag) {
+    if (need > 0) {
+        if (threadIdx.x == 0) {
+            int ok = 0, polls = 0;
+            for (; polls < GATHER_TAIL_POLLS; ++polls) {
+                if (__hip_atomic_load(t.sync, __ATOMIC_RELAXED, __HIP_MEMORY_SCOPE_AGENT) == need) { ok = 1; break; }
+                __builtin_amdgcn_s_sleep(32);
+            }
+            if (!ok) __hip_atomic_store(t.sync + 2, 1, __ATOMIC_RELAXED, __HIP_MEMORY_SCOPE_AGENT);
+            *flag = polls;
+        }
+        __syncthreads();
+        MEAS_TAIL_WAITED(rid, *flag);
+    }
+    if constexpr (!MEAS_EMPTY_GATHER_RIDERS) gather_rows_block<bf16_t, 16>(rid, nthreads, t.gat);
+    if (need > 0 && threadIdx.x == 0) {
+        if (__hip_atomic_fetch_add(t.sync + 1, 1, __ATOMIC_RELAXED, __HIP_MEMORY_SCOPE_AGENT) == t.ngat - 1) {
+            __hip_atomic_store(t.sync, 0, __ATOMIC_RELAXED, __HIP_MEMORY_SCOPE_AGENT);
+            __hip_atomic_store(t.sync + 1, 0, __ATOMIC_RELAXED, __HIP_MEMORY_SCOPE_AGENT);
+        }
+    }
+}
 template <int BM, int BN, int LAYOUT, int EPI, int NSTAGE, int NW = 4, bool SHORTK = false>
 __global__ __launch_bounds__(64 * NW, NW == 8 ? 4 : 1) void gemm_bf16_grouped_kernel(GroupedArgs g) {
     __shared__ __attribute__((aligned(16))) bf16_t smem[SHORTK ? 2 * (64 + 64) * BK : 3 * (128 + 64) * BK];
     const dmvae_adam_ctx* ac = EPI == DMVAE_EPI_ADAM ? &g.adam : nullptr;
+    if constexpr (EPI == DMVAE_EPI_ADAM && LAYOUT == DMVAE_GEMM_DW) {
+        if ((int)blockIdx.x >= (int)gridDim.x - g.tail.ngat) {
+            MEAS_WG_BEGIN();
+            gather_tail_rider(g.tail, g.tail_need, (int)blockIdx.x - ((int)gridDim.x - g.tail.ngat), 64 * NW, reinterpret_cast<int*>(smem));
+            MEAS_WG_END(LAYOUT, 7);
+            return;
+        }
+    }
     if constexpr (EPI == DMVAE_EPI_ADAM) {
         if ((int)blockIdx.x < g.lead) {
             if ((int)blockIdx.x >= g.lead_work) return;
@@ -635,7 +670,15 @@
 }
 
 template <int LAYOUT, int EPI>
-static int grouped_launch(hipStream_t s, const GemmArgs* probs, int nprob, const dmvae_adam_ctx* ctx = nullptr, const dmvae_finalize_args* fin = nullptr) {
+static int grouped_launch(hipStream_t s, const GemmArgs* probs, int nprob, const dmvae_adam_ctx* ctx = nullptr, const dmvae_finalize_args* fin = nullptr,
+                          const GatherTail* tail = nullptr) {
+    auto reads_tail = [&](const GemmArgs& p) {
+        if (!tail) return false;
+        const char* lo = reinterpret_cast<const char*>(tail->gat.out_act);
+        const char* hi = lo + (int64_t)tail->gat.B_pad * tail->gat.ld_act * 2;
+        auto in = [&](const void* q) { return reinterpret_cast<const char*>(q) >= lo && reinterpret_cast<const char*>(q) < hi; };
+        return (!p.bias_only && in(p.A)) || in(p.B);
+    };
     auto best_kind = [](const GemmArgs& p) { return p.bias_only ? 3 : (p.M % 128 == 0 && p.N % 128 == 0) ? 0 : (p.M % 128 == 0 ? 1 : 2); };
     auto nslices = [](const GemmArgs& p) { return (p.k_split > 0 && p.k_split < p.K) ? p.K / p.k_split : 1; };
     auto tiles = [&](const GemmArgs& p, int kind) {
@@ -685,9 +728,16 @@
     }
     int order[DMVAE_MAX_GROUP];
     for (int i = 0; i < nprob; ++i) order[i] = i;
-    std::stable_sort(order, order + nprob, [&](int x, int y) { return wg_bytes(probs[x], kinds[x]) > wg_bytes(probs[y], kinds[y]); });
+    std::stable_sort(order, order + nprob, [&](int x, int y) {
+        const double bx = wg_bytes(probs[x], kinds[x]), by = wg_bytes(probs[y], kinds[y]);
+        if (bx != by || !tail) return bx > by;
+        if (kinds[x] != kinds[y]) return kinds[x] < kinds[y];
+        return reads_tail(probs[x]) && !reads_tail(probs[y]);
+    });
     GroupedArgs g;
     g.nprob = nprob;
+    g.tail = GatherTail{};
+    g.tail_need = 0;
     int total = 0, n = 0;
     double flops = 0.0, bytes = 0.0;
     for (int o = 0; o < nprob; ++o) {
@@ -760,6 +810,17 @@
         bytes += elems * (24.0 + (ctx->param_bf16 ? 2.0 : 0.0) + (ctx->store_grad ? 4.0 : 0.0)) + 4.0 * ctx->seg_n;
         if (ctx->seg_n > 0) { g.lead_work = (int)std::min<int64_t>(4, (ctx->seg_n / 4 + 255) / 256); g.lead = 8; extra = g.lead; }
     }
+    int riders = 0;
+    if constexpr (LAYOUT == DMVAE_GEMM_DW && EPI == DMVAE_EPI_ADAM) {
+        if (tail) {
+            g.tail = *tail;
+            g.tail.gat.nblocks = tail->ngat;
+            for (int i = 0; i < nprob; ++i)
+                if (reads_tail(g.p[i])) { g.p[i].arrive = tail->sync; g.tail_need += g.start[i + 1] - g.start[i]; }
+            riders = tail->ngat;
+            bytes += (double)tail->gat.n_valid * tail->gat.dim * 4.0 + (double)tail->gat.B_pad * tail->gat.cols_pad * 2.0;
+        }
+    }
     static const std::string pname = [] {
         char b[64];
         snprintf(b, sizeof(b), "gemm_bf16_grouped_mixed_tiles<L%d, E%d>", LAYOUT, EPI);
@@ -778,7 +839,7 @@
             return check_launch("gemm_bf16_grouped");
         }
     }
-    DMVAE_LAUNCH((gemm_bf16_grouped_kernel<64, 64, LAYOUT, EPI, 4, 4>), dim3(grid_items + extra), dim3(256), 0, s, g);
+    DMVAE_LAUNCH((gemm_bf16_grouped_kernel<64, 64, LAYOUT, EPI, 4, 4>), dim3(grid_items + extra + riders), dim3(256), 0, s, g);
     return check_launch("gemm_bf16_grouped");
 }
 
@@ -806,8 +867,7 @@
     set_error("dmvae_gemm_grouped: layout %d with epilogue %d is not instantiated", layout, epi);
     return DMVAE_EUNSUPPORTED;
 }
-static int peel_large_dw(hipStream_t s, const GemmArgs* probs, int nprob, const dmvae_adam_ctx* ctx, std::vector<GemmArgs>& rest) {
-    std::vector<GemmArgs> large;
+static void split_large_dw(const GemmArgs* probs, int nprob, std::vector<GemmArgs>& large, std::vector<GemmArgs>& rest) {
     bool any = false;
     for (int i = 0; i < nprob; ++i)
         any = any || (probs[i].k_split == probs[i].K && gemm_bf16_256_ok(DMVAE_GEMM_DW, probs[i].epi.kind, probs[i].M, probs[i].N, probs[i].K, probs[i].conv_c != 0));
@@ -820,7 +880,19 @@
         if (own || rides) large.push_back(p);
         else rest.push_back(p);
     }
+}
+static int peel_large_dw(hipStream_t s, const GemmArgs* probs, int nprob, const dmvae_adam_ctx* ctx, std::vector<GemmArgs>& rest) {
+    std::vector<GemmArgs> large;
+    split_large_dw(probs, nprob, large, rest);
     return large.empty() ? 0 : gemm_bf16_256_dw_all(s, large.data(), (int)large.size(), ctx);
+}
+bool gemm_bf16_grouped_dw_whole(const GemmArgs* probs, int nprob) {
+    if (nprob < 1 || nprob > DMVAE_MAX_GROUP) return false;
+    std::vector<GemmArgs> large, rest;
+    split_large_dw(probs, nprob, large, rest);
+    for (int i = 0; i < nprob; ++i)
+        if (probs[i].k_split != probs[i].K || probs[i].bias_only) return false;
+    return large.empty();
 }
 int gemm_bf16_grouped_dw(hipStream_t s, const GemmArgs* probs, int nprob) {
     if (nprob < 1 || nprob > DMVAE_MAX_GROUP) { set_error("dmvae_gemm_grouped_dw: 1..%d problems", DMVAE_MAX_GROUP); return DMVAE_EINVAL; }
@@ -831,8 +903,20 @@
     if (rc) return rc;
     return rest.empty() ? 0 : gemm_bf16_grouped(s, DMVAE_GEMM_DW, rest.data(), (int)rest.size(), nullptr);
 }
-int gemm_bf16_grouped_dw_adam(hipStream_t s, const GemmArgs* probs, int nprob, const dmvae_adam_ctx& ctx) {
+int gemm_bf16_grouped_dw_adam(hipStream_t s, const GemmArgs* probs, int nprob, const dmvae_adam_ctx& ctx, const GatherTail* tail) {
     if (nprob < 1 || nprob > DMVAE_MAX_GROUP) { set_error("dmvae_gemm_grouped_dw_adam: 1..%d problems", DMVAE_MAX_GROUP); return DMVAE_EINVAL; }
+    if (tail) {
+        const dmvae_gather_args& t = tail->gat;
+        if (tail->ngat < 8 || tail->ngat > 512 || tail->ngat % 8 || !tail->sync || !t.data || !t.out_act || t.out_f32 || t.B_pad <= 0 || t.n_valid < 0 || t.n_valid > t.B_pad ||
+            t.cols_pad % 4 || t.cols_pad < t.dim || t.ld_act < t.cols_pad || (int64_t)t.B_pad * (t.cols_pad / 4) >= (int64_t(1) << 31) - int64_t(512) * 256 * 16) {
+            set_error("dmvae_gemm_grouped_dw_adam: gather riders: 8..512 of them in eights, a sync area, a bf16 destination only, n_valid <= B_pad, B_pad x cols within 32-bit quad indices");
+            return DMVAE_EINVAL;
+        }
+        if (!gemm_bf16_grouped_dw_whole(probs, nprob)) {
+            set_error("dmvae_gemm_grouped_dw_adam: gather riders go with the unsliced small-tile group only (a problem is K-sliced or takes the macro tile)");
+            return DMVAE_EUNSUPPORTED;
+        }
+    }
     for (int i = 0; i < nprob; ++i)
         if (probs[i].epi.kind != DMVAE_EPI_ADAM || !probs[i].epi.out) { set_error("dmvae_gemm_grouped_dw_adam: every problem needs epilogue kind ADAM and out = its gradient address"); return DMVAE_EINVAL; }
     if (!ctx.param || !ctx.grad || !ctx.m || !ctx.v || !ctx.state || (ctx.seg_off & 3) || (ctx.seg_n & 3) || ctx.seg_n < 0) {
@@ -848,7 +932,7 @@
     c1.seg_n = 0;
     const int rc = peel_large_dw(s, probs, nprob, &c1, rest);
     if (rc) return rc;
-    if (!rest.empty()) return grouped_launch<DMVAE_GEMM_DW, DMVAE_EPI_ADAM>(s, rest.data(), (int)rest.size(), &ctx);
+    if (!rest.empty()) return grouped_launch<DMVAE_GEMM_DW, DMVAE_EPI_ADAM>(s, rest.data(), (int)rest.size(), &ctx, nullptr, tail);
     if (ctx.seg_n > 0) {
         AdamArgs a;
         a.n = ctx.seg_n; a.p = ctx.param + ctx.seg_off; a.g = ctx.grad + ctx.seg_off; a.m = ctx.m + ctx.seg_off; a.v = ctx.v + ctx.seg_off;
diff --git a/deep-mixture-vae_amd/csrc/gemm_epilogue.h b/deep-mixture-vae_amd/csrc/gemm_epilogue.h
--- a/deep-mixture-vae_amd/csrc/gemm_epilogue.h
+++ b/deep-mixture-vae_amd/csrc/gemm_epilogue.h
@@ -17,6 +17,7 @@
     const float* csum_in = nullptr; int csum_rows = 0;
     int bias_only = 0;
     int* tick = nullptr;
+    int* arrive = nullptr;
 };
 
 __host__ __device__ __forceinline__ int64_t conv_tap_offset(int tap, int c0, int P, int64_t lda) {
@@ -131,6 +132,12 @@
     dmvae_gather_args gat; int ngat = 0;
     int gat_last = 0;
 };
+
+struct GatherTail {
+    dmvae_gather_args gat; int ngat = 0;
+    int* sync = nullptr;
+};
+constexpr int GATHER_TAIL_POLLS = 1 << 12;
 
 __device__ __forceinline__ void xent_sigmoid(float l, float x, float& xent, float& sig) {
     const float e = __expf(-fabsf(l));
diff --git a/deep-mixture-vae_amd/csrc/kernels.h b/deep-mixture-vae_amd/csrc/kernels.h
--- a/deep-mixture-vae_amd/csrc/kernels.h
+++ b/deep-mixture-vae_amd/csrc/kernels.h
@@ -71,7 +71,8 @@
 int loss_finalize_launch(hipStream_t s, const float* rp, int nr, const float* lp, int nl, float inv_B, void* st, int bump_adam);
 int step_finalize_launch(hipStream_t s, const float* rp, int nr, const float* lp, int nl, float inv_B, void* st, int bump_adam,
                          float b1, float b2, const float* part, int nblk, int ncol, float* gout);
-int gemm_bf16_grouped_dw_adam(hipStream_t s, const GemmArgs* probs, int nprob, const dmvae_adam_ctx& ctx);
+int gemm_bf16_grouped_dw_adam(hipStream_t s, const GemmArgs* probs, int nprob, const dmvae_adam_ctx& ctx, const GatherTail* tail = nullptr);
+bool gemm_bf16_grouped_dw_whole(const GemmArgs* probs, int nprob);
 dmvae_gather_args gather_args(int act_dtype, const float* data, int64_t n_rows, int dim, const int32_t* perm, int64_t first, int batch, int n_valid,
                               int B_pad, void* out_act, int64_t ld_act, float* out_f32, int64_t ld_f32, int cols_pad, const void* st);
 int gather_launch(hipStream_t s, int act_dtype, const float* data, int64_t n_rows, int dim, const int32_t* perm, int64_t first, int batch,
diff --git a/deep-mixture-vae_amd/csrc/measure.h b/deep-mixture-vae_amd/csrc/measure.h
--- a/deep-mixture-vae_amd/csrc/measure.h
+++ b/deep-mixture-vae_amd/csrc/measure.h
@@ -32,6 +32,13 @@
         if (threadIdx.x == 0 && blockIdx.x < 2048) g_anat[blockIdx.x * 8 + 5] = MEAS_HWID();          \
     } while (0)
 #define MEAS_WG_BEGIN() const unsigned long long meas_t0_ = __builtin_amdgcn_s_memrealtime()
+#define MEAS_TAIL_WAITED(rid, polls)                                                                  \
+    do {                                                                                              \
+        if (threadIdx.x == 0 && blockIdx.x < 2048) {                                                  \
+            g_mid[blockIdx.x] = __builtin_amdgcn_s_memrealtime();                                     \
+            g_anat[blockIdx.x * 8 + 6] = (unsigned long long)(polls);                                 \
+        }                                                                                             \
+    } while (0)
 #define MEAS_WG_END(layout, kind)                                                                                          \
     do {                                                                                                                   \
         if (threadIdx.x == 0 && blockIdx.x < 2048) {                                                                       \
@@ -65,6 +72,7 @@
 #define MEAS_KLOOP_END() do { } while (0)
 #define MEAS_ANAT_DRAIN() do { } while (0)
 #define MEAS_WG_BEGIN() do { } while (0)
+#define MEAS_TAIL_WAITED(rid, polls) do { } while (0)
 #define MEAS_WG_END(layout, kind) do { } while (0)
 #define MEAS_ANAT256(i) do { } while (0)
 #define MEAS_ANAT256_DRAIN() do { } while (0)
diff --git a/deep-mixture-vae_amd/csrc/plan.h b/deep-mixture-vae_amd/csrc/plan.h
--- a/deep-mixture-vae_amd/csrc/plan.h
+++ b/deep-mixture-vae_amd/csrc/plan.h
@@ -86,6 +86,7 @@
     bool tgt_gather = false;
     int xsel = 0;
     struct { const float* data; int64_t n_rows; const int32_t* perm; int64_t first; int n_valid; const void* st; bool armed, done; dmvae::dmvae_gather_args gat; } pf{};
+    struct { const float* data; int64_t n_rows; const int32_t* perm; int64_t first; int n_valid; const void* st; bool armed; int ngat; int* sync; } tg{};
     bool vade = false;
     struct {
         bool on = false;
diff --git a/deep-mixture-vae_amd/csrc/plan.hip b/deep-mixture-vae_amd/csrc/plan.hip
--- a/deep-mixture-vae_amd/csrc/plan.hip
+++ b/deep-mixture-vae_amd/csrc/plan.hip
@@ -229,7 +229,10 @@
     return 0;
 }
 
-extern "C" void dmvae_plan_destroy(dmvae_plan* p) { delete p; }
+extern "C" void dmvae_plan_destroy(dmvae_plan* p) {
+    if (p && p->tg.sync) (void)hipFree(p->tg.sync);
+    delete p;
+}
 
 extern "C" int dmvae_plan_sizes(const dmvae_plan* p, dmvae_sizes* o) {
     DMVAE_REQUIRE(p && o, "dmvae_plan_sizes: null argument");
diff --git a/deep-mixture-vae_amd/csrc/step.hip b/deep-mixture-vae_amd/csrc/step.hip
--- a/deep-mixture-vae_amd/csrc/step.hip
+++ b/deep-mixture-vae_amd/csrc/step.hip
@@ -12,15 +12,18 @@
 static int g_fin_rides = 1;
 static int g_heads_dx_form = 0;
 static int g_ksplit = 1;
+static int g_tail_gather = 1;
+constexpr int TAIL_GATHER_RIDERS = 256;
 bool dmvae::step_set_knob(int which, int value) {
     int* const k = which == 10 ? &g_dw_slices : which == 11 ? &g_dw_macro : which == 12 ? &g_heads_dx_form : which == 16 ? &g_fin_rides :
-                   which == 17 ? &g_pf_rides : which == 21 ? &g_ksplit : nullptr;
+                   which == 17 ? &g_pf_rides : which == 21 ? &g_ksplit : which == 23 ? &g_tail_gather : nullptr;
     if (k) *k = value;
     return k != nullptr;
 }
 
 static void batch_rows(dmvae_plan* p, const int32_t* perm, int64_t first, const void* st) {
     p->pf.armed = p->pf.done = false;
+    p->tg.armed = false;
     p->moe.perm = perm; p->moe.first = first; p->moe.st = st;
 }
 extern "C" int dmvae_plan_load_batch(dmvae_plan* p, void* stream, const float* data, int64_t n_rows, const int32_t* perm,
@@ -191,6 +194,20 @@
         c.ieee = p->cfg.adam_ieee;
         c.seg_off = p->prior_off;
         c.seg_n = with_prior ? ((2 * (int64_t)p->cfg.n_classes * p->cfg.latent_dim + 3) & ~(int64_t)3) : 0;
+        if (p->tg.armed && with_prior) {
+            GatherTail t;
+            t.gat = gather_args(DMVAE_BF16, p->tg.data, p->tg.n_rows, p->cfg.input_dim, p->tg.perm, p->tg.first, p->cfg.max_batch, p->tg.n_valid, p->Bp, WS(p, XB(p)), p->Ip,
+                                nullptr, p->Ip, p->Ip, p->tg.st);
+            t.ngat = p->tg.ngat;
+            t.sync = p->tg.sync;
+            rc = gemm_bf16_grouped_dw_adam(target, p->dw_queue.data(), (int)p->dw_queue.size(), c, &t);
+            p->tg.armed = false;
+            if (!rc) {
+                p->tsrc.data = p->tg.data; p->tsrc.n_rows = p->tg.n_rows; p->tsrc.perm = p->tg.perm; p->tsrc.first = p->tg.first; p->tsrc.n_valid = p->tg.n_valid;
+                p->tsrc.st = p->tg.st;
+                p->tsrc_valid = true; p->tsrc_used = false;
+            }
+        } else
         rc = gemm_bf16_grouped_dw_adam(target, p->dw_queue.data(), (int)p->dw_queue.size(), c);
     } else {
         rc = gemm_bf16_grouped_dw(target, p->dw_queue.data(), (int)p->dw_queue.size());
@@ -396,6 +413,58 @@
     p->dw_macro_now = g_dw_macro && p->dw_slices_now > 1;
 }
 
+static bool tail_gather_default(const dmvae_plan* p) { return p->Bp >= 4096; }
+
+extern "C" int dmvae_plan_tail_gather_batch(dmvae_plan* p, const float* data, int64_t n_rows, const int32_t* perm, int64_t first, int n_valid,
+                                            int use_state_cursor) {
+    DMVAE_REQUIRE(p && p->bound && data, "dmvae_plan_tail_gather_batch: plan not bound / null data");
+    DMVAE_REQUIRE(n_valid >= 0 && n_valid <= p->cfg.max_batch, "dmvae_plan_tail_gather_batch: n_valid=%d exceeds max_batch=%d", n_valid, p->cfg.max_batch);
+    p->tg.armed = false;
+    if (p->cfg.dtype != DMVAE_BF16 || !p->conv.empty() || p->moe.on || !p->tgt_gather) {
+        set_error("dmvae_plan_tail_gather_batch: bf16 plans with the MLP trunk, no MoE attachment, batches assembled by dmvae_plan_load_batch_step");
+        return DMVAE_EUNSUPPORTED;
+    }
+    if (g_tail_gather == 0 || (g_tail_gather == 1 && !tail_gather_default(p))) { set_error("dmvae_plan_tail_gather_batch: off for this plan (knob 23)"); return DMVAE_EUNSUPPORTED; }
+    DMVAE_REQUIRE(g_tail_gather == 1 || (g_tail_gather >= 8 && g_tail_gather <= 512 && g_tail_gather % 8 == 0), "dmvae_plan_tail_gather_batch: knob 23 = %d (0, 1, or 8 .. 512 riders in eights)", g_tail_gather);
+    pick_dw_slices(p);
+    std::vector<GemmArgs> q;
+    auto add = [&](const PLayer& L) { GemmArgs a{}; a.M = L.in_pad; a.N = L.out_pad; a.K = a.k_split = p->Bp; a.epi.kind = DMVAE_EPI_ADAM; q.push_back(a); };
+    for (auto& L : p->enc) add(L);
+    for (auto& L : p->dec) add(L);
+    if (!p->vade) { add(p->zc); add(p->lg); }
+    add(p->mv); add(p->out);
+    if (p->dw_slices_now > 1 || (int)q.size() > DMVAE_MAX_GROUP || !gemm_bf16_grouped_dw_whole(q.data(), (int)q.size())) {
+        set_error("dmvae_plan_tail_gather_batch: the weight-gradient group of this plan is K-sliced, takes the macro tile or goes out as more than one launch");
+        return DMVAE_EUNSUPPORTED;
+    }
+    DMVAE_REQUIRE(p->tsrc_valid && !p->tsrc_used, "dmvae_plan_tail_gather_batch: no current batch (dmvae_plan_load_batch_step first)");
+    DMVAE_REQUIRE(!p->pf.armed, "dmvae_plan_tail_gather_batch: a prefetch into the other batch buffer is armed (dmvae_plan_prefetch_batch): one or the other");
+    if (!p->tg.sync) {
+        void* d = nullptr;
+        if (hipMalloc(&d, 256) != hipSuccess || hipMemset(d, 0, 256) != hipSuccess) {
+            (void)hipGetLastError();
+            if (d) (void)hipFree(d);
+            set_error("dmvae_plan_tail_gather_batch: no device memory for the sync words (first call inside a stream capture?)");
+            return DMVAE_ESTATE;
+        }
+        p->tg.sync = reinterpret_cast<int*>(d);
+    }
+    p->tg.data = data; p->tg.n_rows = n_rows; p->tg.perm = perm; p->tg.first = first; p->tg.n_valid = n_valid;
+    p->tg.st = use_state_cursor ? p->buf.state : nullptr;
+    p->tg.ngat = g_tail_gather == 1 ? TAIL_GATHER_RIDERS : g_tail_gather;
+    p->tg.armed = true;
+    return 0;
+}
+extern "C" int dmvae_plan_tail_gather_status(dmvae_plan* p, void* stream, int32_t* out) {
+    DMVAE_REQUIRE(p && out, "dmvae_plan_tail_gather_status: null argument");
+    out[0] = out[1] = out[2] = out[3] = 0;
+    if (!p->tg.sync) return 0;
+    hipError_t e = hipMemcpyAsync(out, p->tg.sync, 16, hipMemcpyDeviceToHost, (hipStream_t)stream);
+    if (e == hipSuccess) e = hipStreamSynchronize((hipStream_t)stream);
+    DMVAE_REQUIRE(e == hipSuccess, "dmvae_plan_tail_gather_status: %s", hipGetErrorString(e));
+    return 0;
+}
+
 static int pick_forms(dmvae_plan* p, Pass& ps) {
     const dmvae_config& c = p->cfg;
     const int dt = c.dtype;
@@ -609,6 +678,11 @@
     ps.s = (hipStream_t)stream; ps.n_valid = n_valid; ps.stage = stage; ps.all = stage < 0; ps.inv_B = inv_B;
     p->staged = !ps.all;
     if (ps.all || stage == 0) pick_dw_slices(p);
+    if (p->tg.armed && !(ps.all && p->fused_update && p->dw_slices_now == 1)) {
+        p->tg.armed = false;
+        set_error("dmvae_plan_forward_backward: a tail gather is armed (dmvae_plan_tail_gather_batch) and this pass is not a whole fused step with an unsliced dW group");
+        return DMVAE_EUNSUPPORTED;
+    }
     TRY(pick_forms(p, ps));
     place_riders(p, ps);
     latent_args_of(p, ps, eps, ld_eps, gumbel, ld_gumbel);
diff --git a/deep-mixture-vae_amd/dmvae_hip/_lib.py b/deep-mixture-vae_amd/dmvae_hip/_lib.py
--- a/deep-mixture-vae_amd/dmvae_hip/_lib.py
+++ b/deep-mixture-vae_amd/dmvae_hip/_lib.py
@@ -25,7 +25,7 @@
     "dmvae_adam_tf", "dmvae_adam_finish", "dmvae_gather_rows", "dmvae_philox_normal",
     "dmvae_philox_gumbel", "dmvae_cast_f32_to_bf16", "dmvae_cast_bf16_to_f32",
     "dmvae_plan_create", "dmvae_plan_destroy", "dmvae_plan_sizes", "dmvae_plan_tensor",
-    "dmvae_plan_bind", "dmvae_plan_load_batch", "dmvae_plan_load_batch_step", "dmvae_plan_prefetch_batch", "dmvae_plan_swap_batch", "dmvae_plan_forward_backward",
+    "dmvae_plan_bind", "dmvae_plan_load_batch", "dmvae_plan_load_batch_step", "dmvae_plan_prefetch_batch", "dmvae_plan_swap_batch", "dmvae_plan_tail_gather_batch", "dmvae_plan_tail_gather_status", "dmvae_plan_forward_backward",
     "dmvae_plan_update", "dmvae_plan_encode", "dmvae_plan_decode", "dmvae_plan_view",
     "dmvae_plan_attach_moe", "dmvae_plan_moe_set_labels", "dmvae_plan_moe_predict",
     "dmvae_gmm_ws_bytes", "dmvae_gmm_fit", "dmvae_gmm_kmeans",
@@ -40,7 +40,7 @@
     "dmvae_prof_enable", "dmvae_prof_collect", "dmvae_debug_spin", "dmvae_debug_strip_fwd2", "dmvae_debug_stamps", "dmvae_debug_anatomy", "dmvae_debug_anatomy256", "dmvae_debug_set_tile", "dmvae_debug_set_knob", "dmvae_abi_version", "dmvae_last_error",
     "dmvae_debug_conv_first_fwd", "dmvae_debug_conv_first_dw", "dmvae_debug_zero_border", "dmvae_debug_maxpool2_fwd", "dmvae_debug_maxpool2_bwd_relu",
     "dmvae_debug_conv_wflip", "dmvae_debug_conv_gemm", "dmvae_debug_conv_dw",
-    "dmvae_debug_step_finalize", "dmvae_debug_gemm_dx_riders", "dmvae_debug_gemm_grouped_fin",
+    "dmvae_debug_step_finalize", "dmvae_debug_gemm_dx_riders", "dmvae_debug_gemm_grouped_fin", "dmvae_debug_gemm_grouped_dw_adam_gather",
 ]
 
 
@@ -229,6 +229,8 @@
         "dmvae_plan_load_batch_step": [vp, vp, vp, i64, vp, i64, i32, i32],
         "dmvae_plan_prefetch_batch": [vp, vp, i64, vp, i64, i32, i32],
         "dmvae_plan_swap_batch": [vp],
+        "dmvae_plan_tail_gather_batch": [vp, vp, i64, vp, i64, i32, i32],
+        "dmvae_plan_tail_gather_status": [vp, vp, P(C.c_int32)],
         "dmvae_plan_forward_backward": [vp, vp, i32, vp, i64, vp, i64, f32],
         "dmvae_plan_update": [vp, vp, f32],
         "dmvae_plan_encode": [vp, vp, i32],
@@ -287,6 +289,7 @@
         "dmvae_debug_step_finalize": [vp, P(DebugFinalize)],
         "dmvae_debug_gemm_dx_riders": [vp, i32, i32, i32, vp, i64, vp, i64, P(Epilogue), P(DebugFinalize), P(DebugGather), i32, i32],
         "dmvae_debug_gemm_grouped_fin": [vp, P(GemmProblem), i32, P(DebugFinalize)],
+        "dmvae_debug_gemm_grouped_dw_adam_gather": [vp, P(GemmProblem), i32, P(AdamCtx), P(DebugGather), i32, vp],
         "dmvae_abi_version": [],
         "dmvae_last_error": [],
     }
diff --git a/deep-mixture-vae_amd/dmvae_hip/runtime.py b/deep-mixture-vae_amd/dmvae_hip/runtime.py
--- a/deep-mixture-vae_amd/dmvae_hip/runtime.py
+++ b/deep-mixture-vae_amd/dmvae_hip/runtime.py
@@ -169,6 +169,7 @@
             self.tensors[ti.name.decode()] = (ti.offset, ti.rows, ti.cols, ti.ld)
         self.write_state(kl_ratio=1.0, lr=0.002, epoch_weight=1.0, batches_per_epoch=0)
         self._graph = None
+        self._tail_armed = False
         self._pf_primed = False
         self._xsel = 0
 
@@ -287,9 +288,28 @@
             check(lib.dmvae_cast_f32_to_bf16(self._stream(), ptr(self.param), ptr(self.param_bf16),
                                              self.param.numel()), "dmvae_cast_f32_to_bf16")
 
+    @property
+    def _pf_primed(self):
+        return self._pf_primed_
+
+    @_pf_primed.setter
+    def _pf_primed(self, v):
+        self._pf_primed_ = bool(v)
+        self._tail_primed = None
+
     def read_state(self):
         raw = self.state_t.cpu().numpy().tobytes()
+        if getattr(self, "_tail_armed", False):
+            self.tail_gather_status()
         return _lib.State.from_buffer_copy(raw)
+
+    def tail_gather_status(self):
+        w = (C.c_int32 * 4)()
+        check(lib.dmvae_plan_tail_gather_status(self._plan, self._stream(), w), "dmvae_plan_tail_gather_status")
+        if w[2]:
+            raise RuntimeError("tail gather: a rider of the weight-gradient launch gave up its bounded wait for the readers of the batch buffer "
+                               "(sticky error word %d): the batch may have been overwritten while it was still being read" % w[2])
+        return int(w[0]), int(w[1])
 
     def write_state(self, **kw):
         st = self.read_state() if kw.pop("_merge", True) else _lib.State()
@@ -636,6 +656,24 @@
         check(lib.dmvae_plan_prefetch_batch(self._plan, ptr(data), data.shape[0], ptr(perm), int(first), n_valid, 1 if use_state_cursor else 0),
               "dmvae_plan_prefetch_batch")
 
+    def _tail_gather_batch(self, data, perm, first=0, n_valid=None, use_state_cursor=True):
+        n_valid = self.max_batch if n_valid is None else int(n_valid)
+        self._step_src = (data, perm)
+        check(lib.dmvae_plan_tail_gather_batch(self._plan, ptr(data), data.shape[0], ptr(perm), int(first), n_valid, 1 if use_state_cursor else 0),
+              "dmvae_plan_tail_gather_batch")
+
+    def _tail_gather_ok(self, data, perm, side):
+        if self.dtype != _lib.BF16:
+            return False
+        with torch.cuda.stream(side):
+            self._load_batch_for_step(data, perm, 0, None, True)
+        side.synchronize()
+        rc = lib.dmvae_plan_tail_gather_batch(self._plan, ptr(data), data.shape[0], ptr(perm), 0, self.max_batch, 1)
+        if rc == _lib.EUNSUPPORTED:
+            return False
+        check(rc, "dmvae_plan_tail_gather_batch")
+        return True
+
     def _prefetch_ok(self, data, perm, side):
         if self.dtype != _lib.BF16:
             return False
@@ -685,6 +723,22 @@
                 graphs[self._xsel].replay()
                 self._xsel ^= 1
             return replay_pipelined
+        if grad_sync is None and float(grad_scale) == 1.0 and self._tail_gather_ok(data, perm, side):
+            g = torch.cuda.CUDAGraph()
+            with torch.cuda.graph(g, stream=side):
+                self._tail_gather_batch(data, perm)
+                self.forward_backward_update(None, None, None, inv_B)
+            self._graph = (g,)
+            self._tail_armed = True
+            self._tail_primed = g
+
+            def replay_tail():
+                if self._tail_primed is not g:
+                    self._load_batch_for_step(data, perm, 0, None, True)
+                g.replay()
+                self._pf_primed = False
+                self._tail_primed = g
+            return replay_tail
         if grad_sync is None:
             g = torch.cuda.CUDAGraph()
             with torch.cuda.graph(g, stream=side):
diff --git a/include/dmvae_hip.h b/include/dmvae_hip.h
--- a/include/dmvae_hip.h
+++ b/include/dmvae_hip.h
@@ -233,6 +233,9 @@
 int dmvae_plan_prefetch_batch(dmvae_plan* plan, const float* data, int64_t n_rows, const int32_t* perm, int64_t first, int n_valid,
                               int use_state_cursor);
 int dmvae_plan_swap_batch(dmvae_plan* plan);
+int dmvae_plan_tail_gather_batch(dmvae_plan* plan, const float* data, int64_t n_rows, const int32_t* perm, int64_t first, int n_valid,
+                                 int use_state_cursor);
+int dmvae_plan_tail_gather_status(dmvae_plan* plan, void* stream, int32_t* out);
 int dmvae_plan_forward_backward(dmvae_plan* p, void* stream, int n_valid,
                                 const float* eps, int64_t ld_eps, const float* gumbel, int64_t ld_gumbel,
                                 float inv_B);
diff --git a/include/dmvae_hip_debug.h b/include/dmvae_hip_debug.h
--- a/include/dmvae_hip_debug.h
+++ b/include/dmvae_hip_debug.h
@@ -59,6 +59,8 @@
 int dmvae_debug_gemm_dx_riders(void* stream, int M, int N, int K, const void* A, int64_t lda, const void* B, int64_t ldb, const dmvae_epilogue* epi,
                                const dmvae_debug_finalize* fin, const dmvae_debug_gather* gat, int ngat, int gat_last);
 int dmvae_debug_gemm_grouped_fin(void* stream, const dmvae_gemm_problem* probs, int n, const dmvae_debug_finalize* fin);
+int dmvae_debug_gemm_grouped_dw_adam_gather(void* stream, const dmvae_gemm_problem* probs, int n, const dmvae_adam_ctx* ctx,
+                                            const dmvae_debug_gather* gat, int ngat, int32_t* sync);
 
 #ifdef __cplusplus
 }
```

After: 14.70 million images/sec, median of 6. 1.2% higher.
